# distributed-lab/era-boojum

Measured on AMD Instinct MI355X. Metric: LDE+Merkle commit Goldilocks elems/s (2^22x256, LDE x4), higher is better.
Workload: dtype u64 (Goldilocks); 1 GPU; C3: 2^22 rows x 256 cols, LDE x4, Poseidon2 cap 16; rows=4194304, cols=256, lde=4, cap=16, tree_hasher=poseidon2, parallelism=single, launch=stream

## Files before the change

### era-boojum_amd/csrc/ntt_ct_common.hpp

```cpp
#pragma once
#include <hip/hip_runtime.h>
#include "gl.hpp"
#include "gl_asm.hpp"
#include "ntt_pow2.hpp"

namespace bj {
namespace {

constexpr int NT = 256;
constexpr int PT = 32;
constexpr int TILE = NT * PT;

__device__ __forceinline__ void split2(uint64_t x, uint32_t& lo, uint32_t& hi) {
    lo = (uint32_t)x;
    hi = (uint32_t)(x >> 32);
}
__device__ __forceinline__ uint64_t join2(uint32_t lo, uint32_t hi) { return ((uint64_t)hi << 32) | lo; }

__device__ __forceinline__ void ct_bfly_x4(uint64_t& xa0, uint64_t& xc0, uint64_t& xa1, uint64_t& xc1,
                                           uint64_t& xa2, uint64_t& xc2, uint64_t& xa3, uint64_t& xc3, uint64_t w0,
                                           uint64_t w1, uint64_t w2, uint64_t w3) {
    uint64_t A[4], C[4];
    glasm::ct_bfly_x4((uint32_t)xa0, (uint32_t)(xa0 >> 32), (uint32_t)xc0, (uint32_t)(xc0 >> 32), (uint32_t)w0,
                      (uint32_t)(w0 >> 32), A[0], C[0],
                      (uint32_t)xa1, (uint32_t)(xa1 >> 32), (uint32_t)xc1, (uint32_t)(xc1 >> 32), (uint32_t)w1,
                      (uint32_t)(w1 >> 32), A[1], C[1],
                      (uint32_t)xa2, (uint32_t)(xa2 >> 32), (uint32_t)xc2, (uint32_t)(xc2 >> 32), (uint32_t)w2,
                      (uint32_t)(w2 >> 32), A[2], C[2],
                      (uint32_t)xa3, (uint32_t)(xa3 >> 32), (uint32_t)xc3, (uint32_t)(xc3 >> 32), (uint32_t)w3,
                      (uint32_t)(w3 >> 32), A[3], C[3]);
    xa0 = A[0]; xc0 = C[0];
    xa1 = A[1]; xc1 = C[1];
    xa2 = A[2]; xc2 = C[2];
    xa3 = A[3]; xc3 = C[3];
}

__device__ __forceinline__ void mul4_by(uint64_t& x0, uint64_t& x1, uint64_t& x2, uint64_t& x3, uint64_t k) {
    uint32_t a0[4], a1[4], z0[4], z1[4], k0, k1;
    split2(k, k0, k1);
    split2(x0, a0[0], a1[0]); split2(x1, a0[1], a1[1]);
    split2(x2, a0[2], a1[2]); split2(x3, a0[3], a1[3]);
    glasm::mul_x4(a0[0], a1[0], k0, k1, z0[0], z1[0], a0[1], a1[1], k0, k1, z0[1], z1[1],
                  a0[2], a1[2], k0, k1, z0[2], z1[2], a0[3], a1[3], k0, k1, z0[3], z1[3]);
    x0 = join2(z0[0], z1[0]); x1 = join2(z0[1], z1[1]);
    x2 = join2(z0[2], z1[2]); x3 = join2(z0[3], z1[3]);
}

__device__ __forceinline__ constexpr int pair_lo(int q, int hk) { return (q / hk) * 2 * hk + (q % hk); }

template <int HK>
__device__ __forceinline__ void ct_stage(uint64_t* x, const uint64_t* w) {
#pragma unroll
    for (int b = 0; b < 4; b++) {
        const int q0 = 4 * b;
        ct_bfly_x4(x[pair_lo(q0, HK)], x[pair_lo(q0, HK) + HK], x[pair_lo(q0 + 1, HK)], x[pair_lo(q0 + 1, HK) + HK],
                   x[pair_lo(q0 + 2, HK)], x[pair_lo(q0 + 2, HK) + HK], x[pair_lo(q0 + 3, HK)],
                   x[pair_lo(q0 + 3, HK) + HK], w[q0], w[q0 + 1], w[q0 + 2], w[q0 + 3]);
    }
}

__device__ __forceinline__ void canon4(uint64_t* x) {
    uint32_t z0[4], z1[4];
    glasm::canon_x4((uint32_t)x[0], (uint32_t)(x[0] >> 32), z0[0], z1[0], (uint32_t)x[1], (uint32_t)(x[1] >> 32), z0[1],
                    z1[1], (uint32_t)x[2], (uint32_t)(x[2] >> 32), z0[2], z1[2], (uint32_t)x[3], (uint32_t)(x[3] >> 32),
                    z0[3], z1[3]);
#pragma unroll
    for (int i = 0; i < 4; i++) x[i] = join2(z0[i], z1[i]);
}

__device__ __forceinline__ uint64_t canon_u64(uint64_t v) {
    uint32_t a0, a1, z0, z1;
    split2(v, a0, a1);
    glasm::canon_x1(a0, a1, z0, z1);
    return join2(z0, z1);
}

constexpr size_t EXT_HB = 32;
constexpr size_t EXT_TA = 32 + 1024;
__host__ __device__ __forceinline__ size_t ext_tb(uint32_t u0) { return EXT_TA + ((size_t)32 << u0); }

template <int LOG, bool INV, int B>
__device__ __forceinline__ void dft_p2(uint64_t* x) {
    using namespace p2dft;
    if constexpr (LOG == 1) { if constexpr (INV) dft2_inv<B>(x); else dft2_fwd<B>(x); }
    if constexpr (LOG == 2) { if constexpr (INV) dft4_inv<B>(x); else dft4_fwd<B>(x); }
    if constexpr (LOG == 3) { if constexpr (INV) dft8_inv<B>(x); else dft8_fwd<B>(x); }
    if constexpr (LOG == 4) { if constexpr (INV) dft16_inv<B>(x); else dft16_fwd<B>(x); }
    if constexpr (LOG == 5) { if constexpr (INV) dft32_inv<B>(x); else dft32_fwd<B>(x); }
}

template <int LOG, bool INV, int G = 0>
__device__ __forceinline__ void dft_p2_groups(uint64_t* x) {
    if constexpr (G < (32 >> LOG)) {
        dft_p2<LOG, INV, (G << LOG)>(x);
        dft_p2_groups<LOG, INV, G + 1>(x);
    }
}

__device__ __forceinline__ void load32(uint64_t* r, const uint64_t* __restrict__ f) {
#pragma unroll
    for (int k = 0; k < PT; k++) r[k] = f[k];
}

template <int K>
__device__ __forceinline__ void prescale_n(uint64_t* x, const uint64_t* f) {
#pragma unroll
    for (int k = 0; k < K; k += 4) {
        uint32_t z0[4], z1[4];
        glasm::mul_x4((uint32_t)x[k], (uint32_t)(x[k] >> 32), (uint32_t)f[k], (uint32_t)(f[k] >> 32), z0[0], z1[0],
                      (uint32_t)x[k + 1], (uint32_t)(x[k + 1] >> 32), (uint32_t)f[k + 1], (uint32_t)(f[k + 1] >> 32),
                      z0[1], z1[1], (uint32_t)x[k + 2], (uint32_t)(x[k + 2] >> 32), (uint32_t)f[k + 2],
                      (uint32_t)(f[k + 2] >> 32), z0[2], z1[2], (uint32_t)x[k + 3], (uint32_t)(x[k + 3] >> 32),
                      (uint32_t)f[k + 3], (uint32_t)(f[k + 3] >> 32), z0[3], z1[3]);
#pragma unroll
        for (int i = 0; i < 4; i++) x[k + i] = join2(z0[i], z1[i]);
    }
}

__device__ __forceinline__ void prescale32(uint64_t* x, const uint64_t* f) {
#pragma unroll
    for (int k = 0; k < PT; k += 4) {
        uint32_t z0[4], z1[4];
        glasm::mul_x4((uint32_t)x[k], (uint32_t)(x[k] >> 32), (uint32_t)f[k], (uint32_t)(f[k] >> 32), z0[0], z1[0],
                      (uint32_t)x[k + 1], (uint32_t)(x[k + 1] >> 32), (uint32_t)f[k + 1], (uint32_t)(f[k + 1] >> 32),
                      z0[1], z1[1], (uint32_t)x[k + 2], (uint32_t)(x[k + 2] >> 32), (uint32_t)f[k + 2],
                      (uint32_t)(f[k + 2] >> 32), z0[2], z1[2], (uint32_t)x[k + 3], (uint32_t)(x[k + 3] >> 32),
                      (uint32_t)f[k + 3], (uint32_t)(f[k + 3] >> 32), z0[3], z1[3]);
#pragma unroll
        for (int i = 0; i < 4; i++) x[k + i] = join2(z0[i], z1[i]);
    }
}

constexpr int PAD_LDS = TILE + TILE / 32;

__device__ __forceinline__ uint32_t tail_base_a(uint32_t t) { return t + (t >> 5); }
__device__ __forceinline__ uint32_t tail_base_b(uint32_t thi, uint32_t tlo) { return 264 * thi + tlo; }
__device__ __forceinline__ uint32_t tail_base_c(uint32_t t) { return 33 * t; }
__device__ __forceinline__ constexpr uint32_t tail_off_a(int k) { return 264 * k; }
__device__ __forceinline__ constexpr uint32_t tail_off_b(int k) { return 8 * k + (k >> 2); }

template <int V>
__device__ __forceinline__ void tw_ct_tailC(uint64_t* w, const uint64_t* __restrict__ ct, uint32_t u0, size_t q,
                                            uint32_t t) {
    constexpr int HK = 4 >> (V - 10);
    const uint64_t* base = ct + ((size_t)1 << (u0 + V)) + (q << V) + ((size_t)t << (V - 8));
#pragma unroll
    for (int p = 0; p < 16; p++) w[p] = base[pair_lo(p, HK) >> (13 - V)];
}

}
}
```

### era-boojum_amd/csrc/ntt_lde3.hip

```cpp
#include <hip/hip_runtime.h>
#include "gl.hpp"
#include "gl_asm.hpp"
#include "ntt_pow2.hpp"
#include "ntt_ct_common.hpp"
#include "bj_internal.hpp"

namespace bj {

namespace {

constexpr size_t L3_C = 0;
constexpr size_t L3_HA = 8192;
constexpr size_t L3_HB = L3_HA + 32;
constexpr size_t L3_F1 = L3_HB + 1024;
constexpr size_t L3_U = L3_F1 + ((size_t)1 << 18);
constexpr size_t L3_A = L3_U + 1024;
constexpr size_t L3_F2 = L3_A + ((size_t)1 << 18);

__host__ __device__ constexpr uint32_t cbrev(uint32_t x, int bits) {
    uint32_t r = 0;
    for (int i = 0; i < bits; i++) r |= ((x >> i) & 1u) << (bits - 1 - i);
    return r;
}

__device__ __forceinline__ uint32_t brev(uint32_t x, int bits) {
    return bits == 0 ? 0u : (__builtin_bitreverse32(x) >> (32 - bits));
}

__device__ __forceinline__ void prescale32_brev(uint64_t* y, const uint64_t* x, const uint64_t* f) {
#pragma unroll
    for (int k = 0; k < PT; k += 4) {
        uint32_t z0[4], z1[4];
        const uint64_t a0 = x[cbrev(k, 5)], a1 = x[cbrev(k + 1, 5)], a2 = x[cbrev(k + 2, 5)], a3 = x[cbrev(k + 3, 5)];
        glasm::mul_x4((uint32_t)a0, (uint32_t)(a0 >> 32), (uint32_t)f[k], (uint32_t)(f[k] >> 32), z0[0], z1[0],
                      (uint32_t)a1, (uint32_t)(a1 >> 32), (uint32_t)f[k + 1], (uint32_t)(f[k + 1] >> 32), z0[1], z1[1],
                      (uint32_t)a2, (uint32_t)(a2 >> 32), (uint32_t)f[k + 2], (uint32_t)(f[k + 2] >> 32), z0[2], z1[2],
                      (uint32_t)a3, (uint32_t)(a3 >> 32), (uint32_t)f[k + 3], (uint32_t)(f[k + 3] >> 32), z0[3],
                      z1[3]);
#pragma unroll
        for (int i = 0; i < 4; i++) y[k + i] = join2(z0[i], z1[i]);
    }
}

__device__ __forceinline__ __amdgpu_buffer_rsrc_t uniform_rsrc(const uint64_t* p, uint32_t bytes) {
    const uint64_t a = (uint64_t)p;
    const uint32_t lo = __builtin_amdgcn_readfirstlane((uint32_t)a);
    const uint32_t hi = __builtin_amdgcn_readfirstlane((uint32_t)(a >> 32));
    return __builtin_amdgcn_make_buffer_rsrc((void*)(((uint64_t)hi << 32) | lo), 0, (int)bytes, 0x00020000);
}

typedef unsigned int u32x2 __attribute__((ext_vector_type(2)));
__device__ __forceinline__ u32x2 as_u32x2(uint64_t v) {
    u32x2 r;
    r.x = (uint32_t)v;
    r.y = (uint32_t)(v >> 32);
    return r;
}
__device__ __forceinline__ uint64_t from_u32x2(u32x2 v) { return ((uint64_t)v.y << 32) | v.x; }

__device__ __forceinline__ void prescale32_brev_uniform(uint64_t* y, const uint64_t* x, const uint64_t* __restrict__ h) {
#pragma unroll
    for (int k8 = 0; k8 < PT; k8 += 8) {
        uint64_t hf[8];
#pragma unroll
        for (int i = 0; i < 8; i++) hf[i] = h[k8 + i];
#pragma unroll
        for (int k = k8; k < k8 + 8; k += 4) {
            uint32_t z0[4], z1[4];
            const uint64_t a0 = x[cbrev(k, 5)], a1 = x[cbrev(k + 1, 5)], a2 = x[cbrev(k + 2, 5)], a3 = x[cbrev(k + 3, 5)];
            const uint64_t f0 = hf[k - k8], f1 = hf[k - k8 + 1], f2 = hf[k - k8 + 2], f3 = hf[k - k8 + 3];
            glasm::mul_sb_x4((uint32_t)a0, (uint32_t)(a0 >> 32), (uint32_t)f0, (uint32_t)(f0 >> 32), z0[0], z1[0],
                             (uint32_t)a1, (uint32_t)(a1 >> 32), (uint32_t)f1, (uint32_t)(f1 >> 32), z0[1], z1[1],
                             (uint32_t)a2, (uint32_t)(a2 >> 32), (uint32_t)f2, (uint32_t)(f2 >> 32), z0[2], z1[2],
                             (uint32_t)a3, (uint32_t)(a3 >> 32), (uint32_t)f3, (uint32_t)(f3 >> 32), z0[3], z1[3]);
#pragma unroll
            for (int i = 0; i < 4; i++) y[k + i] = join2(z0[i], z1[i]);
        }
    }
}

__device__ __forceinline__ constexpr int c_reg(int e) { return 8 * (e / 7) + e % 7 + 1; }
template <int E0, int E1>
__device__ __forceinline__ void load_c(uint64_t* f, const uint64_t* __restrict__ c) {
#pragma unroll
    for (int e = E0; e < E1; e++) f[c_reg(e)] = c[c_reg(e)];
}

template <int E0, int E1>
__device__ __forceinline__ void prescale_c(uint64_t* y, const uint64_t* f) {
#pragma unroll
    for (int q = E0 / 4; q < E1 / 4; q++) {
        int k[4];
#pragma unroll
        for (int i = 0; i < 4; i++) k[i] = c_reg(4 * q + i);
        uint32_t z0[4], z1[4];
        glasm::mul_x4((uint32_t)y[k[0]], (uint32_t)(y[k[0]] >> 32), (uint32_t)f[k[0]], (uint32_t)(f[k[0]] >> 32), z0[0],
                      z1[0], (uint32_t)y[k[1]], (uint32_t)(y[k[1]] >> 32), (uint32_t)f[k[1]],
                      (uint32_t)(f[k[1]] >> 32), z0[1], z1[1], (uint32_t)y[k[2]], (uint32_t)(y[k[2]] >> 32),
                      (uint32_t)f[k[2]], (uint32_t)(f[k[2]] >> 32), z0[2], z1[2], (uint32_t)y[k[3]],
                      (uint32_t)(y[k[3]] >> 32), (uint32_t)f[k[3]], (uint32_t)(f[k[3]] >> 32), z0[3], z1[3]);
#pragma unroll
        for (int i = 0; i < 4; i++) y[k[i]] = join2(z0[i], z1[i]);
    }
}

__device__ __forceinline__ size_t coset_offset(uint32_t i, size_t coset_stride, size_t block_stride, uint32_t log_k) {
    return (size_t)(i >> log_k) * block_stride + (size_t)(i & ((1u << log_k) - 1)) * coset_stride;
}

template <int R>
__device__ __forceinline__ void inverse_tail13(uint64_t* x, const uint64_t* __restrict__ inv_tab, uint32_t q,
                                               uint32_t t, uint64_t* lds) {
    constexpr uint32_t LOGN = R + 13;
    const uint32_t ba = tail_base_a(t), bc = tail_base_c(t);
    const uint64_t* ext = inv_tab + ((size_t)1 << LOGN);
    uint64_t f[PT], wa[16], wb[16], wc[16];
    load32(f, ext + EXT_TA + (size_t)q * 32);
    prescale32(x, f);
    dft_p2<5, true, 0>(x);
    const uint32_t tlo = t & 7, thi = t >> 3;
    const uint32_t bb = tail_base_b(thi, tlo);
#pragma unroll
    for (int k = 0; k < PT; k++) lds[ba + tail_off_a(k)] = x[k];
    const uint64_t* tb = ext + ext_tb(R) + ((((size_t)q << 5) | thi) << 5);
#pragma unroll
    for (int k = 0; k < 16; k++) f[k] = tb[k];
    __syncthreads();
#pragma unroll
    for (int k = 0; k < PT; k++) x[k] = lds[bb + tail_off_b(k)];
    prescale_n<8>(x, f);
#pragma unroll
    for (int k = 16; k < 24; k++) f[k] = tb[k];
    prescale_n<8>(x + 8, f + 8);
#pragma unroll
    for (int k = 24; k < PT; k++) f[k] = tb[k];
    prescale_n<8>(x + 16, f + 16);
    prescale_n<8>(x + 24, f + 24);
    dft_p2<5, true, 0>(x);
    tw_ct_tailC<10>(wa, inv_tab, R, q, t);
#pragma unroll
    for (int k = 0; k < PT; k++) lds[bb + tail_off_b(k)] = x[k];
    tw_ct_tailC<11>(wb, inv_tab, R, q, t);
    tw_ct_tailC<12>(wc, inv_tab, R, q, t);
    __syncthreads();
#pragma unroll
    for (int k = 0; k < PT; k++) x[k] = lds[bc + k];
    ct_stage<4>(x, wa);
    ct_stage<2>(x, wb);
    ct_stage<1>(x, wc);
}

template <int R, bool INV_PART, bool MONO>
__global__ __launch_bounds__(NT, 2) void lde3_mid_kernel(const uint64_t* src, size_t src_stride, uint64_t* mono,
                                                         size_t mono_stride, uint64_t* lde, size_t col_stride,
                                                         size_t coset_stride, size_t block_stride, uint32_t log_k, uint32_t n_cols, uint32_t n_cosets,
                                                         const uint64_t* __restrict__ inv_tab,
                                                         const uint64_t* __restrict__ tabs, size_t tab_stride) {
    constexpr uint32_t LOGN = R + 13;
    constexpr int LW = 13 - R;
    constexpr uint32_t W = 1u << LW;
    __shared__ uint64_t lds[PAD_LDS];
    const uint32_t t = threadIdx.x;
    const uint32_t c = __builtin_amdgcn_readfirstlane(blockIdx.x % n_cols);
    const uint32_t q = __builtin_amdgcn_readfirstlane(blockIdx.x / n_cols);
    const uint64_t* blk = src + (size_t)c * src_stride + (size_t)q * TILE;
    const uint32_t ba = tail_base_a(t), bc = tail_base_c(t);
    uint64_t x[PT];
    {
        const auto rb = uniform_rsrc(blk, 8u * TILE);
#pragma unroll
        for (int k = 0; k < PT; k++)
            x[k] = from_u32x2(__builtin_amdgcn_raw_buffer_load_b64(rb, (int)(t * 8), k * 2048, 0));
    }
    if constexpr (INV_PART) {
        inverse_tail13<R>(x, inv_tab, q, t, lds);
    } else {
#pragma unroll
        for (int k = 0; k < PT; k++) lds[ba + tail_off_a(k)] = x[k];
        __syncthreads();
#pragma unroll
        for (int k = 0; k < PT; k++) x[k] = lds[bc + k];
    }
    if constexpr (MONO) {
#pragma unroll
        for (int k = 0; k < PT; k += 4) {
            uint64_t v[4] = {x[k], x[k + 1], x[k + 2], x[k + 3]};
            canon4(v);
#pragma unroll
            for (int i = 0; i < 4; i++) lds[bc + k + i] = v[i];
        }
        __syncthreads();
        const auto rm = uniform_rsrc(mono + (size_t)c * mono_stride + (size_t)q * TILE, 8u * TILE);
#pragma unroll
        for (int k = 0; k < PT; k++)
            __builtin_amdgcn_raw_buffer_store_b64(as_u32x2(lds[ba + tail_off_a(k)]), rm, (int)(t * 8), k * 2048, 0);
    }
    const uint32_t s8 = brev(t, 8);
    const uint32_t b1 = 33 * t;
    const uint32_t b2 = 1056 * (t >> 5) + (t & 31);
    const uint32_t b3 = s8 + (s8 >> 5);
    const uint32_t g5 = brev(t & 31, 5);
    const uint32_t qrot = ((q & 31u) << (R - 5)) | (q >> 5);
    const uint32_t vo = ((t >> LW) << 13) + qrot * W + (t & (W - 1));
#pragma unroll 1
    for (uint32_t i = 0; i < n_cosets; i++) {
        const uint64_t* tab = tabs + (size_t)i * tab_stride;
        uint64_t y[PT], f[PT];
        prescale32_brev_uniform(y, x, tab + L3_HA);
        dft_p2<5, false, 0>(y);
        __syncthreads();
#pragma unroll
        for (int k = 0; k < PT; k++) lds[b1 + cbrev(k, 5)] = y[k];
        const uint64_t* hb = tab + L3_HB + 32 * g5;
#pragma unroll
        for (int k = 0; k < 16; k++) f[k] = hb[k];
        __syncthreads();
#pragma unroll
        for (int k = 0; k < PT; k++) y[k] = lds[b2 + 33 * cbrev(k, 5)];
        prescale_n<8>(y, f);
#pragma unroll
        for (int k = 16; k < 24; k++) f[k] = hb[k];
        prescale_n<8>(y + 8, f + 8);
#pragma unroll
        for (int k = 24; k < PT; k++) f[k] = hb[k];
        prescale_n<8>(y + 16, f + 16);
        prescale_n<8>(y + 24, f + 24);
        dft_p2<5, false, 0>(y);
#pragma unroll
        for (int k = 0; k < PT; k++) lds[b2 + 33 * cbrev(k, 5)] = y[k];
        const uint64_t* fc = tab + L3_C + 32 * t;
        load_c<0, 16>(f, fc);
        __syncthreads();
#pragma unroll
        for (int k = 0; k < PT; k++) y[k] = lds[b3 + 264 * cbrev(k, 5)];
        prescale_c<0, 8>(y, f);
        load_c<16, 28>(f, fc);
        prescale_c<8, 16>(y, f);
        prescale_c<16, 28>(y, f);
        dft_p2_groups<3, false>(y);
        __syncthreads();
#pragma unroll
        for (int k = 0; k < PT; k++) lds[bc + k] = y[k];
        __syncthreads();
#pragma unroll
        for (int k = 0; k < PT; k++) y[k] = lds[ba + tail_off_a(k)];
        const auto rs = uniform_rsrc(lde + (size_t)c * col_stride + coset_offset(i, coset_stride, block_stride, log_k), 8u << LOGN);
#pragma unroll
        for (int k = 0; k < PT; k++)
            __builtin_amdgcn_raw_buffer_store_b64(as_u32x2(y[k]), rs, (int)(vo * 8), (int)((uint32_t)k << (24 - LW)),
                                                  0);
    }
}

constexpr uint32_t kInvFoldConsts = 256;
struct InvFoldZ {
    uint64_t z[kInvFoldConsts];
};

template <uint32_t OUTS, uint32_t F>
__device__ __forceinline__ void fold_term(uint64_t* acc, const uint64_t* x, uint32_t b, uint64_t zb, bool set) {
    const uint32_t z0 = (uint32_t)zb, z1 = (uint32_t)(zb >> 32);
#pragma unroll
    for (uint32_t i = 0; i < OUTS; i += 4) {
        uint32_t p0[4], p1[4], s0[4], s1[4];
        glasm::mul_sb_x4((uint32_t)x[F * i + b], (uint32_t)(x[F * i + b] >> 32), z0, z1, p0[0], p1[0],
                         (uint32_t)x[F * (i + 1) + b], (uint32_t)(x[F * (i + 1) + b] >> 32), z0, z1, p0[1], p1[1],
                         (uint32_t)x[F * (i + 2) + b], (uint32_t)(x[F * (i + 2) + b] >> 32), z0, z1, p0[2], p1[2],
                         (uint32_t)x[F * (i + 3) + b], (uint32_t)(x[F * (i + 3) + b] >> 32), z0, z1, p0[3], p1[3]);
        if (set) {
#pragma unroll
            for (int j = 0; j < 4; j++) acc[i + j] = join2(p0[j], p1[j]);
            continue;
        }
        glasm::add_x4((uint32_t)acc[i], (uint32_t)(acc[i] >> 32), p0[0], p1[0], s0[0], s1[0], (uint32_t)acc[i + 1],
                      (uint32_t)(acc[i + 1] >> 32), p0[1], p1[1], s0[1], s1[1], (uint32_t)acc[i + 2],
                      (uint32_t)(acc[i + 2] >> 32), p0[2], p1[2], s0[2], s1[2], (uint32_t)acc[i + 3],
                      (uint32_t)(acc[i + 3] >> 32), p0[3], p1[3], s0[3], s1[3]);
#pragma unroll
        for (int j = 0; j < 4; j++) acc[i + j] = join2(s0[j], s1[j]);
    }
}

__device__ __forceinline__ void add_sub4(uint64_t* a, uint64_t* b) {
    uint32_t s0[4], s1[4], d0[4], d1[4];
    glasm::add_x4((uint32_t)a[0], (uint32_t)(a[0] >> 32), (uint32_t)b[0], (uint32_t)(b[0] >> 32), s0[0], s1[0],
                  (uint32_t)a[1], (uint32_t)(a[1] >> 32), (uint32_t)b[1], (uint32_t)(b[1] >> 32), s0[1], s1[1],
                  (uint32_t)a[2], (uint32_t)(a[2] >> 32), (uint32_t)b[2], (uint32_t)(b[2] >> 32), s0[2], s1[2],
                  (uint32_t)a[3], (uint32_t)(a[3] >> 32), (uint32_t)b[3], (uint32_t)(b[3] >> 32), s0[3], s1[3]);
    glasm::sub_x4((uint32_t)a[0], (uint32_t)(a[0] >> 32), (uint32_t)b[0], (uint32_t)(b[0] >> 32), d0[0], d1[0],
                  (uint32_t)a[1], (uint32_t)(a[1] >> 32), (uint32_t)b[1], (uint32_t)(b[1] >> 32), d0[1], d1[1],
                  (uint32_t)a[2], (uint32_t)(a[2] >> 32), (uint32_t)b[2], (uint32_t)(b[2] >> 32), d0[2], d1[2],
                  (uint32_t)a[3], (uint32_t)(a[3] >> 32), (uint32_t)b[3], (uint32_t)(b[3] >> 32), d0[3], d1[3]);
#pragma unroll
    for (int j = 0; j < 4; j++) {
        a[j] = join2(s0[j], s1[j]);
        b[j] = join2(d0[j], d1[j]);
    }
}

template <uint32_t OUTS>
__device__ __forceinline__ void store_fold_target(const uint64_t* h, uint64_t* lds, uint32_t P, uint32_t t, uint64_t* dst,
                                                  size_t dst_col_stride, size_t dst_shard_stride, uint32_t c,
                                                  uint32_t q) {
    constexpr uint32_t BLK = NT * OUTS, HALF = PAD_LDS / 2;
    uint64_t* buf = lds + (P & 1) * HALF;
#pragma unroll
    for (uint32_t i = 0; i < OUTS; i++) {
        const uint32_t w = OUTS * t + i;
        buf[w + (w >> 5)] = h[i];
    }
    __syncthreads();
    const auto rs = uniform_rsrc(dst + (size_t)P * dst_shard_stride + (size_t)c * dst_col_stride + (size_t)q * BLK,
                                 8u * BLK);
#pragma unroll
    for (uint32_t k = 0; k < OUTS; k++) {
        const uint32_t w = t + NT * k;
        __builtin_amdgcn_raw_buffer_store_b64(as_u32x2(buf[w + (w >> 5)]), rs, (int)(t * 8), (int)(k * 2048), 0);
    }
}

template <int R, int LOG_F>
__global__ __launch_bounds__(NT, 2) void lde3_inv_fold_kernel(const uint64_t* src, size_t src_stride, uint64_t* dst,
                                                              size_t dst_col_stride, size_t dst_shard_stride,
                                                              uint32_t n_cols, uint32_t shards, uint32_t paired,
                                                              const uint64_t* __restrict__ inv_tab, InvFoldZ zc) {
    __shared__ uint64_t lds[PAD_LDS];
    const uint32_t t = threadIdx.x;
    const uint32_t rest = blockIdx.x >> 3;
    const uint32_t c = __builtin_amdgcn_readfirstlane(rest % n_cols);
    const uint32_t q = __builtin_amdgcn_readfirstlane(((rest / n_cols) << 3) | (blockIdx.x & 7));
    uint64_t x[PT];
    {
        const auto rb = uniform_rsrc(src + (size_t)c * src_stride + (size_t)q * TILE, 8u * TILE);
#pragma unroll
        for (int k = 0; k < PT; k++)
            x[k] = from_u32x2(__builtin_amdgcn_raw_buffer_load_b64(rb, (int)(t * 8), k * 2048, 0));
    }
    inverse_tail13<R>(x, inv_tab, q, t, lds);
    {
        constexpr uint32_t F = 1u << LOG_F, OUTS = PT / F, BLK = TILE / F, HALF = PAD_LDS / 2;
        static_assert(OUTS % 4 == 0 && BLK + BLK / 32 <= HALF, "fold layout");
        __syncthreads();
        if (paired) {
#pragma unroll 1
            for (uint32_t P = 0; P < shards; P += 2) {
                uint64_t h0[OUTS], h1[OUTS];
                if constexpr (F == 2) {
                    const uint64_t z = zc.z[P * F + 1];
#pragma unroll
                    for (uint32_t i = 0; i < OUTS; i++) {
                        h0[i] = x[2 * i];
                        h1[i] = x[2 * i + 1];
                    }
#pragma unroll
                    for (uint32_t i = 0; i < OUTS; i += 4)
                        ct_bfly_x4(h0[i], h1[i], h0[i + 1], h1[i + 1], h0[i + 2], h1[i + 2], h0[i + 3], h1[i + 3], z,
                                   z, z, z);
                } else {
                    uint64_t e[OUTS], o[OUTS];
#pragma unroll
                    for (uint32_t i = 0; i < OUTS; i++) e[i] = x[F * i];
#pragma unroll
                    for (uint32_t b = 1; b < F; b++)
                        fold_term<OUTS, F>(b < F / 2 ? e : o, x, b, zc.z[P * F + b], b == F / 2);
#pragma unroll
                    for (uint32_t i = 0; i < OUTS; i += 4)
                        for (int j = 0; j < 4; j++) {
                            h0[i + j] = e[i + j];
                            h1[i + j] = o[i + j];
                        }
#pragma unroll
                    for (uint32_t i = 0; i < OUTS; i += 4) add_sub4(h0 + i, h1 + i);
                }
#pragma unroll
                for (uint32_t i = 0; i < OUTS; i += 4) {
                    canon4(h0 + i);
                    canon4(h1 + i);
                }
                store_fold_target<OUTS>(h0, lds, P, t, dst, dst_col_stride, dst_shard_stride, c, q);
                store_fold_target<OUTS>(h1, lds, P + 1, t, dst, dst_col_stride, dst_shard_stride, c, q);
            }
            return;
        }
#pragma unroll 1
        for (uint32_t P = 0; P < shards; P++) {
            uint64_t h[OUTS];
#pragma unroll
            for (uint32_t i = 0; i < OUTS; i++) h[i] = x[F * i];
#pragma unroll
            for (uint32_t b = 1; b < F; b++) fold_term<OUTS, F>(h, x, b, zc.z[P * F + b], false);
#pragma unroll
            for (uint32_t i = 0; i < OUTS; i += 4) canon4(h + i);
            store_fold_target<OUTS>(h, lds, P, t, dst, dst_col_stride, dst_shard_stride, c, q);
        }
    }
}

template <int R>
__device__ __forceinline__ constexpr uint32_t fin_slot(uint32_t r, uint32_t o) {
    const uint32_t e = R == 5 ? (o << R) + r : r * (1u << (13 - R)) + o;
    return e + (e >> 5);
}
template <int R>
__device__ __forceinline__ constexpr uint32_t fin_p1(uint32_t t, uint32_t k) {
    constexpr int LW = 13 - R;
    return fin_slot<R>((k << (R - 5)) + cbrev(t >> LW, R - 5), t & ((1u << LW) - 1));
}
template <int R>
__device__ __forceinline__ constexpr uint32_t fin_p2(uint32_t t, uint32_t k) {
    constexpr int LW = 13 - R;
    const uint32_t h = k >> (R - 5), rl = k & ((1u << (R - 5)) - 1);
    const uint32_t p = (t >> LW) + (h << (R - 5));
    return fin_slot<R>((p << (R - 5)) + rl, t & ((1u << LW) - 1));
}
template <int R>
__device__ __forceinline__ constexpr uint32_t fin_p3(uint32_t t, uint32_t k) {
    const uint32_t P = t + 256 * k;
    return fin_slot<R>(P & ((1u << R) - 1), P >> R);
}

template <int R>
struct FinLds {
    static constexpr int LW = 13 - R, RL = R - 5;
    static constexpr uint32_t W = 1u << LW;
    static constexpr bool F1_LDS = R >= 8;
    static constexpr uint32_t F1 = F1_LDS ? 32 * W : 0;
    static constexpr uint32_t A = (1u << RL) * W;
    static constexpr uint32_t UP = (1u << RL) + 1;
    static constexpr uint32_t U = 32 * UP;
};

template <int R, int F2MODE>
__global__ __launch_bounds__(NT, 2) void lde3_final_kernel(uint64_t* lde, size_t col_stride, size_t coset_stride, size_t block_stride, uint32_t log_k,
                                                           uint32_t n_cols, uint32_t n_cosets,
                                                           const uint64_t* __restrict__ tabs, size_t tab_stride) {
    using FL = FinLds<R>;
    constexpr int LW = FL::LW, RL = FL::RL;
    constexpr uint32_t W = FL::W;
    __shared__ uint64_t lds[PAD_LDS];
    __shared__ uint64_t lf1[FL::F1 ? FL::F1 : 1];
    __shared__ uint64_t la[R > 5 && F2MODE == 1 ? FL::A : 1];
    __shared__ uint64_t lu[R > 5 && F2MODE == 1 ? FL::U : 1];
    const uint32_t t = threadIdx.x;
    const uint32_t rest = blockIdx.x >> 3;
    const uint32_t c = __builtin_amdgcn_readfirstlane(rest % n_cols);
    const uint32_t pair = ((rest / n_cols) << 3) | (blockIdx.x & 7);
    const uint32_t i = __builtin_amdgcn_readfirstlane(pair % n_cosets);
    const uint32_t T = __builtin_amdgcn_readfirstlane(pair / n_cosets);
    uint64_t* d = lde + (size_t)c * col_stride + coset_offset(i, coset_stride, block_stride, log_k) + (size_t)T * TILE;
    const uint64_t* tab = tabs + (size_t)i * tab_stride;
    const uint32_t o = t & (W - 1);
    const uint32_t M0 = T * W, M = M0 + o;
    uint64_t x[PT], y[PT], f[PT];
    const auto rd = uniform_rsrc(d, 8u * TILE);
    constexpr uint32_t NF1 = FL::F1_LDS ? FL::F1 / NT : 1;
    uint64_t f1v[NF1];
    if constexpr (FL::F1_LDS) {
#pragma unroll
        for (uint32_t j = 0; j < NF1; j++) {
            const uint32_t e = t + j * NT;
            f1v[j] = tab[L3_F1 + ((size_t)(e >> LW) << 13) + M0 + (e & (W - 1))];
        }
    }
#pragma unroll
    for (int k = 0; k < PT; k++) x[k] = from_u32x2(__builtin_amdgcn_raw_buffer_load_b64(rd, (int)(t * 8), k * 2048, 0));
    if constexpr (R > 5 && F2MODE == 1) {
        la[t] = tab[L3_A + ((size_t)(t >> LW) << 13) + M0 + (t & (W - 1))];
#pragma unroll
        for (uint32_t e = t; e < (32u << RL); e += NT) lu[(e >> RL) * FL::UP + (e & ((1u << RL) - 1))] = tab[L3_U + e];
    }
    uint64_t g2[F2MODE == 0 && R > 5 ? PT : 1];
    if constexpr (F2MODE == 0 && R > 5) {
        const auto rf = uniform_rsrc(tab + L3_F2 + M0, 8u << (R + 13));
        const int vf = (int)((o + ((t >> LW) << 13)) * 8);
#pragma unroll
        for (int k = 0; k < PT; k++) {
            const uint32_t h = k >> RL, rl = k & ((1u << RL) - 1);
            g2[k] = from_u32x2(__builtin_amdgcn_raw_buffer_load_b64(rf, vf, (int)((rl * 32 + (h << RL)) << 16), 0));
        }
    }
    if constexpr (FL::F1_LDS) {
#pragma unroll
        for (uint32_t j = 0; j < NF1; j++) lf1[t + j * NT] = f1v[j];
        __syncthreads();
#pragma unroll
        for (int k = 0; k < PT; k++) f[k] = lf1[k * W + o];
    } else {
        const uint64_t* f1 = tab + L3_F1 + M;
#pragma unroll
        for (int k = 0; k < PT; k++) f[k] = f1[(size_t)k << 13];
    }
    prescale32_brev(y, x, f);
    dft_p2<5, false, 0>(y);
    const uint32_t b1 = fin_p1<R>(t, 0);
#pragma unroll
    for (int k = 0; k < PT; k++) lds[b1 + (fin_p1<R>(0, k) - fin_p1<R>(0, 0))] = y[k];
    if constexpr (R > 5) {
        const uint32_t pl = t >> LW;
        if constexpr (F2MODE == 1) {
            if constexpr (!FL::F1_LDS) __syncthreads();
            uint64_t a[PT];
#pragma unroll
            for (int k = 0; k < PT; k++) {
                const uint32_t h = k >> RL, rl = k & ((1u << RL) - 1);
                a[k] = la[rl * W + o];
                f[k] = lu[(pl + (h << RL)) * FL::UP + rl];
            }
            prescale32(f, a);
        } else {
#pragma unroll
            for (int k = 0; k < PT; k++) f[k] = g2[k];
        }
        __syncthreads();
        const uint32_t b2 = fin_p2<R>(t, 0);
#pragma unroll
        for (int k = 0; k < PT; k++) y[k] = lds[b2 + (fin_p2<R>(0, k) - fin_p2<R>(0, 0))];
        prescale32(y, f);
        dft_p2_groups<RL, false>(y);
#pragma unroll
        for (int k = 0; k < PT; k++) lds[b2 + (fin_p2<R>(0, k) - fin_p2<R>(0, 0))] = y[k];
    }
    __syncthreads();
    const uint32_t b3 = fin_p3<R>(t, 0);
#pragma unroll
    for (int k = 0; k < PT; k++) y[k] = lds[b3 + (fin_p3<R>(0, k) - fin_p3<R>(0, 0))];
#pragma unroll
    for (int k = 0; k < PT; k += 4) canon4(y + k);
#pragma unroll
    for (int k = 0; k < PT; k++) __builtin_amdgcn_raw_buffer_store_b64(as_u32x2(y[k]), rd, (int)(t * 8), k * 2048, 0);
}

__global__ void lde3_table_kernel(uint64_t* out, uint32_t log_n, uint64_t w_n, uint64_t s, size_t len) {
    const size_t n = (size_t)1 << log_n;
    const uint32_t R = log_n - 13;
    for (size_t idx = blockIdx.x * (size_t)blockDim.x + threadIdx.x; idx < len;
         idx += (size_t)gridDim.x * blockDim.x) {
        uint64_t v;
        if (idx < L3_HA) {
            const uint32_t G = (uint32_t)idx >> 3, j = (uint32_t)idx & 7;
            const uint64_t sigma = gl::mul(s, gl::pow(w_n, gl::bitrev32(G, 10)));
            v = gl::pow(sigma, (n >> 13) * j);
        } else if (idx < L3_HB) {
            v = gl::pow(s, (n >> 5) * (idx - L3_HA));
        } else if (idx < L3_F1) {
            const uint32_t j = (uint32_t)(idx - L3_HB);
            const uint64_t sigma = gl::mul(s, gl::pow(w_n, gl::bitrev32(j >> 5, 5)));
            v = gl::pow(sigma, (n >> 10) * (j & 31));
        } else if (idx < L3_U) {
            const uint32_t j = (uint32_t)(idx - L3_F1);
            const uint32_t M = j & 8191, k = j >> 13;
            const uint64_t sigma = gl::mul(s, gl::pow(w_n, gl::bitrev32(M, 13)));
            v = gl::pow(sigma, (uint64_t)k << (R - 5));
        } else if (idx < L3_A) {
            const uint32_t j = (uint32_t)(idx - L3_U);
            const uint32_t p = j >> (R - 5), rl = j & ((1u << (R - 5)) - 1);
            v = (j >> R) ? 0 : gl::pow(gl::pow(w_n, 8192), (uint64_t)gl::bitrev32(p, 5) * rl);
        } else if (idx < L3_F2) {
            const uint32_t j = (uint32_t)(idx - L3_A);
            const uint32_t M = j & 8191, rl = j >> 13;
            const uint64_t sigma = gl::mul(s, gl::pow(w_n, gl::bitrev32(M, 13)));
            v = (rl >> (R - 5)) ? 0 : gl::pow(sigma, rl);
        } else {
            const size_t j = idx - L3_F2;
            const uint32_t M = (uint32_t)(j & 8191), rest = (uint32_t)(j >> 13);
            const uint32_t p = rest & 31, rl = rest >> 5;
            const uint64_t sigma = gl::mul(s, gl::pow(w_n, gl::bitrev32(M * 32 + p, 18)));
            v = gl::pow(sigma, rl);
        }
        out[idx] = gl::canon(v);
    }
}

template <int R>
void launch_lde3_R(uint64_t* lde, size_t col_stride, size_t coset_stride, size_t block_stride, uint32_t log_k, uint32_t n_cosets, const uint64_t* src,
                   size_t src_stride, uint64_t* mono, size_t mono_stride, uint32_t n_cols, const uint64_t* inv_tab,
                   const uint64_t* tabs, size_t tab_stride, hipStream_t st, uint32_t passes) {
    const dim3 gm(n_cols << R);
    if (!(passes & LDE3_MID))
        ;
    else if (inv_tab && mono)
        hipLaunchKernelGGL((lde3_mid_kernel<R, true, true>), gm, dim3(NT), 0, st, src, src_stride, mono, mono_stride,
                           lde, col_stride, coset_stride, block_stride, log_k, n_cols, n_cosets, inv_tab, tabs, tab_stride);
    else if (inv_tab)
        hipLaunchKernelGGL((lde3_mid_kernel<R, true, false>), gm, dim3(NT), 0, st, src, src_stride, mono,
                           mono_stride, lde, col_stride, coset_stride, block_stride, log_k, n_cols, n_cosets, inv_tab, tabs, tab_stride);
    else
        hipLaunchKernelGGL((lde3_mid_kernel<R, false, false>), gm, dim3(NT), 0, st, src, src_stride, mono,
                           mono_stride, lde, col_stride, coset_stride, block_stride, log_k, n_cols, n_cosets, inv_tab, tabs, tab_stride);
    const dim3 gf((n_cols * n_cosets) << R);
    if (passes & LDE3_FINAL)
        hipLaunchKernelGGL((lde3_final_kernel<R, 0>), gf, dim3(NT), 0, st, lde, col_stride, coset_stride, block_stride,
                           log_k, n_cols, n_cosets, tabs, tab_stride);
}

}

bool lde3_supported(uint32_t log_n) { return log_n >= 18 && log_n <= 23; }

size_t lde3_table_len(uint32_t log_n) {
    return log_n > 18 ? L3_F2 + ((size_t)1 << log_n) : L3_F2;
}

hipError_t launch_lde3_table(uint64_t* out, uint32_t log_n, uint64_t shift, hipStream_t st) {
    if (!lde3_supported(log_n)) return hipErrorInvalidValue;
    const size_t len = lde3_table_len(log_n);
    size_t blocks = (len + 255) / 256;
    if (blocks > 16384) blocks = 16384;
    hipLaunchKernelGGL(lde3_table_kernel, dim3((unsigned)blocks), dim3(256), 0, st, out, log_n,
                       gl::domain_generator(log_n), gl::canon(shift), len);
    return hipGetLastError();
}

hipError_t launch_lde3(uint64_t* lde, size_t col_stride, size_t coset_stride, uint32_t n_cosets, const uint64_t* src,
                       size_t src_stride, uint64_t* mono, size_t mono_stride, uint32_t n_cols, uint32_t log_n,
                       const uint64_t* inv_tab, const uint64_t* tabs, size_t tab_stride, hipStream_t st,
                       uint32_t log_k, size_t block_stride, uint32_t passes) {
    if (n_cols == 0 || n_cosets == 0) return hipSuccess;
    if (log_k > 31) log_k = 31;
    if (!lde3_supported(log_n)) return hipErrorInvalidValue;
    if (((uint64_t)n_cols * n_cosets) << (log_n - 13) > (0xffffffffull / NT)) return hipErrorInvalidValue;
#define BJ_LDE3(RR)                                                                                              \
    launch_lde3_R<RR>(lde, col_stride, coset_stride, block_stride, log_k, n_cosets, src, src_stride, mono, mono_stride, n_cols, inv_tab, \
                      tabs, tab_stride, st, passes)
    switch (log_n - 13) {
        case 5: BJ_LDE3(5); break;
        case 6: BJ_LDE3(6); break;
        case 7: BJ_LDE3(7); break;
        case 8: BJ_LDE3(8); break;
        case 9: BJ_LDE3(9); break;
        default: BJ_LDE3(10); break;
    }
#undef BJ_LDE3
    return hipGetLastError();
}

namespace {
template <int R>
void launch_lde3_inv_fold_R(uint64_t* dst, size_t dst_col_stride, size_t dst_shard_stride, const uint64_t* src,
                            size_t src_stride, uint32_t n_cols, uint32_t log_f, uint32_t shards, uint32_t paired,
                            const uint64_t* inv_tab, const InvFoldZ& zc, hipStream_t st) {
    const dim3 g(n_cols << R);
#define BJ_INV(LF)                                                                                             \
    hipLaunchKernelGGL((lde3_inv_fold_kernel<R, LF>), g, dim3(NT), 0, st, src, src_stride, dst, dst_col_stride, \
                       dst_shard_stride, n_cols, shards, paired, inv_tab, zc)
    switch (log_f) {
        case 1: BJ_INV(1); break;
        case 2: BJ_INV(2); break;
        default: BJ_INV(3); break;
    }
#undef BJ_INV
}
}

bool lde3_inv_fold_supported(uint32_t log_n, uint32_t log_f, uint32_t shards) {
    return lde3_supported(log_n) && log_f >= 1 && log_f <= 3 && shards >= 1 &&
           (size_t)shards << log_f <= kInvFoldConsts;
}

hipError_t launch_lde3_inv_fold(uint64_t* dst, size_t dst_col_stride, size_t dst_shard_stride, const uint64_t* src,
                                size_t src_stride, uint32_t n_cols, uint32_t log_n, uint32_t log_f, uint32_t shards,
                                const uint64_t* s_pow_m, const uint64_t* inv_tab, hipStream_t st) {
    if (n_cols == 0) return hipSuccess;
    if (!lde3_inv_fold_supported(log_n, log_f, shards)) return hipErrorInvalidValue;
    if (((uint64_t)n_cols << (log_n - 13)) > 0xffffffffull / NT) return hipErrorInvalidValue;
    InvFoldZ zc{};
    const uint32_t F = 1u << log_f;
    for (uint32_t P = 0; P < shards; P++) {
        uint64_t acc = 1;
        for (uint32_t a = 0; a < F; a++) {
            zc.z[P * F + gl::bitrev32(a, log_f)] = acc;
            acc = gl::mul(acc, s_pow_m[P]);
        }
    }
    uint32_t paired = shards % 2 == 0 && !knobs().inv_fold_unpaired;
    for (uint32_t P = 0; paired && P < shards; P += 2)
        paired = gl::canon(s_pow_m[P + 1]) == gl::canon(gl::sub(0, s_pow_m[P]));
#define BJ_INVR(RR) \
    launch_lde3_inv_fold_R<RR>(dst, dst_col_stride, dst_shard_stride, src, src_stride, n_cols, log_f, shards, paired, \
                               inv_tab, zc, st)
    switch (log_n - 13) {
        case 5: BJ_INVR(5); break;
        case 6: BJ_INVR(6); break;
        case 7: BJ_INVR(7); break;
        case 8: BJ_INVR(8); break;
        case 9: BJ_INVR(9); break;
        default: BJ_INVR(10); break;
    }
#undef BJ_INVR
    return hipGetLastError();
}

}
```

### era-boojum_amd/csrc/ntt_pow2.hpp

```cpp
#pragma once
#include <stdint.h>

namespace glasm {

__device__ __forceinline__ void p2c0_x1(uint32_t a00, uint32_t a10, uint32_t c00, uint32_t c10, uint64_t& A0, uint64_t& C0) {
    uint64_t q40, q42, q64;
    uint32_t k66;
    asm volatile(
        "v_mov_b32 v10, 0xfffeffff\n"
        "s_mov_b32 %[k66], 0xffff\n"
        "v_add_co_u32 v0, %[q40], %[c00], -1\n"
        "s_nop 1\n"
        "v_addc_co_u32 v1, %[q40], %[c10], 0, %[q40]\n"
        "s_nop 1\n"
        "v_cndmask_b32_e64 v2, %[c00], v0, %[q40]\n"
        "v_cndmask_b32_e64 v3, %[c10], v1, %[q40]\n"
        "v_sub_co_u32 v0, %[q42], %[a00], v2\n"
        "s_nop 1\n"
        "v_subb_co_u32 v1, %[q42], %[a10], v3, %[q42]\n"
        "s_nop 1\n"
        "v_cndmask_b32_e64 v6, 0, v10, %[q42]\n"
        "v_mad_i64_i32 %[C0], %[q64], v6, %[k66], v[0:1]\n"
        "v_add_co_u32 v4, %[q40], %[a00], v2\n"
        "s_nop 1\n"
// ... 653 lines not shown
        "v_cndmask_b32_e64 v23, v23, v21, %[q52]\n"
        "v_cndmask_b32_e64 v33, v33, v31, %[q58]\n"
        "v_sub_co_u32 v0, %[q42], %[a00], v2\n"
        "v_sub_co_u32 v10, %[q48], %[a01], v12\n"
        "v_sub_co_u32 v20, %[q54], %[a02], v22\n"
        "v_sub_co_u32 v30, %[q60], %[a03], v32\n"
        "v_subb_co_u32 v1, %[q42], %[a10], v3, %[q42]\n"
        "v_subb_co_u32 v11, %[q48], %[a11], v13, %[q48]\n"
        "v_subb_co_u32 v21, %[q54], %[a12], v23, %[q54]\n"
        "v_subb_co_u32 v31, %[q60], %[a13], v33, %[q60]\n"
        "v_cndmask_b32_e64 v6, 0, v40, %[q42]\n"
        "v_cndmask_b32_e64 v16, 0, v40, %[q48]\n"
        "v_cndmask_b32_e64 v26, 0, v40, %[q54]\n"
        "v_cndmask_b32_e64 v36, 0, v40, %[q60]\n"
        "v_mad_i64_i32 %[C0], %[q64], v6, %[k66], v[0:1]\n"
        "v_mad_i64_i32 %[C1], %[q64], v16, %[k66], v[10:11]\n"
        "v_mad_i64_i32 %[C2], %[q64], v26, %[k66], v[20:21]\n"
        "v_mad_i64_i32 %[C3], %[q64], v36, %[k66], v[30:31]\n"
        "v_add_co_u32 v4, %[q40], %[a00], v2\n"
        "v_add_co_u32 v14, %[q46], %[a01], v12\n"
        "v_add_co_u32 v24, %[q52], %[a02], v22\n"
        "v_add_co_u32 v34, %[q58], %[a03], v32\n"
        "v_addc_co_u32 v5, %[q40], %[a10], v3, %[q40]\n"
        "v_addc_co_u32 v15, %[q46], %[a11], v13, %[q46]\n"
        "v_addc_co_u32 v25, %[q52], %[a12], v23, %[q52]\n"
        "v_addc_co_u32 v35, %[q58], %[a13], v33, %[q58]\n"
        "v_cndmask_b32_e64 v2, 0, -1, %[q40]\n"
        "v_cndmask_b32_e64 v12, 0, -1, %[q46]\n"
        "v_cndmask_b32_e64 v22, 0, -1, %[q52]\n"
        "v_cndmask_b32_e64 v32, 0, -1, %[q58]\n"
        "v_mad_u64_u32 %[A0], %[q64], v2, 1, v[4:5]\n"
        "v_mad_u64_u32 %[A1], %[q64], v12, 1, v[14:15]\n"
        "v_mad_u64_u32 %[A2], %[q64], v22, 1, v[24:25]\n"
        "v_mad_u64_u32 %[A3], %[q64], v32, 1, v[34:35]\n"
        : [A0] "=&v"(A0), [C0] "=&v"(C0), [A1] "=&v"(A1), [C1] "=&v"(C1), [A2] "=&v"(A2), [C2] "=&v"(C2), [A3] "=&v"(A3), [C3] "=&v"(C3), [q40] "=&s"(q40), [q42] "=&s"(q42), [q46] "=&s"(q46), [q48] "=&s"(q48), [q52] "=&s"(q52), [q54] "=&s"(q54), [q58] "=&s"(q58), [q60] "=&s"(q60), [q64] "=&s"(q64), [k66] "=&s"(k66)
        : [a00] "v"(a00), [a10] "v"(a10), [c00] "v"(c00), [c10] "v"(c10), [e0] "n"(S0), [r0] "n"(32 - S0), [a01] "v"(a01), [a11] "v"(a11), [c01] "v"(c01), [c11] "v"(c11), [e1] "n"(S1), [r1] "n"(32 - S1), [a02] "v"(a02), [a12] "v"(a12), [c02] "v"(c02), [c12] "v"(c12), [e2] "n"(S2), [r2] "n"(32 - S2), [a03] "v"(a03), [a13] "v"(a13), [c03] "v"(c03), [c13] "v"(c13), [e3] "n"(S3), [r3] "n"(32 - S3)
        : "v0", "v1", "v2", "v3", "v4", "v5", "v6", "v7", "v8", "v9", "v10", "v11", "v12", "v13", "v14", "v15", "v16", "v17", "v18", "v19", "v20", "v21", "v22", "v23", "v24", "v25", "v26", "v27", "v28", "v29", "v30", "v31", "v32", "v33", "v34", "v35", "v36", "v37", "v38", "v39", "v40");
}

template <int S0>
__device__ __forceinline__ void p2c3_x1(uint32_t a00, uint32_t a10, uint32_t c00, uint32_t c10, uint64_t& A0, uint64_t& C0) {
    uint64_t q40, q42, q64;
    uint32_t k66;
    asm volatile(
        "v_mov_b32 v10, 0xfffeffff\n"
        "s_mov_b32 %[k66], 0xffff\n"
        "v_lshlrev_b32 v8, %[e0], %[c00]\n"
        "v_alignbit_b32 v4, %[c10], %[c00], %[r0]\n"
        "v_lshrrev_b32 v5, %[r0], %[c10]\n"
        "v_mad_u64_u32 v[2:3], %[q64], v8, -1, 0\n"
        "v_sub_co_u32 v2, %[q42], v2, v4\n"
        "s_nop 1\n"
        "v_subb_co_u32 v3, %[q42], v3, v5, %[q42]\n"
        "s_nop 1\n"
        "v_cndmask_b32_e64 v9, 0, v10, %[q42]\n"
        "v_mad_i64_i32 v[2:3], %[q64], v9, %[k66], v[2:3]\n"
        "v_add_co_u32 v0, %[q40], v2, -1\n"
        "s_nop 1\n"
        "v_addc_co_u32 v1, %[q40], v3, 0, %[q40]\n"
        "s_nop 1\n"
        "v_cndmask_b32_e64 v2, v2, v0, %[q40]\n"
        "v_cndmask_b32_e64 v3, v3, v1, %[q40]\n"
        "v_sub_co_u32 v0, %[q42], %[a00], v2\n"
        "s_nop 1\n"
        "v_subb_co_u32 v1, %[q42], %[a10], v3, %[q42]\n"
        "s_nop 1\n"
        "v_cndmask_b32_e64 v6, 0, v10, %[q42]\n"
        "v_mad_i64_i32 %[C0], %[q64], v6, %[k66], v[0:1]\n"
        "v_add_co_u32 v4, %[q40], %[a00], v2\n"
        "s_nop 1\n"
        "v_addc_co_u32 v5, %[q40], %[a10], v3, %[q40]\n"
        "s_nop 1\n"
        "v_cndmask_b32_e64 v2, 0, -1, %[q40]\n"
        "v_mad_u64_u32 %[A0], %[q64], v2, 1, v[4:5]\n"
        : [A0] "=&v"(A0), [C0] "=&v"(C0), [q40] "=&s"(q40), [q42] "=&s"(q42), [q64] "=&s"(q64), [k66] "=&s"(k66)
        : [a00] "v"(a00), [a10] "v"(a10), [c00] "v"(c00), [c10] "v"(c10), [e0] "n"(S0), [r0] "n"(32 - S0)
        : "v0", "v1", "v2", "v3", "v4", "v5", "v6", "v7", "v8", "v9", "v10");
}

template <int S0, int S1>
__device__ __forceinline__ void p2c3_x2(uint32_t a00, uint32_t a10, uint32_t c00, uint32_t c10, uint64_t& A0, uint64_t& C0, uint32_t a01, uint32_t a11, uint32_t c01, uint32_t c11, uint64_t& A1, uint64_t& C1) {
    uint64_t q40, q42, q46, q48, q64;
    uint32_t k66;
    asm volatile(
        "v_mov_b32 v20, 0xfffeffff\n"
        "s_mov_b32 %[k66], 0xffff\n"
        "v_lshlrev_b32 v8, %[e0], %[c00]\n"
        "v_lshlrev_b32 v18, %[e1], %[c01]\n"
        "v_alignbit_b32 v4, %[c10], %[c00], %[r0]\n"
        "v_alignbit_b32 v14, %[c11], %[c01], %[r1]\n"
        "v_lshrrev_b32 v5, %[r0], %[c10]\n"
        "v_lshrrev_b32 v15, %[r1], %[c11]\n"
        "v_mad_u64_u32 v[2:3], %[q64], v8, -1, 0\n"
        "v_mad_u64_u32 v[12:13], %[q64], v18, -1, 0\n"
        "v_sub_co_u32 v2, %[q42], v2, v4\n"
        "v_sub_co_u32 v12, %[q48], v12, v14\n"
        "s_nop 0\n"
        "v_subb_co_u32 v3, %[q42], v3, v5, %[q42]\n"
        "v_subb_co_u32 v13, %[q48], v13, v15, %[q48]\n"
        "s_nop 0\n"
        "v_cndmask_b32_e64 v9, 0, v20, %[q42]\n"
        "v_cndmask_b32_e64 v19, 0, v20, %[q48]\n"
        "v_mad_i64_i32 v[2:3], %[q64], v9, %[k66], v[2:3]\n"
        "v_mad_i64_i32 v[12:13], %[q64], v19, %[k66], v[12:13]\n"
        "v_add_co_u32 v0, %[q40], v2, -1\n"
        "v_add_co_u32 v10, %[q46], v12, -1\n"
        "s_nop 0\n"
        "v_addc_co_u32 v1, %[q40], v3, 0, %[q40]\n"
        "v_addc_co_u32 v11, %[q46], v13, 0, %[q46]\n"
        "s_nop 0\n"
        "v_cndmask_b32_e64 v2, v2, v0, %[q40]\n"
        "v_cndmask_b32_e64 v12, v12, v10, %[q46]\n"
        "v_cndmask_b32_e64 v3, v3, v1, %[q40]\n"
        "v_cndmask_b32_e64 v13, v13, v11, %[q46]\n"
        "v_sub_co_u32 v0, %[q42], %[a00], v2\n"
        "v_sub_co_u32 v10, %[q48], %[a01], v12\n"
        "s_nop 0\n"
        "v_subb_co_u32 v1, %[q42], %[a10], v3, %[q42]\n"
        "v_subb_co_u32 v11, %[q48], %[a11], v13, %[q48]\n"
        "s_nop 0\n"
        "v_cndmask_b32_e64 v6, 0, v20, %[q42]\n"
        "v_cndmask_b32_e64 v16, 0, v20, %[q48]\n"
        "v_mad_i64_i32 %[C0], %[q64], v6, %[k66], v[0:1]\n"
        "v_mad_i64_i32 %[C1], %[q64], v16, %[k66], v[10:11]\n"
        "v_add_co_u32 v4, %[q40], %[a00], v2\n"
        "v_add_co_u32 v14, %[q46], %[a01], v12\n"
        "s_nop 0\n"
        "v_addc_co_u32 v5, %[q40], %[a10], v3, %[q40]\n"
        "v_addc_co_u32 v15, %[q46], %[a11], v13, %[q46]\n"
        "s_nop 0\n"
        "v_cndmask_b32_e64 v2, 0, -1, %[q40]\n"
        "v_cndmask_b32_e64 v12, 0, -1, %[q46]\n"
        "v_mad_u64_u32 %[A0], %[q64], v2, 1, v[4:5]\n"
        "v_mad_u64_u32 %[A1], %[q64], v12, 1, v[14:15]\n"
        : [A0] "=&v"(A0), [C0] "=&v"(C0), [A1] "=&v"(A1), [C1] "=&v"(C1), [q40] "=&s"(q40), [q42] "=&s"(q42), [q46] "=&s"(q46), [q48] "=&s"(q48), [q64] "=&s"(q64), [k66] "=&s"(k66)
        : [a00] "v"(a00), [a10] "v"(a10), [c00] "v"(c00), [c10] "v"(c10), [e0] "n"(S0), [r0] "n"(32 - S0), [a01] "v"(a01), [a11] "v"(a11), [c01] "v"(c01), [c11] "v"(c11), [e1] "n"(S1), [r1] "n"(32 - S1)
        : "v0", "v1", "v2", "v3", "v4", "v5", "v6", "v7", "v8", "v9", "v10", "v11", "v12", "v13", "v14", "v15", "v16", "v17", "v18", "v19", "v20");
}

template <int S0, int S1, int S2>
__device__ __forceinline__ void p2c3_x3(uint32_t a00, uint32_t a10, uint32_t c00, uint32_t c10, uint64_t& A0, uint64_t& C0, uint32_t a01, uint32_t a11, uint32_t c01, uint32_t c11, uint64_t& A1, uint64_t& C1, uint32_t a02, uint32_t a12, uint32_t c02, uint32_t c12, uint64_t& A2, uint64_t& C2) {
    uint64_t q40, q42, q46, q48, q52, q54, q64;
    uint32_t k66;
    asm volatile(
        "v_mov_b32 v30, 0xfffeffff\n"
        "s_mov_b32 %[k66], 0xffff\n"
        "v_lshlrev_b32 v8, %[e0], %[c00]\n"
        "v_lshlrev_b32 v18, %[e1], %[c01]\n"
        "v_lshlrev_b32 v28, %[e2], %[c02]\n"
        "v_alignbit_b32 v4, %[c10], %[c00], %[r0]\n"
        "v_alignbit_b32 v14, %[c11], %[c01], %[r1]\n"
        "v_alignbit_b32 v24, %[c12], %[c02], %[r2]\n"
        "v_lshrrev_b32 v5, %[r0], %[c10]\n"
        "v_lshrrev_b32 v15, %[r1], %[c11]\n"
        "v_lshrrev_b32 v25, %[r2], %[c12]\n"
        "v_mad_u64_u32 v[2:3], %[q64], v8, -1, 0\n"
        "v_mad_u64_u32 v[12:13], %[q64], v18, -1, 0\n"
        "v_mad_u64_u32 v[22:23], %[q64], v28, -1, 0\n"
        "v_sub_co_u32 v2, %[q42], v2, v4\n"
        "v_sub_co_u32 v12, %[q48], v12, v14\n"
        "v_sub_co_u32 v22, %[q54], v22, v24\n"
        "v_subb_co_u32 v3, %[q42], v3, v5, %[q42]\n"
        "v_subb_co_u32 v13, %[q48], v13, v15, %[q48]\n"
        "v_subb_co_u32 v23, %[q54], v23, v25, %[q54]\n"
        "v_cndmask_b32_e64 v9, 0, v30, %[q42]\n"
        "v_cndmask_b32_e64 v19, 0, v30, %[q48]\n"
        "v_cndmask_b32_e64 v29, 0, v30, %[q54]\n"
        "v_mad_i64_i32 v[2:3], %[q64], v9, %[k66], v[2:3]\n"
        "v_mad_i64_i32 v[12:13], %[q64], v19, %[k66], v[12:13]\n"
        "v_mad_i64_i32 v[22:23], %[q64], v29, %[k66], v[22:23]\n"
        "v_add_co_u32 v0, %[q40], v2, -1\n"
        "v_add_co_u32 v10, %[q46], v12, -1\n"
        "v_add_co_u32 v20, %[q52], v22, -1\n"
        "v_addc_co_u32 v1, %[q40], v3, 0, %[q40]\n"
        "v_addc_co_u32 v11, %[q46], v13, 0, %[q46]\n"
        "v_addc_co_u32 v21, %[q52], v23, 0, %[q52]\n"
        "v_cndmask_b32_e64 v2, v2, v0, %[q40]\n"
        "v_cndmask_b32_e64 v12, v12, v10, %[q46]\n"
        "v_cndmask_b32_e64 v22, v22, v20, %[q52]\n"
        "v_cndmask_b32_e64 v3, v3, v1, %[q40]\n"
        "v_cndmask_b32_e64 v13, v13, v11, %[q46]\n"
        "v_cndmask_b32_e64 v23, v23, v21, %[q52]\n"
        "v_sub_co_u32 v0, %[q42], %[a00], v2\n"
        "v_sub_co_u32 v10, %[q48], %[a01], v12\n"
        "v_sub_co_u32 v20, %[q54], %[a02], v22\n"
        "v_subb_co_u32 v1, %[q42], %[a10], v3, %[q42]\n"
        "v_subb_co_u32 v11, %[q48], %[a11], v13, %[q48]\n"
        "v_subb_co_u32 v21, %[q54], %[a12], v23, %[q54]\n"
        "v_cndmask_b32_e64 v6, 0, v30, %[q42]\n"
        "v_cndmask_b32_e64 v16, 0, v30, %[q48]\n"
        "v_cndmask_b32_e64 v26, 0, v30, %[q54]\n"
        "v_mad_i64_i32 %[C0], %[q64], v6, %[k66], v[0:1]\n"
        "v_mad_i64_i32 %[C1], %[q64], v16, %[k66], v[10:11]\n"
        "v_mad_i64_i32 %[C2], %[q64], v26, %[k66], v[20:21]\n"
        "v_add_co_u32 v4, %[q40], %[a00], v2\n"
        "v_add_co_u32 v14, %[q46], %[a01], v12\n"
        "v_add_co_u32 v24, %[q52], %[a02], v22\n"
        "v_addc_co_u32 v5, %[q40], %[a10], v3, %[q40]\n"
        "v_addc_co_u32 v15, %[q46], %[a11], v13, %[q46]\n"
        "v_addc_co_u32 v25, %[q52], %[a12], v23, %[q52]\n"
        "v_cndmask_b32_e64 v2, 0, -1, %[q40]\n"
        "v_cndmask_b32_e64 v12, 0, -1, %[q46]\n"
        "v_cndmask_b32_e64 v22, 0, -1, %[q52]\n"
        "v_mad_u64_u32 %[A0], %[q64], v2, 1, v[4:5]\n"
        "v_mad_u64_u32 %[A1], %[q64], v12, 1, v[14:15]\n"
        "v_mad_u64_u32 %[A2], %[q64], v22, 1, v[24:25]\n"
        : [A0] "=&v"(A0), [C0] "=&v"(C0), [A1] "=&v"(A1), [C1] "=&v"(C1), [A2] "=&v"(A2), [C2] "=&v"(C2), [q40] "=&s"(q40), [q42] "=&s"(q42), [q46] "=&s"(q46), [q48] "=&s"(q48), [q52] "=&s"(q52), [q54] "=&s"(q54), [q64] "=&s"(q64), [k66] "=&s"(k66)
        : [a00] "v"(a00), [a10] "v"(a10), [c00] "v"(c00), [c10] "v"(c10), [e0] "n"(S0), [r0] "n"(32 - S0), [a01] "v"(a01), [a11] "v"(a11), [c01] "v"(c01), [c11] "v"(c11), [e1] "n"(S1), [r1] "n"(32 - S1), [a02] "v"(a02), [a12] "v"(a12), [c02] "v"(c02), [c12] "v"(c12), [e2] "n"(S2), [r2] "n"(32 - S2)
        : "v0", "v1", "v2", "v3", "v4", "v5", "v6", "v7", "v8", "v9", "v10", "v11", "v12", "v13", "v14", "v15", "v16", "v17", "v18", "v19", "v20", "v21", "v22", "v23", "v24", "v25", "v26", "v27", "v28", "v29", "v30");
}

template <int S0, int S1, int S2, int S3>
__device__ __forceinline__ void p2c3_x4(uint32_t a00, uint32_t a10, uint32_t c00, uint32_t c10, uint64_t& A0, uint64_t& C0, uint32_t a01, uint32_t a11, uint32_t c01, uint32_t c11, uint64_t& A1, uint64_t& C1, uint32_t a02, uint32_t a12, uint32_t c02, uint32_t c12, uint64_t& A2, uint64_t& C2, uint32_t a03, uint32_t a13, uint32_t c03, uint32_t c13, uint64_t& A3, uint64_t& C3) {
    uint64_t q40, q42, q46, q48, q52, q54, q58, q60, q64;
    uint32_t k66;
    asm volatile(
        "v_mov_b32 v40, 0xfffeffff\n"
        "s_mov_b32 %[k66], 0xffff\n"
        "v_lshlrev_b32 v8, %[e0], %[c00]\n"
        "v_lshlrev_b32 v18, %[e1], %[c01]\n"
        "v_lshlrev_b32 v28, %[e2], %[c02]\n"
        "v_lshlrev_b32 v38, %[e3], %[c03]\n"
        "v_alignbit_b32 v4, %[c10], %[c00], %[r0]\n"
        "v_alignbit_b32 v14, %[c11], %[c01], %[r1]\n"
        "v_alignbit_b32 v24, %[c12], %[c02], %[r2]\n"
        "v_alignbit_b32 v34, %[c13], %[c03], %[r3]\n"
        "v_lshrrev_b32 v5, %[r0], %[c10]\n"
        "v_lshrrev_b32 v15, %[r1], %[c11]\n"
        "v_lshrrev_b32 v25, %[r2], %[c12]\n"
        "v_lshrrev_b32 v35, %[r3], %[c13]\n"
        "v_mad_u64_u32 v[2:3], %[q64], v8, -1, 0\n"
        "v_mad_u64_u32 v[12:13], %[q64], v18, -1, 0\n"
        "v_mad_u64_u32 v[22:23], %[q64], v28, -1, 0\n"
        "v_mad_u64_u32 v[32:33], %[q64], v38, -1, 0\n"
        "v_sub_co_u32 v2, %[q42], v2, v4\n"
        "v_sub_co_u32 v12, %[q48], v12, v14\n"
        "v_sub_co_u32 v22, %[q54], v22, v24\n"
        "v_sub_co_u32 v32, %[q60], v32, v34\n"
        "v_subb_co_u32 v3, %[q42], v3, v5, %[q42]\n"
        "v_subb_co_u32 v13, %[q48], v13, v15, %[q48]\n"
        "v_subb_co_u32 v23, %[q54], v23, v25, %[q54]\n"
        "v_subb_co_u32 v33, %[q60], v33, v35, %[q60]\n"
        "v_cndmask_b32_e64 v9, 0, v40, %[q42]\n"
        "v_cndmask_b32_e64 v19, 0, v40, %[q48]\n"
        "v_cndmask_b32_e64 v29, 0, v40, %[q54]\n"
        "v_cndmask_b32_e64 v39, 0, v40, %[q60]\n"
        "v_mad_i64_i32 v[2:3], %[q64], v9, %[k66], v[2:3]\n"
        "v_mad_i64_i32 v[12:13], %[q64], v19, %[k66], v[12:13]\n"
        "v_mad_i64_i32 v[22:23], %[q64], v29, %[k66], v[22:23]\n"
        "v_mad_i64_i32 v[32:33], %[q64], v39, %[k66], v[32:33]\n"
        "v_add_co_u32 v0, %[q40], v2, -1\n"
        "v_add_co_u32 v10, %[q46], v12, -1\n"
        "v_add_co_u32 v20, %[q52], v22, -1\n"
        "v_add_co_u32 v30, %[q58], v32, -1\n"
        "v_addc_co_u32 v1, %[q40], v3, 0, %[q40]\n"
        "v_addc_co_u32 v11, %[q46], v13, 0, %[q46]\n"
        "v_addc_co_u32 v21, %[q52], v23, 0, %[q52]\n"
        "v_addc_co_u32 v31, %[q58], v33, 0, %[q58]\n"
        "v_cndmask_b32_e64 v2, v2, v0, %[q40]\n"
        "v_cndmask_b32_e64 v12, v12, v10, %[q46]\n"
        "v_cndmask_b32_e64 v22, v22, v20, %[q52]\n"
        "v_cndmask_b32_e64 v32, v32, v30, %[q58]\n"
        "v_cndmask_b32_e64 v3, v3, v1, %[q40]\n"
        "v_cndmask_b32_e64 v13, v13, v11, %[q46]\n"
        "v_cndmask_b32_e64 v23, v23, v21, %[q52]\n"
        "v_cndmask_b32_e64 v33, v33, v31, %[q58]\n"
        "v_sub_co_u32 v0, %[q42], %[a00], v2\n"
        "v_sub_co_u32 v10, %[q48], %[a01], v12\n"
        "v_sub_co_u32 v20, %[q54], %[a02], v22\n"
        "v_sub_co_u32 v30, %[q60], %[a03], v32\n"
        "v_subb_co_u32 v1, %[q42], %[a10], v3, %[q42]\n"
        "v_subb_co_u32 v11, %[q48], %[a11], v13, %[q48]\n"
        "v_subb_co_u32 v21, %[q54], %[a12], v23, %[q54]\n"
        "v_subb_co_u32 v31, %[q60], %[a13], v33, %[q60]\n"
        "v_cndmask_b32_e64 v6, 0, v40, %[q42]\n"
        "v_cndmask_b32_e64 v16, 0, v40, %[q48]\n"
        "v_cndmask_b32_e64 v26, 0, v40, %[q54]\n"
        "v_cndmask_b32_e64 v36, 0, v40, %[q60]\n"
        "v_mad_i64_i32 %[C0], %[q64], v6, %[k66], v[0:1]\n"
        "v_mad_i64_i32 %[C1], %[q64], v16, %[k66], v[10:11]\n"
        "v_mad_i64_i32 %[C2], %[q64], v26, %[k66], v[20:21]\n"
        "v_mad_i64_i32 %[C3], %[q64], v36, %[k66], v[30:31]\n"
        "v_add_co_u32 v4, %[q40], %[a00], v2\n"
        "v_add_co_u32 v14, %[q46], %[a01], v12\n"
        "v_add_co_u32 v24, %[q52], %[a02], v22\n"
        "v_add_co_u32 v34, %[q58], %[a03], v32\n"
        "v_addc_co_u32 v5, %[q40], %[a10], v3, %[q40]\n"
        "v_addc_co_u32 v15, %[q46], %[a11], v13, %[q46]\n"
        "v_addc_co_u32 v25, %[q52], %[a12], v23, %[q52]\n"
        "v_addc_co_u32 v35, %[q58], %[a13], v33, %[q58]\n"
        "v_cndmask_b32_e64 v2, 0, -1, %[q40]\n"
        "v_cndmask_b32_e64 v12, 0, -1, %[q46]\n"
        "v_cndmask_b32_e64 v22, 0, -1, %[q52]\n"
        "v_cndmask_b32_e64 v32, 0, -1, %[q58]\n"
        "v_mad_u64_u32 %[A0], %[q64], v2, 1, v[4:5]\n"
        "v_mad_u64_u32 %[A1], %[q64], v12, 1, v[14:15]\n"
        "v_mad_u64_u32 %[A2], %[q64], v22, 1, v[24:25]\n"
        "v_mad_u64_u32 %[A3], %[q64], v32, 1, v[34:35]\n"
        : [A0] "=&v"(A0), [C0] "=&v"(C0), [A1] "=&v"(A1), [C1] "=&v"(C1), [A2] "=&v"(A2), [C2] "=&v"(C2), [A3] "=&v"(A3), [C3] "=&v"(C3), [q40] "=&s"(q40), [q42] "=&s"(q42), [q46] "=&s"(q46), [q48] "=&s"(q48), [q52] "=&s"(q52), [q54] "=&s"(q54), [q58] "=&s"(q58), [q60] "=&s"(q60), [q64] "=&s"(q64), [k66] "=&s"(k66)
        : [a00] "v"(a00), [a10] "v"(a10), [c00] "v"(c00), [c10] "v"(c10), [e0] "n"(S0), [r0] "n"(32 - S0), [a01] "v"(a01), [a11] "v"(a11), [c01] "v"(c01), [c11] "v"(c11), [e1] "n"(S1), [r1] "n"(32 - S1), [a02] "v"(a02), [a12] "v"(a12), [c02] "v"(c02), [c12] "v"(c12), [e2] "n"(S2), [r2] "n"(32 - S2), [a03] "v"(a03), [a13] "v"(a13), [c03] "v"(c03), [c13] "v"(c13), [e3] "n"(S3), [r3] "n"(32 - S3)
        : "v0", "v1", "v2", "v3", "v4", "v5", "v6", "v7", "v8", "v9", "v10", "v11", "v12", "v13", "v14", "v15", "v16", "v17", "v18", "v19", "v20", "v21", "v22", "v23", "v24", "v25", "v26", "v27", "v28", "v29", "v30", "v31", "v32", "v33", "v34", "v35", "v36", "v37", "v38", "v39", "v40");
}

}

namespace bj {
namespace p2dft {
#define LO(v) ((uint32_t)(v))
#define HI(v) ((uint32_t)((v) >> 32))

template <int B>
__device__ __forceinline__ void dft2_fwd(uint64_t* x) {
    {
        uint64_t ta0, tc0;
        glasm::p2c0_x1(LO(x[B + 0]), HI(x[B + 0]), LO(x[B + 1]), HI(x[B + 1]), ta0, tc0);
        x[B + 0] = ta0; x[B + 1] = tc0;
    }
}

template <int B>
__device__ __forceinline__ void dft4_fwd(uint64_t* x) {
    {
        uint64_t ta0, tc0, ta1, tc1;
        glasm::p2c0_x2(LO(x[B + 0]), HI(x[B + 0]), LO(x[B + 2]), HI(x[B + 2]), ta0, tc0, LO(x[B + 1]), HI(x[B + 1]), LO(x[B + 3]), HI(x[B + 3]), ta1, tc1);
        x[B + 0] = ta0; x[B + 2] = tc0;
        x[B + 1] = ta1; x[B + 3] = tc1;
    }
    {
        uint64_t ta0, tc0;
        glasm::p2c0_x1(LO(x[B + 0]), HI(x[B + 0]), LO(x[B + 1]), HI(x[B + 1]), ta0, tc0);
        x[B + 0] = ta0; x[B + 1] = tc0;
    }
    {
        uint64_t ta0, tc0;
        glasm::p2c2_x1<16>(LO(x[B + 2]), HI(x[B + 2]), LO(x[B + 3]), HI(x[B + 3]), ta0, tc0);
        x[B + 2] = ta0; x[B + 3] = tc0;
    }
}

template <int B>
__device__ __forceinline__ void dft8_fwd(uint64_t* x) {
    {
        uint64_t ta0, tc0, ta1, tc1, ta2, tc2, ta3, tc3;
        glasm::p2c0_x4(LO(x[B + 0]), HI(x[B + 0]), LO(x[B + 4]), HI(x[B + 4]), ta0, tc0, LO(x[B + 1]), HI(x[B + 1]), LO(x[B + 5]), HI(x[B + 5]), ta1, tc1, LO(x[B + 2]), HI(x[B + 2]), LO(x[B + 6]), HI(x[B + 6]), ta2, tc2, LO(x[B + 3]), HI(x[B + 3]), LO(x[B + 7]), HI(x[B + 7]), ta3, tc3);
        x[B + 0] = ta0; x[B + 4] = tc0;
        x[B + 1] = ta1; x[B + 5] = tc1;
        x[B + 2] = ta2; x[B + 6] = tc2;
        x[B + 3] = ta3; x[B + 7] = tc3;
    }
    {
        uint64_t ta0, tc0, ta1, tc1;
        glasm::p2c0_x2(LO(x[B + 0]), HI(x[B + 0]), LO(x[B + 2]), HI(x[B + 2]), ta0, tc0, LO(x[B + 1]), HI(x[B + 1]), LO(x[B + 3]), HI(x[B + 3]), ta1, tc1);
        x[B + 0] = ta0; x[B + 2] = tc0;
        x[B + 1] = ta1; x[B + 3] = tc1;
    }
    {
        uint64_t ta0, tc0, ta1, tc1;
        glasm::p2c2_x2<16, 16>(LO(x[B + 4]), HI(x[B + 4]), LO(x[B + 6]), HI(x[B + 6]), ta0, tc0, LO(x[B + 5]), HI(x[B + 5]), LO(x[B + 7]), HI(x[B + 7]), ta1, tc1);
        x[B + 4] = ta0; x[B + 6] = tc0;
        x[B + 5] = ta1; x[B + 7] = tc1;
    }
    {
        uint64_t ta0, tc0;
        glasm::p2c0_x1(LO(x[B + 0]), HI(x[B + 0]), LO(x[B + 1]), HI(x[B + 1]), ta0, tc0);
        x[B + 0] = ta0; x[B + 1] = tc0;
    }
    {
        uint64_t ta0, tc0;
        glasm::p2c1_x1<24>(LO(x[B + 4]), HI(x[B + 4]), LO(x[B + 5]), HI(x[B + 5]), ta0, tc0);
        x[B + 4] = tc0; x[B + 5] = ta0;
    }
    {
        uint64_t ta0, tc0;
        glasm::p2c2_x1<16>(LO(x[B + 2]), HI(x[B + 2]), LO(x[B + 3]), HI(x[B + 3]), ta0, tc0);
        x[B + 2] = ta0; x[B + 3] = tc0;
    }
    {
        uint64_t ta0, tc0;
        glasm::p2c3_x1<8>(LO(x[B + 6]), HI(x[B + 6]), LO(x[B + 7]), HI(x[B + 7]), ta0, tc0);
        x[B + 6] = tc0; x[B + 7] = ta0;
    }
}

template <int B>
__device__ __forceinline__ void dft16_fwd(uint64_t* x) {
    {
        uint64_t ta0, tc0, ta1, tc1, ta2, tc2, ta3, tc3;
        glasm::p2c0_x4(LO(x[B + 0]), HI(x[B + 0]), LO(x[B + 8]), HI(x[B + 8]), ta0, tc0, LO(x[B + 1]), HI(x[B + 1]), LO(x[B + 9]), HI(x[B + 9]), ta1, tc1, LO(x[B + 2]), HI(x[B + 2]), LO(x[B + 10]), HI(x[B + 10]), ta2, tc2, LO(x[B + 3]), HI(x[B + 3]), LO(x[B + 11]), HI(x[B + 11]), ta3, tc3);
        x[B + 0] = ta0; x[B + 8] = tc0;
        x[B + 1] = ta1; x[B + 9] = tc1;
        x[B + 2] = ta2; x[B + 10] = tc2;
        x[B + 3] = ta3; x[B + 11] = tc3;
    }
    {
        uint64_t ta0, tc0, ta1, tc1, ta2, tc2, ta3, tc3;
        glasm::p2c0_x4(LO(x[B + 4]), HI(x[B + 4]), LO(x[B + 12]), HI(x[B + 12]), ta0, tc0, LO(x[B + 5]), HI(x[B + 5]), LO(x[B + 13]), HI(x[B + 13]), ta1, tc1, LO(x[B + 6]), HI(x[B + 6]), LO(x[B + 14]), HI(x[B + 14]), ta2, tc2, LO(x[B + 7]), HI(x[B + 7]), LO(x[B + 15]), HI(x[B + 15]), ta3, tc3);
        x[B + 4] = ta0; x[B + 12] = tc0;
        x[B + 5] = ta1; x[B + 13] = tc1;
        x[B + 6] = ta2; x[B + 14] = tc2;
        x[B + 7] = ta3; x[B + 15] = tc3;
    }
    {
        uint64_t ta0, tc0, ta1, tc1, ta2, tc2, ta3, tc3;
        glasm::p2c0_x4(LO(x[B + 0]), HI(x[B + 0]), LO(x[B + 4]), HI(x[B + 4]), ta0, tc0, LO(x[B + 1]), HI(x[B + 1]), LO(x[B + 5]), HI(x[B + 5]), ta1, tc1, LO(x[B + 2]), HI(x[B + 2]), LO(x[B + 6]), HI(x[B + 6]), ta2, tc2, LO(x[B + 3]), HI(x[B + 3]), LO(x[B + 7]), HI(x[B + 7]), ta3, tc3);
        x[B + 0] = ta0; x[B + 4] = tc0;
        x[B + 1] = ta1; x[B + 5] = tc1;
        x[B + 2] = ta2; x[B + 6] = tc2;
        x[B + 3] = ta3; x[B + 7] = tc3;
    }
    {
        uint64_t ta0, tc0, ta1, tc1, ta2, tc2, ta3, tc3;
        glasm::p2c2_x4<16, 16, 16, 16>(LO(x[B + 8]), HI(x[B + 8]), LO(x[B + 12]), HI(x[B + 12]), ta0, tc0, LO(x[B + 9]), HI(x[B + 9]), LO(x[B + 13]), HI(x[B + 13]), ta1, tc1, LO(x[B + 10]), HI(x[B + 10]), LO(x[B + 14]), HI(x[B + 14]), ta2, tc2, LO(x[B + 11]), HI(x[B + 11]), LO(x[B + 15]), HI(x[B + 15]), ta3, tc3);
        x[B + 8] = ta0; x[B + 12] = tc0;
        x[B + 9] = ta1; x[B + 13] = tc1;
        x[B + 10] = ta2; x[B + 14] = tc2;
        x[B + 11] = ta3; x[B + 15] = tc3;
    }
    {
        uint64_t ta0, tc0, ta1, tc1;
        glasm::p2c0_x2(LO(x[B + 0]), HI(x[B + 0]), LO(x[B + 2]), HI(x[B + 2]), ta0, tc0, LO(x[B + 1]), HI(x[B + 1]), LO(x[B + 3]), HI(x[B + 3]), ta1, tc1);
        x[B + 0] = ta0; x[B + 2] = tc0;
        x[B + 1] = ta1; x[B + 3] = tc1;
    }
    {
        uint64_t ta0, tc0, ta1, tc1;
        glasm::p2c1_x2<24, 24>(LO(x[B + 8]), HI(x[B + 8]), LO(x[B + 10]), HI(x[B + 10]), ta0, tc0, LO(x[B + 9]), HI(x[B + 9]), LO(x[B + 11]), HI(x[B + 11]), ta1, tc1);
        x[B + 8] = tc0; x[B + 10] = ta0;
        x[B + 9] = tc1; x[B + 11] = ta1;
    }
    {
        uint64_t ta0, tc0, ta1, tc1;
        glasm::p2c2_x2<16, 16>(LO(x[B + 4]), HI(x[B + 4]), LO(x[B + 6]), HI(x[B + 6]), ta0, tc0, LO(x[B + 5]), HI(x[B + 5]), LO(x[B + 7]), HI(x[B + 7]), ta1, tc1);
        x[B + 4] = ta0; x[B + 6] = tc0;
        x[B + 5] = ta1; x[B + 7] = tc1;
    }
    {
        uint64_t ta0, tc0, ta1, tc1;
        glasm::p2c3_x2<8, 8>(LO(x[B + 12]), HI(x[B + 12]), LO(x[B + 14]), HI(x[B + 14]), ta0, tc0, LO(x[B + 13]), HI(x[B + 13]), LO(x[B + 15]), HI(x[B + 15]), ta1, tc1);
        x[B + 12] = tc0; x[B + 14] = ta0;
        x[B + 13] = tc1; x[B + 15] = ta1;
    }
    {
        uint64_t ta0, tc0;
        glasm::p2c0_x1(LO(x[B + 0]), HI(x[B + 0]), LO(x[B + 1]), HI(x[B + 1]), ta0, tc0);
        x[B + 0] = ta0; x[B + 1] = tc0;
    }
    {
        uint64_t ta0, tc0, ta1, tc1;
        glasm::p2c1_x2<24, 12>(LO(x[B + 4]), HI(x[B + 4]), LO(x[B + 5]), HI(x[B + 5]), ta0, tc0, LO(x[B + 10]), HI(x[B + 10]), LO(x[B + 11]), HI(x[B + 11]), ta1, tc1);
        x[B + 4] = tc0; x[B + 5] = ta0;
        x[B + 10] = ta1; x[B + 11] = tc1;
    }
    {
        uint64_t ta0, tc0, ta1, tc1, ta2, tc2;
        glasm::p2c2_x3<16, 28, 4>(LO(x[B + 2]), HI(x[B + 2]), LO(x[B + 3]), HI(x[B + 3]), ta0, tc0, LO(x[B + 8]), HI(x[B + 8]), LO(x[B + 9]), HI(x[B + 9]), ta1, tc1, LO(x[B + 14]), HI(x[B + 14]), LO(x[B + 15]), HI(x[B + 15]), ta2, tc2);
        x[B + 2] = ta0; x[B + 3] = tc0;
        x[B + 8] = tc1; x[B + 9] = ta1;
        x[B + 14] = tc2; x[B + 15] = ta2;
    }
    {
        uint64_t ta0, tc0, ta1, tc1;
        glasm::p2c3_x2<8, 20>(LO(x[B + 6]), HI(x[B + 6]), LO(x[B + 7]), HI(x[B + 7]), ta0, tc0, LO(x[B + 12]), HI(x[B + 12]), LO(x[B + 13]), HI(x[B + 13]), ta1, tc1);
        x[B + 6] = tc0; x[B + 7] = ta0;
        x[B + 12] = ta1; x[B + 13] = tc1;
    }
}

template <int B>
__device__ __forceinline__ void dft32_fwd(uint64_t* x) {
    {
        uint64_t ta0, tc0, ta1, tc1, ta2, tc2, ta3, tc3;
        glasm::p2c0_x4(LO(x[B + 0]), HI(x[B + 0]), LO(x[B + 16]), HI(x[B + 16]), ta0, tc0, LO(x[B + 1]), HI(x[B + 1]), LO(x[B + 17]), HI(x[B + 17]), ta1, tc1, LO(x[B + 2]), HI(x[B + 2]), LO(x[B + 18]), HI(x[B + 18]), ta2, tc2, LO(x[B + 3]), HI(x[B + 3]), LO(x[B + 19]), HI(x[B + 19]), ta3, tc3);
        x[B + 0] = ta0; x[B + 16] = tc0;
        x[B + 1] = ta1; x[B + 17] = tc1;
        x[B + 2] = ta2; x[B + 18] = tc2;
        x[B + 3] = ta3; x[B + 19] = tc3;
    }
    {
        uint64_t ta0, tc0, ta1, tc1, ta2, tc2, ta3, tc3;
        glasm::p2c0_x4(LO(x[B + 4]), HI(x[B + 4]), LO(x[B + 20]), HI(x[B + 20]), ta0, tc0, LO(x[B + 5]), HI(x[B + 5]), LO(x[B + 21]), HI(x[B + 21]), ta1, tc1, LO(x[B + 6]), HI(x[B + 6]), LO(x[B + 22]), HI(x[B + 22]), ta2, tc2, LO(x[B + 7]), HI(x[B + 7]), LO(x[B + 23]), HI(x[B + 23]), ta3, tc3);
        x[B + 4] = ta0; x[B + 20] = tc0;
        x[B + 5] = ta1; x[B + 21] = tc1;
        x[B + 6] = ta2; x[B + 22] = tc2;
        x[B + 7] = ta3; x[B + 23] = tc3;
    }
    {
        uint64_t ta0, tc0, ta1, tc1, ta2, tc2, ta3, tc3;
        glasm::p2c0_x4(LO(x[B + 8]), HI(x[B + 8]), LO(x[B + 24]), HI(x[B + 24]), ta0, tc0, LO(x[B + 9]), HI(x[B + 9]), LO(x[B + 25]), HI(x[B + 25]), ta1, tc1, LO(x[B + 10]), HI(x[B + 10]), LO(x[B + 26]), HI(x[B + 26]), ta2, tc2, LO(x[B + 11]), HI(x[B + 11]), LO(x[B + 27]), HI(x[B + 27]), ta3, tc3);
        x[B + 8] = ta0; x[B + 24] = tc0;
        x[B + 9] = ta1; x[B + 25] = tc1;
        x[B + 10] = ta2; x[B + 26] = tc2;
        x[B + 11] = ta3; x[B + 27] = tc3;
    }
    {
        uint64_t ta0, tc0, ta1, tc1, ta2, tc2, ta3, tc3;
        glasm::p2c0_x4(LO(x[B + 12]), HI(x[B + 12]), LO(x[B + 28]), HI(x[B + 28]), ta0, tc0, LO(x[B + 13]), HI(x[B + 13]), LO(x[B + 29]), HI(x[B + 29]), ta1, tc1, LO(x[B + 14]), HI(x[B + 14]), LO(x[B + 30]), HI(x[B + 30]), ta2, tc2, LO(x[B + 15]), HI(x[B + 15]), LO(x[B + 31]), HI(x[B + 31]), ta3, tc3);
        x[B + 12] = ta0; x[B + 28] = tc0;
        x[B + 13] = ta1; x[B + 29] = tc1;
        x[B + 14] = ta2; x[B + 30] = tc2;
        x[B + 15] = ta3; x[B + 31] = tc3;
    }
    {
        uint64_t ta0, tc0, ta1, tc1, ta2, tc2, ta3, tc3;
        glasm::p2c0_x4(LO(x[B + 0]), HI(x[B + 0]), LO(x[B + 8]), HI(x[B + 8]), ta0, tc0, LO(x[B + 1]), HI(x[B + 1]), LO(x[B + 9]), HI(x[B + 9]), ta1, tc1, LO(x[B + 2]), HI(x[B + 2]), LO(x[B + 10]), HI(x[B + 10]), ta2, tc2, LO(x[B + 3]), HI(x[B + 3]), LO(x[B + 11]), HI(x[B + 11]), ta3, tc3);
        x[B + 0] = ta0; x[B + 8] = tc0;
        x[B + 1] = ta1; x[B + 9] = tc1;
        x[B + 2] = ta2; x[B + 10] = tc2;
        x[B + 3] = ta3; x[B + 11] = tc3;
    }
    {
        uint64_t ta0, tc0, ta1, tc1, ta2, tc2, ta3, tc3;
        glasm::p2c0_x4(LO(x[B + 4]), HI(x[B + 4]), LO(x[B + 12]), HI(x[B + 12]), ta0, tc0, LO(x[B + 5]), HI(x[B + 5]), LO(x[B + 13]), HI(x[B + 13]), ta1, tc1, LO(x[B + 6]), HI(x[B + 6]), LO(x[B + 14]), HI(x[B + 14]), ta2, tc2, LO(x[B + 7]), HI(x[B + 7]), LO(x[B + 15]), HI(x[B + 15]), ta3, tc3);
        x[B + 4] = ta0; x[B + 12] = tc0;
        x[B + 5] = ta1; x[B + 13] = tc1;
        x[B + 6] = ta2; x[B + 14] = tc2;
        x[B + 7] = ta3; x[B + 15] = tc3;
    }
    {
        uint64_t ta0, tc0, ta1, tc1, ta2, tc2, ta3, tc3;
        glasm::p2c2_x4<16, 16, 16, 16>(LO(x[B + 16]), HI(x[B + 16]), LO(x[B + 24]), HI(x[B + 24]), ta0, tc0, LO(x[B + 17]), HI(x[B + 17]), LO(x[B + 25]), HI(x[B + 25]), ta1, tc1, LO(x[B + 18]), HI(x[B + 18]), LO(x[B + 26]), HI(x[B + 26]), ta2, tc2, LO(x[B + 19]), HI(x[B + 19]), LO(x[B + 27]), HI(x[B + 27]), ta3, tc3);
        x[B + 16] = ta0; x[B + 24] = tc0;
        x[B + 17] = ta1; x[B + 25] = tc1;
        x[B + 18] = ta2; x[B + 26] = tc2;
        x[B + 19] = ta3; x[B + 27] = tc3;
    }
    {
        uint64_t ta0, tc0, ta1, tc1, ta2, tc2, ta3, tc3;
        glasm::p2c2_x4<16, 16, 16, 16>(LO(x[B + 20]), HI(x[B + 20]), LO(x[B + 28]), HI(x[B + 28]), ta0, tc0, LO(x[B + 21]), HI(x[B + 21]), LO(x[B + 29]), HI(x[B + 29]), ta1, tc1, LO(x[B + 22]), HI(x[B + 22]), LO(x[B + 30]), HI(x[B + 30]), ta2, tc2, LO(x[B + 23]), HI(x[B + 23]), LO(x[B + 31]), HI(x[B + 31]), ta3, tc3);
        x[B + 20] = ta0; x[B + 28] = tc0;
        x[B + 21] = ta1; x[B + 29] = tc1;
        x[B + 22] = ta2; x[B + 30] = tc2;
        x[B + 23] = ta3; x[B + 31] = tc3;
    }
    {
        uint64_t ta0, tc0, ta1, tc1, ta2, tc2, ta3, tc3;
        glasm::p2c0_x4(LO(x[B + 0]), HI(x[B + 0]), LO(x[B + 4]), HI(x[B + 4]), ta0, tc0, LO(x[B + 1]), HI(x[B + 1]), LO(x[B + 5]), HI(x[B + 5]), ta1, tc1, LO(x[B + 2]), HI(x[B + 2]), LO(x[B + 6]), HI(x[B + 6]), ta2, tc2, LO(x[B + 3]), HI(x[B + 3]), LO(x[B + 7]), HI(x[B + 7]), ta3, tc3);
        x[B + 0] = ta0; x[B + 4] = tc0;
        x[B + 1] = ta1; x[B + 5] = tc1;
        x[B + 2] = ta2; x[B + 6] = tc2;
        x[B + 3] = ta3; x[B + 7] = tc3;
    }
    {
        uint64_t ta0, tc0, ta1, tc1, ta2, tc2, ta3, tc3;
        glasm::p2c1_x4<24, 24, 24, 24>(LO(x[B + 16]), HI(x[B + 16]), LO(x[B + 20]), HI(x[B + 20]), ta0, tc0, LO(x[B + 17]), HI(x[B + 17]), LO(x[B + 21]), HI(x[B + 21]), ta1, tc1, LO(x[B + 18]), HI(x[B + 18]), LO(x[B + 22]), HI(x[B + 22]), ta2, tc2, LO(x[B + 19]), HI(x[B + 19]), LO(x[B + 23]), HI(x[B + 23]), ta3, tc3);
        x[B + 16] = tc0; x[B + 20] = ta0;
        x[B + 17] = tc1; x[B + 21] = ta1;
        x[B + 18] = tc2; x[B + 22] = ta2;
        x[B + 19] = tc3; x[B + 23] = ta3;
    }
    {
        uint64_t ta0, tc0, ta1, tc1, ta2, tc2, ta3, tc3;
        glasm::p2c2_x4<16, 16, 16, 16>(LO(x[B + 8]), HI(x[B + 8]), LO(x[B + 12]), HI(x[B + 12]), ta0, tc0, LO(x[B + 9]), HI(x[B + 9]), LO(x[B + 13]), HI(x[B + 13]), ta1, tc1, LO(x[B + 10]), HI(x[B + 10]), LO(x[B + 14]), HI(x[B + 14]), ta2, tc2, LO(x[B + 11]), HI(x[B + 11]), LO(x[B + 15]), HI(x[B + 15]), ta3, tc3);
        x[B + 8] = ta0; x[B + 12] = tc0;
        x[B + 9] = ta1; x[B + 13] = tc1;
        x[B + 10] = ta2; x[B + 14] = tc2;
        x[B + 11] = ta3; x[B + 15] = tc3;
    }
    {
        uint64_t ta0, tc0, ta1, tc1, ta2, tc2, ta3, tc3;
        glasm::p2c3_x4<8, 8, 8, 8>(LO(x[B + 24]), HI(x[B + 24]), LO(x[B + 28]), HI(x[B + 28]), ta0, tc0, LO(x[B + 25]), HI(x[B + 25]), LO(x[B + 29]), HI(x[B + 29]), ta1, tc1, LO(x[B + 26]), HI(x[B + 26]), LO(x[B + 30]), HI(x[B + 30]), ta2, tc2, LO(x[B + 27]), HI(x[B + 27]), LO(x[B + 31]), HI(x[B + 31]), ta3, tc3);
        x[B + 24] = tc0; x[B + 28] = ta0;
        x[B + 25] = tc1; x[B + 29] = ta1;
        x[B + 26] = tc2; x[B + 30] = ta2;
        x[B + 27] = tc3; x[B + 31] = ta3;
    }
    {
        uint64_t ta0, tc0, ta1, tc1;
        glasm::p2c0_x2(LO(x[B + 0]), HI(x[B + 0]), LO(x[B + 2]), HI(x[B + 2]), ta0, tc0, LO(x[B + 1]), HI(x[B + 1]), LO(x[B + 3]), HI(x[B + 3]), ta1, tc1);
        x[B + 0] = ta0; x[B + 2] = tc0;
        x[B + 1] = ta1; x[B + 3] = tc1;
    }
    {
        uint64_t ta0, tc0, ta1, tc1, ta2, tc2, ta3, tc3;
        glasm::p2c1_x4<24, 24, 12, 12>(LO(x[B + 8]), HI(x[B + 8]), LO(x[B + 10]), HI(x[B + 10]), ta0, tc0, LO(x[B + 9]), HI(x[B + 9]), LO(x[B + 11]), HI(x[B + 11]), ta1, tc1, LO(x[B + 20]), HI(x[B + 20]), LO(x[B + 22]), HI(x[B + 22]), ta2, tc2, LO(x[B + 21]), HI(x[B + 21]), LO(x[B + 23]), HI(x[B + 23]), ta3, tc3);
        x[B + 8] = tc0; x[B + 10] = ta0;
        x[B + 9] = tc1; x[B + 11] = ta1;
        x[B + 20] = ta2; x[B + 22] = tc2;
        x[B + 21] = ta3; x[B + 23] = tc3;
    }
    {
        uint64_t ta0, tc0, ta1, tc1, ta2, tc2, ta3, tc3;
        glasm::p2c2_x4<16, 16, 28, 28>(LO(x[B + 4]), HI(x[B + 4]), LO(x[B + 6]), HI(x[B + 6]), ta0, tc0, LO(x[B + 5]), HI(x[B + 5]), LO(x[B + 7]), HI(x[B + 7]), ta1, tc1, LO(x[B + 16]), HI(x[B + 16]), LO(x[B + 18]), HI(x[B + 18]), ta2, tc2, LO(x[B + 17]), HI(x[B + 17]), LO(x[B + 19]), HI(x[B + 19]), ta3, tc3);
        x[B + 4] = ta0; x[B + 6] = tc0;
        x[B + 5] = ta1; x[B + 7] = tc1;
        x[B + 16] = tc2; x[B + 18] = ta2;
        x[B + 17] = tc3; x[B + 19] = ta3;
    }
    {
        uint64_t ta0, tc0, ta1, tc1;
        glasm::p2c2_x2<4, 4>(LO(x[B + 28]), HI(x[B + 28]), LO(x[B + 30]), HI(x[B + 30]), ta0, tc0, LO(x[B + 29]), HI(x[B + 29]), LO(x[B + 31]), HI(x[B + 31]), ta1, tc1);
        x[B + 28] = tc0; x[B + 30] = ta0;
        x[B + 29] = tc1; x[B + 31] = ta1;
    }
    {
        uint64_t ta0, tc0, ta1, tc1, ta2, tc2, ta3, tc3;
        glasm::p2c3_x4<8, 8, 20, 20>(LO(x[B + 12]), HI(x[B + 12]), LO(x[B + 14]), HI(x[B + 14]), ta0, tc0, LO(x[B + 13]), HI(x[B + 13]), LO(x[B + 15]), HI(x[B + 15]), ta1, tc1, LO(x[B + 24]), HI(x[B + 24]), LO(x[B + 26]), HI(x[B + 26]), ta2, tc2, LO(x[B + 25]), HI(x[B + 25]), LO(x[B + 27]), HI(x[B + 27]), ta3, tc3);
        x[B + 12] = tc0; x[B + 14] = ta0;
        x[B + 13] = tc1; x[B + 15] = ta1;
        x[B + 24] = ta2; x[B + 26] = tc2;
        x[B + 25] = ta3; x[B + 27] = tc3;
    }
    {
        uint64_t ta0, tc0;
        glasm::p2c0_x1(LO(x[B + 0]), HI(x[B + 0]), LO(x[B + 1]), HI(x[B + 1]), ta0, tc0);
        x[B + 0] = ta0; x[B + 1] = tc0;
    }
    {
        uint64_t ta0, tc0, ta1, tc1, ta2, tc2, ta3, tc3;
        glasm::p2c1_x4<24, 12, 30, 6>(LO(x[B + 4]), HI(x[B + 4]), LO(x[B + 5]), HI(x[B + 5]), ta0, tc0, LO(x[B + 10]), HI(x[B + 10]), LO(x[B + 11]), HI(x[B + 11]), ta1, tc1, LO(x[B + 18]), HI(x[B + 18]), LO(x[B + 19]), HI(x[B + 19]), ta2, tc2, LO(x[B + 20]), HI(x[B + 20]), LO(x[B + 21]), HI(x[B + 21]), ta3, tc3);
        x[B + 4] = tc0; x[B + 5] = ta0;
        x[B + 10] = ta1; x[B + 11] = tc1;
        x[B + 18] = tc2; x[B + 19] = ta2;
        x[B + 20] = ta3; x[B + 21] = tc3;
    }
    {
        uint64_t ta0, tc0;
        glasm::p2c1_x1<18>(LO(x[B + 30]), HI(x[B + 30]), LO(x[B + 31]), HI(x[B + 31]), ta0, tc0);
        x[B + 30] = ta0; x[B + 31] = tc0;
    }
    {
        uint64_t ta0, tc0, ta1, tc1, ta2, tc2, ta3, tc3;
        glasm::p2c2_x4<16, 28, 4, 22>(LO(x[B + 2]), HI(x[B + 2]), LO(x[B + 3]), HI(x[B + 3]), ta0, tc0, LO(x[B + 8]), HI(x[B + 8]), LO(x[B + 9]), HI(x[B + 9]), ta1, tc1, LO(x[B + 14]), HI(x[B + 14]), LO(x[B + 15]), HI(x[B + 15]), ta2, tc2, LO(x[B + 22]), HI(x[B + 22]), LO(x[B + 23]), HI(x[B + 23]), ta3, tc3);
        x[B + 2] = ta0; x[B + 3] = tc0;
        x[B + 8] = tc1; x[B + 9] = ta1;
        x[B + 14] = tc2; x[B + 15] = ta2;
        x[B + 22] = ta3; x[B + 23] = tc3;
    }
    {
        uint64_t ta0, tc0;
        glasm::p2c2_x1<10>(LO(x[B + 24]), HI(x[B + 24]), LO(x[B + 25]), HI(x[B + 25]), ta0, tc0);
        x[B + 24] = ta0; x[B + 25] = tc0;
    }
    {
        uint64_t ta0, tc0, ta1, tc1, ta2, tc2, ta3, tc3;
        glasm::p2c3_x4<8, 20, 14, 26>(LO(x[B + 6]), HI(x[B + 6]), LO(x[B + 7]), HI(x[B + 7]), ta0, tc0, LO(x[B + 12]), HI(x[B + 12]), LO(x[B + 13]), HI(x[B + 13]), ta1, tc1, LO(x[B + 16]), HI(x[B + 16]), LO(x[B + 17]), HI(x[B + 17]), ta2, tc2, LO(x[B + 26]), HI(x[B + 26]), LO(x[B + 27]), HI(x[B + 27]), ta3, tc3);
        x[B + 6] = tc0; x[B + 7] = ta0;
        x[B + 12] = ta1; x[B + 13] = tc1;
        x[B + 16] = ta2; x[B + 17] = tc2;
        x[B + 26] = ta3; x[B + 27] = tc3;
    }
    {
        uint64_t ta0, tc0;
        glasm::p2c3_x1<2>(LO(x[B + 28]), HI(x[B + 28]), LO(x[B + 29]), HI(x[B + 29]), ta0, tc0);
        x[B + 28] = tc0; x[B + 29] = ta0;
    }
}

template <int B>
__device__ __forceinline__ void dft2_inv(uint64_t* x) {
    {
        uint64_t ta0, tc0;
        glasm::p2c0_x1(LO(x[B + 0]), HI(x[B + 0]), LO(x[B + 1]), HI(x[B + 1]), ta0, tc0);
        x[B + 0] = ta0; x[B + 1] = tc0;
    }
}

template <int B>
__device__ __forceinline__ void dft4_inv(uint64_t* x) {
    {
        uint64_t ta0, tc0, ta1, tc1;
        glasm::p2c0_x2(LO(x[B + 0]), HI(x[B + 0]), LO(x[B + 2]), HI(x[B + 2]), ta0, tc0, LO(x[B + 1]), HI(x[B + 1]), LO(x[B + 3]), HI(x[B + 3]), ta1, tc1);
        x[B + 0] = ta0; x[B + 2] = tc0;
        x[B + 1] = ta1; x[B + 3] = tc1;
    }
    {
        uint64_t ta0, tc0;
        glasm::p2c0_x1(LO(x[B + 0]), HI(x[B + 0]), LO(x[B + 1]), HI(x[B + 1]), ta0, tc0);
        x[B + 0] = ta0; x[B + 1] = tc0;
    }
    {
        uint64_t ta0, tc0;
        glasm::p2c2_x1<16>(LO(x[B + 2]), HI(x[B + 2]), LO(x[B + 3]), HI(x[B + 3]), ta0, tc0);
        x[B + 2] = tc0; x[B + 3] = ta0;
    }
}

template <int B>
__device__ __forceinline__ void dft8_inv(uint64_t* x) {
    {
        uint64_t ta0, tc0, ta1, tc1, ta2, tc2, ta3, tc3;
        glasm::p2c0_x4(LO(x[B + 0]), HI(x[B + 0]), LO(x[B + 4]), HI(x[B + 4]), ta0, tc0, LO(x[B + 1]), HI(x[B + 1]), LO(x[B + 5]), HI(x[B + 5]), ta1, tc1, LO(x[B + 2]), HI(x[B + 2]), LO(x[B + 6]), HI(x[B + 6]), ta2, tc2, LO(x[B + 3]), HI(x[B + 3]), LO(x[B + 7]), HI(x[B + 7]), ta3, tc3);
        x[B + 0] = ta0; x[B + 4] = tc0;
        x[B + 1] = ta1; x[B + 5] = tc1;
        x[B + 2] = ta2; x[B + 6] = tc2;
        x[B + 3] = ta3; x[B + 7] = tc3;
    }
    {
        uint64_t ta0, tc0, ta1, tc1;
        glasm::p2c0_x2(LO(x[B + 0]), HI(x[B + 0]), LO(x[B + 2]), HI(x[B + 2]), ta0, tc0, LO(x[B + 1]), HI(x[B + 1]), LO(x[B + 3]), HI(x[B + 3]), ta1, tc1);
        x[B + 0] = ta0; x[B + 2] = tc0;
        x[B + 1] = ta1; x[B + 3] = tc1;
    }
    {
        uint64_t ta0, tc0, ta1, tc1;
        glasm::p2c2_x2<16, 16>(LO(x[B + 4]), HI(x[B + 4]), LO(x[B + 6]), HI(x[B + 6]), ta0, tc0, LO(x[B + 5]), HI(x[B + 5]), LO(x[B + 7]), HI(x[B + 7]), ta1, tc1);
        x[B + 4] = tc0; x[B + 6] = ta0;
        x[B + 5] = tc1; x[B + 7] = ta1;
    }
    {
        uint64_t ta0, tc0;
        glasm::p2c0_x1(LO(x[B + 0]), HI(x[B + 0]), LO(x[B + 1]), HI(x[B + 1]), ta0, tc0);
        x[B + 0] = ta0; x[B + 1] = tc0;
    }
    {
        uint64_t ta0, tc0;
        glasm::p2c1_x1<24>(LO(x[B + 6]), HI(x[B + 6]), LO(x[B + 7]), HI(x[B + 7]), ta0, tc0);
        x[B + 6] = ta0; x[B + 7] = tc0;
    }
    {
        uint64_t ta0, tc0;
        glasm::p2c2_x1<16>(LO(x[B + 2]), HI(x[B + 2]), LO(x[B + 3]), HI(x[B + 3]), ta0, tc0);
        x[B + 2] = tc0; x[B + 3] = ta0;
    }
    {
        uint64_t ta0, tc0;
        glasm::p2c3_x1<8>(LO(x[B + 4]), HI(x[B + 4]), LO(x[B + 5]), HI(x[B + 5]), ta0, tc0);
        x[B + 4] = ta0; x[B + 5] = tc0;
    }
}

template <int B>
__device__ __forceinline__ void dft16_inv(uint64_t* x) {
    {
        uint64_t ta0, tc0, ta1, tc1, ta2, tc2, ta3, tc3;
        glasm::p2c0_x4(LO(x[B + 0]), HI(x[B + 0]), LO(x[B + 8]), HI(x[B + 8]), ta0, tc0, LO(x[B + 1]), HI(x[B + 1]), LO(x[B + 9]), HI(x[B + 9]), ta1, tc1, LO(x[B + 2]), HI(x[B + 2]), LO(x[B + 10]), HI(x[B + 10]), ta2, tc2, LO(x[B + 3]), HI(x[B + 3]), LO(x[B + 11]), HI(x[B + 11]), ta3, tc3);
        x[B + 0] = ta0; x[B + 8] = tc0;
        x[B + 1] = ta1; x[B + 9] = tc1;
        x[B + 2] = ta2; x[B + 10] = tc2;
        x[B + 3] = ta3; x[B + 11] = tc3;
    }
    {
        uint64_t ta0, tc0, ta1, tc1, ta2, tc2, ta3, tc3;
        glasm::p2c0_x4(LO(x[B + 4]), HI(x[B + 4]), LO(x[B + 12]), HI(x[B + 12]), ta0, tc0, LO(x[B + 5]), HI(x[B + 5]), LO(x[B + 13]), HI(x[B + 13]), ta1, tc1, LO(x[B + 6]), HI(x[B + 6]), LO(x[B + 14]), HI(x[B + 14]), ta2, tc2, LO(x[B + 7]), HI(x[B + 7]), LO(x[B + 15]), HI(x[B + 15]), ta3, tc3);
        x[B + 4] = ta0; x[B + 12] = tc0;
        x[B + 5] = ta1; x[B + 13] = tc1;
        x[B + 6] = ta2; x[B + 14] = tc2;
        x[B + 7] = ta3; x[B + 15] = tc3;
    }
    {
        uint64_t ta0, tc0, ta1, tc1, ta2, tc2, ta3, tc3;
        glasm::p2c0_x4(LO(x[B + 0]), HI(x[B + 0]), LO(x[B + 4]), HI(x[B + 4]), ta0, tc0, LO(x[B + 1]), HI(x[B + 1]), LO(x[B + 5]), HI(x[B + 5]), ta1, tc1, LO(x[B + 2]), HI(x[B + 2]), LO(x[B + 6]), HI(x[B + 6]), ta2, tc2, LO(x[B + 3]), HI(x[B + 3]), LO(x[B + 7]), HI(x[B + 7]), ta3, tc3);
        x[B + 0] = ta0; x[B + 4] = tc0;
        x[B + 1] = ta1; x[B + 5] = tc1;
        x[B + 2] = ta2; x[B + 6] = tc2;
        x[B + 3] = ta3; x[B + 7] = tc3;
    }
    {
        uint64_t ta0, tc0, ta1, tc1, ta2, tc2, ta3, tc3;
        glasm::p2c2_x4<16, 16, 16, 16>(LO(x[B + 8]), HI(x[B + 8]), LO(x[B + 12]), HI(x[B + 12]), ta0, tc0, LO(x[B + 9]), HI(x[B + 9]), LO(x[B + 13]), HI(x[B + 13]), ta1, tc1, LO(x[B + 10]), HI(x[B + 10]), LO(x[B + 14]), HI(x[B + 14]), ta2, tc2, LO(x[B + 11]), HI(x[B + 11]), LO(x[B + 15]), HI(x[B + 15]), ta3, tc3);
        x[B + 8] = tc0; x[B + 12] = ta0;
        x[B + 9] = tc1; x[B + 13] = ta1;
        x[B + 10] = tc2; x[B + 14] = ta2;
        x[B + 11] = tc3; x[B + 15] = ta3;
    }
    {
        uint64_t ta0, tc0, ta1, tc1;
        glasm::p2c0_x2(LO(x[B + 0]), HI(x[B + 0]), LO(x[B + 2]), HI(x[B + 2]), ta0, tc0, LO(x[B + 1]), HI(x[B + 1]), LO(x[B + 3]), HI(x[B + 3]), ta1, tc1);
        x[B + 0] = ta0; x[B + 2] = tc0;
        x[B + 1] = ta1; x[B + 3] = tc1;
    }
    {
        uint64_t ta0, tc0, ta1, tc1;
        glasm::p2c1_x2<24, 24>(LO(x[B + 12]), HI(x[B + 12]), LO(x[B + 14]), HI(x[B + 14]), ta0, tc0, LO(x[B + 13]), HI(x[B + 13]), LO(x[B + 15]), HI(x[B + 15]), ta1, tc1);
        x[B + 12] = ta0; x[B + 14] = tc0;
        x[B + 13] = ta1; x[B + 15] = tc1;
    }
    {
        uint64_t ta0, tc0, ta1, tc1;
        glasm::p2c2_x2<16, 16>(LO(x[B + 4]), HI(x[B + 4]), LO(x[B + 6]), HI(x[B + 6]), ta0, tc0, LO(x[B + 5]), HI(x[B + 5]), LO(x[B + 7]), HI(x[B + 7]), ta1, tc1);
        x[B + 4] = tc0; x[B + 6] = ta0;
        x[B + 5] = tc1; x[B + 7] = ta1;
    }
    {
        uint64_t ta0, tc0, ta1, tc1;
        glasm::p2c3_x2<8, 8>(LO(x[B + 8]), HI(x[B + 8]), LO(x[B + 10]), HI(x[B + 10]), ta0, tc0, LO(x[B + 9]), HI(x[B + 9]), LO(x[B + 11]), HI(x[B + 11]), ta1, tc1);
        x[B + 8] = ta0; x[B + 10] = tc0;
        x[B + 9] = ta1; x[B + 11] = tc1;
    }
    {
        uint64_t ta0, tc0;
        glasm::p2c0_x1(LO(x[B + 0]), HI(x[B + 0]), LO(x[B + 1]), HI(x[B + 1]), ta0, tc0);
        x[B + 0] = ta0; x[B + 1] = tc0;
    }
    {
        uint64_t ta0, tc0, ta1, tc1;
        glasm::p2c1_x2<24, 12>(LO(x[B + 6]), HI(x[B + 6]), LO(x[B + 7]), HI(x[B + 7]), ta0, tc0, LO(x[B + 12]), HI(x[B + 12]), LO(x[B + 13]), HI(x[B + 13]), ta1, tc1);
        x[B + 6] = ta0; x[B + 7] = tc0;
        x[B + 12] = tc1; x[B + 13] = ta1;
    }
    {
        uint64_t ta0, tc0, ta1, tc1, ta2, tc2;
        glasm::p2c2_x3<16, 4, 28>(LO(x[B + 2]), HI(x[B + 2]), LO(x[B + 3]), HI(x[B + 3]), ta0, tc0, LO(x[B + 8]), HI(x[B + 8]), LO(x[B + 9]), HI(x[B + 9]), ta1, tc1, LO(x[B + 14]), HI(x[B + 14]), LO(x[B + 15]), HI(x[B + 15]), ta2, tc2);
        x[B + 2] = tc0; x[B + 3] = ta0;
        x[B + 8] = ta1; x[B + 9] = tc1;
        x[B + 14] = ta2; x[B + 15] = tc2;
    }
    {
        uint64_t ta0, tc0, ta1, tc1;
        glasm::p2c3_x2<8, 20>(LO(x[B + 4]), HI(x[B + 4]), LO(x[B + 5]), HI(x[B + 5]), ta0, tc0, LO(x[B + 10]), HI(x[B + 10]), LO(x[B + 11]), HI(x[B + 11]), ta1, tc1);
        x[B + 4] = ta0; x[B + 5] = tc0;
        x[B + 10] = tc1; x[B + 11] = ta1;
    }
}

template <int B>
__device__ __forceinline__ void dft32_inv(uint64_t* x) {
    {
        uint64_t ta0, tc0, ta1, tc1, ta2, tc2, ta3, tc3;
        glasm::p2c0_x4(LO(x[B + 0]), HI(x[B + 0]), LO(x[B + 16]), HI(x[B + 16]), ta0, tc0, LO(x[B + 1]), HI(x[B + 1]), LO(x[B + 17]), HI(x[B + 17]), ta1, tc1, LO(x[B + 2]), HI(x[B + 2]), LO(x[B + 18]), HI(x[B + 18]), ta2, tc2, LO(x[B + 3]), HI(x[B + 3]), LO(x[B + 19]), HI(x[B + 19]), ta3, tc3);
        x[B + 0] = ta0; x[B + 16] = tc0;
        x[B + 1] = ta1; x[B + 17] = tc1;
        x[B + 2] = ta2; x[B + 18] = tc2;
        x[B + 3] = ta3; x[B + 19] = tc3;
    }
    {
        uint64_t ta0, tc0, ta1, tc1, ta2, tc2, ta3, tc3;
        glasm::p2c0_x4(LO(x[B + 4]), HI(x[B + 4]), LO(x[B + 20]), HI(x[B + 20]), ta0, tc0, LO(x[B + 5]), HI(x[B + 5]), LO(x[B + 21]), HI(x[B + 21]), ta1, tc1, LO(x[B + 6]), HI(x[B + 6]), LO(x[B + 22]), HI(x[B + 22]), ta2, tc2, LO(x[B + 7]), HI(x[B + 7]), LO(x[B + 23]), HI(x[B + 23]), ta3, tc3);
        x[B + 4] = ta0; x[B + 20] = tc0;
        x[B + 5] = ta1; x[B + 21] = tc1;
        x[B + 6] = ta2; x[B + 22] = tc2;
        x[B + 7] = ta3; x[B + 23] = tc3;
    }
    {
        uint64_t ta0, tc0, ta1, tc1, ta2, tc2, ta3, tc3;
        glasm::p2c0_x4(LO(x[B + 8]), HI(x[B + 8]), LO(x[B + 24]), HI(x[B + 24]), ta0, tc0, LO(x[B + 9]), HI(x[B + 9]), LO(x[B + 25]), HI(x[B + 25]), ta1, tc1, LO(x[B + 10]), HI(x[B + 10]), LO(x[B + 26]), HI(x[B + 26]), ta2, tc2, LO(x[B + 11]), HI(x[B + 11]), LO(x[B + 27]), HI(x[B + 27]), ta3, tc3);
        x[B + 8] = ta0; x[B + 24] = tc0;
        x[B + 9] = ta1; x[B + 25] = tc1;
        x[B + 10] = ta2; x[B + 26] = tc2;
        x[B + 11] = ta3; x[B + 27] = tc3;
    }
    {
        uint64_t ta0, tc0, ta1, tc1, ta2, tc2, ta3, tc3;
        glasm::p2c0_x4(LO(x[B + 12]), HI(x[B + 12]), LO(x[B + 28]), HI(x[B + 28]), ta0, tc0, LO(x[B + 13]), HI(x[B + 13]), LO(x[B + 29]), HI(x[B + 29]), ta1, tc1, LO(x[B + 14]), HI(x[B + 14]), LO(x[B + 30]), HI(x[B + 30]), ta2, tc2, LO(x[B + 15]), HI(x[B + 15]), LO(x[B + 31]), HI(x[B + 31]), ta3, tc3);
        x[B + 12] = ta0; x[B + 28] = tc0;
        x[B + 13] = ta1; x[B + 29] = tc1;
        x[B + 14] = ta2; x[B + 30] = tc2;
        x[B + 15] = ta3; x[B + 31] = tc3;
    }
    {
        uint64_t ta0, tc0, ta1, tc1, ta2, tc2, ta3, tc3;
        glasm::p2c0_x4(LO(x[B + 0]), HI(x[B + 0]), LO(x[B + 8]), HI(x[B + 8]), ta0, tc0, LO(x[B + 1]), HI(x[B + 1]), LO(x[B + 9]), HI(x[B + 9]), ta1, tc1, LO(x[B + 2]), HI(x[B + 2]), LO(x[B + 10]), HI(x[B + 10]), ta2, tc2, LO(x[B + 3]), HI(x[B + 3]), LO(x[B + 11]), HI(x[B + 11]), ta3, tc3);
        x[B + 0] = ta0; x[B + 8] = tc0;
        x[B + 1] = ta1; x[B + 9] = tc1;
        x[B + 2] = ta2; x[B + 10] = tc2;
        x[B + 3] = ta3; x[B + 11] = tc3;
    }
    {
        uint64_t ta0, tc0, ta1, tc1, ta2, tc2, ta3, tc3;
        glasm::p2c0_x4(LO(x[B + 4]), HI(x[B + 4]), LO(x[B + 12]), HI(x[B + 12]), ta0, tc0, LO(x[B + 5]), HI(x[B + 5]), LO(x[B + 13]), HI(x[B + 13]), ta1, tc1, LO(x[B + 6]), HI(x[B + 6]), LO(x[B + 14]), HI(x[B + 14]), ta2, tc2, LO(x[B + 7]), HI(x[B + 7]), LO(x[B + 15]), HI(x[B + 15]), ta3, tc3);
        x[B + 4] = ta0; x[B + 12] = tc0;
        x[B + 5] = ta1; x[B + 13] = tc1;
        x[B + 6] = ta2; x[B + 14] = tc2;
        x[B + 7] = ta3; x[B + 15] = tc3;
    }
    {
        uint64_t ta0, tc0, ta1, tc1, ta2, tc2, ta3, tc3;
        glasm::p2c2_x4<16, 16, 16, 16>(LO(x[B + 16]), HI(x[B + 16]), LO(x[B + 24]), HI(x[B + 24]), ta0, tc0, LO(x[B + 17]), HI(x[B + 17]), LO(x[B + 25]), HI(x[B + 25]), ta1, tc1, LO(x[B + 18]), HI(x[B + 18]), LO(x[B + 26]), HI(x[B + 26]), ta2, tc2, LO(x[B + 19]), HI(x[B + 19]), LO(x[B + 27]), HI(x[B + 27]), ta3, tc3);
        x[B + 16] = tc0; x[B + 24] = ta0;
        x[B + 17] = tc1; x[B + 25] = ta1;
        x[B + 18] = tc2; x[B + 26] = ta2;
        x[B + 19] = tc3; x[B + 27] = ta3;
    }
    {
        uint64_t ta0, tc0, ta1, tc1, ta2, tc2, ta3, tc3;
        glasm::p2c2_x4<16, 16, 16, 16>(LO(x[B + 20]), HI(x[B + 20]), LO(x[B + 28]), HI(x[B + 28]), ta0, tc0, LO(x[B + 21]), HI(x[B + 21]), LO(x[B + 29]), HI(x[B + 29]), ta1, tc1, LO(x[B + 22]), HI(x[B + 22]), LO(x[B + 30]), HI(x[B + 30]), ta2, tc2, LO(x[B + 23]), HI(x[B + 23]), LO(x[B + 31]), HI(x[B + 31]), ta3, tc3);
        x[B + 20] = tc0; x[B + 28] = ta0;
        x[B + 21] = tc1; x[B + 29] = ta1;
        x[B + 22] = tc2; x[B + 30] = ta2;
        x[B + 23] = tc3; x[B + 31] = ta3;
    }
    {
        uint64_t ta0, tc0, ta1, tc1, ta2, tc2, ta3, tc3;
        glasm::p2c0_x4(LO(x[B + 0]), HI(x[B + 0]), LO(x[B + 4]), HI(x[B + 4]), ta0, tc0, LO(x[B + 1]), HI(x[B + 1]), LO(x[B + 5]), HI(x[B + 5]), ta1, tc1, LO(x[B + 2]), HI(x[B + 2]), LO(x[B + 6]), HI(x[B + 6]), ta2, tc2, LO(x[B + 3]), HI(x[B + 3]), LO(x[B + 7]), HI(x[B + 7]), ta3, tc3);
        x[B + 0] = ta0; x[B + 4] = tc0;
        x[B + 1] = ta1; x[B + 5] = tc1;
        x[B + 2] = ta2; x[B + 6] = tc2;
        x[B + 3] = ta3; x[B + 7] = tc3;
    }
    {
        uint64_t ta0, tc0, ta1, tc1, ta2, tc2, ta3, tc3;
        glasm::p2c1_x4<24, 24, 24, 24>(LO(x[B + 24]), HI(x[B + 24]), LO(x[B + 28]), HI(x[B + 28]), ta0, tc0, LO(x[B + 25]), HI(x[B + 25]), LO(x[B + 29]), HI(x[B + 29]), ta1, tc1, LO(x[B + 26]), HI(x[B + 26]), LO(x[B + 30]), HI(x[B + 30]), ta2, tc2, LO(x[B + 27]), HI(x[B + 27]), LO(x[B + 31]), HI(x[B + 31]), ta3, tc3);
        x[B + 24] = ta0; x[B + 28] = tc0;
        x[B + 25] = ta1; x[B + 29] = tc1;
        x[B + 26] = ta2; x[B + 30] = tc2;
        x[B + 27] = ta3; x[B + 31] = tc3;
    }
    {
        uint64_t ta0, tc0, ta1, tc1, ta2, tc2, ta3, tc3;
        glasm::p2c2_x4<16, 16, 16, 16>(LO(x[B + 8]), HI(x[B + 8]), LO(x[B + 12]), HI(x[B + 12]), ta0, tc0, LO(x[B + 9]), HI(x[B + 9]), LO(x[B + 13]), HI(x[B + 13]), ta1, tc1, LO(x[B + 10]), HI(x[B + 10]), LO(x[B + 14]), HI(x[B + 14]), ta2, tc2, LO(x[B + 11]), HI(x[B + 11]), LO(x[B + 15]), HI(x[B + 15]), ta3, tc3);
        x[B + 8] = tc0; x[B + 12] = ta0;
        x[B + 9] = tc1; x[B + 13] = ta1;
        x[B + 10] = tc2; x[B + 14] = ta2;
        x[B + 11] = tc3; x[B + 15] = ta3;
    }
    {
        uint64_t ta0, tc0, ta1, tc1, ta2, tc2, ta3, tc3;
        glasm::p2c3_x4<8, 8, 8, 8>(LO(x[B + 16]), HI(x[B + 16]), LO(x[B + 20]), HI(x[B + 20]), ta0, tc0, LO(x[B + 17]), HI(x[B + 17]), LO(x[B + 21]), HI(x[B + 21]), ta1, tc1, LO(x[B + 18]), HI(x[B + 18]), LO(x[B + 22]), HI(x[B + 22]), ta2, tc2, LO(x[B + 19]), HI(x[B + 19]), LO(x[B + 23]), HI(x[B + 23]), ta3, tc3);
        x[B + 16] = ta0; x[B + 20] = tc0;
        x[B + 17] = ta1; x[B + 21] = tc1;
        x[B + 18] = ta2; x[B + 22] = tc2;
        x[B + 19] = ta3; x[B + 23] = tc3;
    }
    {
        uint64_t ta0, tc0, ta1, tc1;
        glasm::p2c0_x2(LO(x[B + 0]), HI(x[B + 0]), LO(x[B + 2]), HI(x[B + 2]), ta0, tc0, LO(x[B + 1]), HI(x[B + 1]), LO(x[B + 3]), HI(x[B + 3]), ta1, tc1);
        x[B + 0] = ta0; x[B + 2] = tc0;
        x[B + 1] = ta1; x[B + 3] = tc1;
    }
    {
        uint64_t ta0, tc0, ta1, tc1, ta2, tc2, ta3, tc3;
        glasm::p2c1_x4<24, 24, 12, 12>(LO(x[B + 12]), HI(x[B + 12]), LO(x[B + 14]), HI(x[B + 14]), ta0, tc0, LO(x[B + 13]), HI(x[B + 13]), LO(x[B + 15]), HI(x[B + 15]), ta1, tc1, LO(x[B + 24]), HI(x[B + 24]), LO(x[B + 26]), HI(x[B + 26]), ta2, tc2, LO(x[B + 25]), HI(x[B + 25]), LO(x[B + 27]), HI(x[B + 27]), ta3, tc3);
        x[B + 12] = ta0; x[B + 14] = tc0;
        x[B + 13] = ta1; x[B + 15] = tc1;
        x[B + 24] = tc2; x[B + 26] = ta2;
        x[B + 25] = tc3; x[B + 27] = ta3;
    }
    {
        uint64_t ta0, tc0, ta1, tc1, ta2, tc2, ta3, tc3;
        glasm::p2c2_x4<16, 16, 4, 4>(LO(x[B + 4]), HI(x[B + 4]), LO(x[B + 6]), HI(x[B + 6]), ta0, tc0, LO(x[B + 5]), HI(x[B + 5]), LO(x[B + 7]), HI(x[B + 7]), ta1, tc1, LO(x[B + 16]), HI(x[B + 16]), LO(x[B + 18]), HI(x[B + 18]), ta2, tc2, LO(x[B + 17]), HI(x[B + 17]), LO(x[B + 19]), HI(x[B + 19]), ta3, tc3);
        x[B + 4] = tc0; x[B + 6] = ta0;
        x[B + 5] = tc1; x[B + 7] = ta1;
        x[B + 16] = ta2; x[B + 18] = tc2;
        x[B + 17] = ta3; x[B + 19] = tc3;
    }
    {
        uint64_t ta0, tc0, ta1, tc1;
        glasm::p2c2_x2<28, 28>(LO(x[B + 28]), HI(x[B + 28]), LO(x[B + 30]), HI(x[B + 30]), ta0, tc0, LO(x[B + 29]), HI(x[B + 29]), LO(x[B + 31]), HI(x[B + 31]), ta1, tc1);
        x[B + 28] = ta0; x[B + 30] = tc0;
        x[B + 29] = ta1; x[B + 31] = tc1;
    }
    {
        uint64_t ta0, tc0, ta1, tc1, ta2, tc2, ta3, tc3;
        glasm::p2c3_x4<8, 8, 20, 20>(LO(x[B + 8]), HI(x[B + 8]), LO(x[B + 10]), HI(x[B + 10]), ta0, tc0, LO(x[B + 9]), HI(x[B + 9]), LO(x[B + 11]), HI(x[B + 11]), ta1, tc1, LO(x[B + 20]), HI(x[B + 20]), LO(x[B + 22]), HI(x[B + 22]), ta2, tc2, LO(x[B + 21]), HI(x[B + 21]), LO(x[B + 23]), HI(x[B + 23]), ta3, tc3);
        x[B + 8] = ta0; x[B + 10] = tc0;
        x[B + 9] = ta1; x[B + 11] = tc1;
        x[B + 20] = tc2; x[B + 22] = ta2;
        x[B + 21] = tc3; x[B + 23] = ta3;
    }
    {
        uint64_t ta0, tc0;
        glasm::p2c0_x1(LO(x[B + 0]), HI(x[B + 0]), LO(x[B + 1]), HI(x[B + 1]), ta0, tc0);
        x[B + 0] = ta0; x[B + 1] = tc0;
    }
    {
        uint64_t ta0, tc0, ta1, tc1, ta2, tc2, ta3, tc3;
        glasm::p2c1_x4<24, 12, 18, 6>(LO(x[B + 6]), HI(x[B + 6]), LO(x[B + 7]), HI(x[B + 7]), ta0, tc0, LO(x[B + 12]), HI(x[B + 12]), LO(x[B + 13]), HI(x[B + 13]), ta1, tc1, LO(x[B + 16]), HI(x[B + 16]), LO(x[B + 17]), HI(x[B + 17]), ta2, tc2, LO(x[B + 26]), HI(x[B + 26]), LO(x[B + 27]), HI(x[B + 27]), ta3, tc3);
        x[B + 6] = ta0; x[B + 7] = tc0;
        x[B + 12] = tc1; x[B + 13] = ta1;
        x[B + 16] = tc2; x[B + 17] = ta2;
        x[B + 26] = tc3; x[B + 27] = ta3;
    }
    {
        uint64_t ta0, tc0;
        glasm::p2c1_x1<30>(LO(x[B + 28]), HI(x[B + 28]), LO(x[B + 29]), HI(x[B + 29]), ta0, tc0);
        x[B + 28] = ta0; x[B + 29] = tc0;
    }
    {
        uint64_t ta0, tc0, ta1, tc1, ta2, tc2, ta3, tc3;
        glasm::p2c2_x4<16, 4, 28, 10>(LO(x[B + 2]), HI(x[B + 2]), LO(x[B + 3]), HI(x[B + 3]), ta0, tc0, LO(x[B + 8]), HI(x[B + 8]), LO(x[B + 9]), HI(x[B + 9]), ta1, tc1, LO(x[B + 14]), HI(x[B + 14]), LO(x[B + 15]), HI(x[B + 15]), ta2, tc2, LO(x[B + 22]), HI(x[B + 22]), LO(x[B + 23]), HI(x[B + 23]), ta3, tc3);
        x[B + 2] = tc0; x[B + 3] = ta0;
        x[B + 8] = ta1; x[B + 9] = tc1;
        x[B + 14] = ta2; x[B + 15] = tc2;
        x[B + 22] = tc3; x[B + 23] = ta3;
    }
    {
        uint64_t ta0, tc0;
        glasm::p2c2_x1<22>(LO(x[B + 24]), HI(x[B + 24]), LO(x[B + 25]), HI(x[B + 25]), ta0, tc0);
        x[B + 24] = tc0; x[B + 25] = ta0;
    }
    {
        uint64_t ta0, tc0, ta1, tc1, ta2, tc2, ta3, tc3;
        glasm::p2c3_x4<8, 20, 2, 26>(LO(x[B + 4]), HI(x[B + 4]), LO(x[B + 5]), HI(x[B + 5]), ta0, tc0, LO(x[B + 10]), HI(x[B + 10]), LO(x[B + 11]), HI(x[B + 11]), ta1, tc1, LO(x[B + 18]), HI(x[B + 18]), LO(x[B + 19]), HI(x[B + 19]), ta2, tc2, LO(x[B + 20]), HI(x[B + 20]), LO(x[B + 21]), HI(x[B + 21]), ta3, tc3);
        x[B + 4] = ta0; x[B + 5] = tc0;
        x[B + 10] = tc1; x[B + 11] = ta1;
        x[B + 18] = ta2; x[B + 19] = tc2;
        x[B + 20] = tc3; x[B + 21] = ta3;
    }
    {
        uint64_t ta0, tc0;
        glasm::p2c3_x1<14>(LO(x[B + 30]), HI(x[B + 30]), LO(x[B + 31]), HI(x[B + 31]), ta0, tc0);
        x[B + 30] = tc0; x[B + 31] = ta0;
    }
}

#undef LO
#undef HI
}
}
```

Before: 5.900 billion elems/s.

## Fuse twiddle prescale with first two radix-2 stages via lazy radix-4 asm

Replaces the separate per-element prescale multiply followed by a full 32-point DFT with a hand-written asm radix-4 group. That group multiplies four elements by their factors, uses lazy (not fully reduced) products, and performs the first two butterfly stages in one block. The remaining stages run through new dft32_*_from2 routines that start after those two stages. Twiddle-factor loads are regrouped to match the radix-4 access pattern. This aims to cut reductions and instructions in the NTT inner kernels, at the cost of a large hand-coded asm block with many clobbered registers that may raise register pressure.

```diff
diff --git a/era-boojum_amd/csrc/ntt_ct_common.hpp b/era-boojum_amd/csrc/ntt_ct_common.hpp
--- a/era-boojum_amd/csrc/ntt_ct_common.hpp
+++ b/era-boojum_amd/csrc/ntt_ct_common.hpp
@@ -97,6 +97,38 @@
     }
 }
 
+template <bool INV>
+__device__ __forceinline__ void lazy_r4_group(uint64_t* y, int k, uint64_t xa, uint64_t xb, uint64_t xc, uint64_t xd,
+                                              uint64_t fa, uint64_t fb, uint64_t fc, uint64_t fd) {
+    uint64_t z0, z1, z2, z3;
+    if constexpr (INV)
+        glasm::lazy_r4_inv((uint32_t)xa, (uint32_t)(xa >> 32), (uint32_t)fa, (uint32_t)(fa >> 32), (uint32_t)xb,
+                           (uint32_t)(xb >> 32), (uint32_t)fb, (uint32_t)(fb >> 32), (uint32_t)xc, (uint32_t)(xc >> 32),
+                           (uint32_t)fc, (uint32_t)(fc >> 32), (uint32_t)xd, (uint32_t)(xd >> 32), (uint32_t)fd,
+                           (uint32_t)(fd >> 32), z0, z1, z2, z3);
+    else
+        glasm::lazy_r4_fwd((uint32_t)xa, (uint32_t)(xa >> 32), (uint32_t)fa, (uint32_t)(fa >> 32), (uint32_t)xb,
+                           (uint32_t)(xb >> 32), (uint32_t)fb, (uint32_t)(fb >> 32), (uint32_t)xc, (uint32_t)(xc >> 32),
+                           (uint32_t)fc, (uint32_t)(fc >> 32), (uint32_t)xd, (uint32_t)(xd >> 32), (uint32_t)fd,
+                           (uint32_t)(fd >> 32), z0, z1, z2, z3);
+    y[k] = z0;
+    y[k + 8] = z1;
+    y[k + 16] = z2;
+    y[k + 24] = z3;
+}
+
+template <bool INV, int K0, int K1>
+__device__ __forceinline__ void lazy_head32(uint64_t* x, const uint64_t* f) {
+#pragma unroll
+    for (int k = K0; k < K1; k++)
+        lazy_r4_group<INV>(x, k, x[k], x[k + 8], x[k + 16], x[k + 24], f[k], f[k + 8], f[k + 16], f[k + 24]);
+}
+
+template <bool INV>
+__device__ __forceinline__ void dft32_tail(uint64_t* x) {
+    if constexpr (INV) p2dft::dft32_inv_from2<0>(x); else p2dft::dft32_fwd_from2<0>(x);
+}
+
 __device__ __forceinline__ void load32(uint64_t* r, const uint64_t* __restrict__ f) {
 #pragma unroll
     for (int k = 0; k < PT; k++) r[k] = f[k];
diff --git a/era-boojum_amd/csrc/ntt_lde3.hip b/era-boojum_amd/csrc/ntt_lde3.hip
--- a/era-boojum_amd/csrc/ntt_lde3.hip
+++ b/era-boojum_amd/csrc/ntt_lde3.hip
@@ -27,19 +27,19 @@
     return bits == 0 ? 0u : (__builtin_bitreverse32(x) >> (32 - bits));
 }
 
-__device__ __forceinline__ void prescale32_brev(uint64_t* y, const uint64_t* x, const uint64_t* f) {
-#pragma unroll
-    for (int k = 0; k < PT; k += 4) {
-        uint32_t z0[4], z1[4];
-        const uint64_t a0 = x[cbrev(k, 5)], a1 = x[cbrev(k + 1, 5)], a2 = x[cbrev(k + 2, 5)], a3 = x[cbrev(k + 3, 5)];
-        glasm::mul_x4((uint32_t)a0, (uint32_t)(a0 >> 32), (uint32_t)f[k], (uint32_t)(f[k] >> 32), z0[0], z1[0],
-                      (uint32_t)a1, (uint32_t)(a1 >> 32), (uint32_t)f[k + 1], (uint32_t)(f[k + 1] >> 32), z0[1], z1[1],
-                      (uint32_t)a2, (uint32_t)(a2 >> 32), (uint32_t)f[k + 2], (uint32_t)(f[k + 2] >> 32), z0[2], z1[2],
-                      (uint32_t)a3, (uint32_t)(a3 >> 32), (uint32_t)f[k + 3], (uint32_t)(f[k + 3] >> 32), z0[3],
-                      z1[3]);
-#pragma unroll
-        for (int i = 0; i < 4; i++) y[k + i] = join2(z0[i], z1[i]);
-    }
+template <int K0, int K1>
+__device__ __forceinline__ void load_groups(uint64_t* f, const uint64_t* __restrict__ t) {
+#pragma unroll
+    for (int r = 0; r < 4; r++)
+#pragma unroll
+        for (int k = K0; k < K1; k++) f[8 * r + k] = t[8 * r + k];
+}
+
+__device__ __forceinline__ void lazy_head32_brev(uint64_t* y, const uint64_t* x, const uint64_t* f) {
+#pragma unroll
+    for (int k = 0; k < 8; k++)
+        lazy_r4_group<false>(y, k, x[cbrev(k, 5)], x[cbrev(k + 8, 5)], x[cbrev(k + 16, 5)], x[cbrev(k + 24, 5)], f[k],
+                             f[k + 8], f[k + 16], f[k + 24]);
 }
 
 __device__ __forceinline__ __amdgpu_buffer_rsrc_t uniform_rsrc(const uint64_t* p, uint32_t bytes) {
@@ -58,23 +58,19 @@
 }
 __device__ __forceinline__ uint64_t from_u32x2(u32x2 v) { return ((uint64_t)v.y << 32) | v.x; }
 
-__device__ __forceinline__ void prescale32_brev_uniform(uint64_t* y, const uint64_t* x, const uint64_t* __restrict__ h) {
-#pragma unroll
-    for (int k8 = 0; k8 < PT; k8 += 8) {
-        uint64_t hf[8];
-#pragma unroll
-        for (int i = 0; i < 8; i++) hf[i] = h[k8 + i];
-#pragma unroll
-        for (int k = k8; k < k8 + 8; k += 4) {
-            uint32_t z0[4], z1[4];
-            const uint64_t a0 = x[cbrev(k, 5)], a1 = x[cbrev(k + 1, 5)], a2 = x[cbrev(k + 2, 5)], a3 = x[cbrev(k + 3, 5)];
-            const uint64_t f0 = hf[k - k8], f1 = hf[k - k8 + 1], f2 = hf[k - k8 + 2], f3 = hf[k - k8 + 3];
-            glasm::mul_sb_x4((uint32_t)a0, (uint32_t)(a0 >> 32), (uint32_t)f0, (uint32_t)(f0 >> 32), z0[0], z1[0],
-                             (uint32_t)a1, (uint32_t)(a1 >> 32), (uint32_t)f1, (uint32_t)(f1 >> 32), z0[1], z1[1],
-                             (uint32_t)a2, (uint32_t)(a2 >> 32), (uint32_t)f2, (uint32_t)(f2 >> 32), z0[2], z1[2],
-                             (uint32_t)a3, (uint32_t)(a3 >> 32), (uint32_t)f3, (uint32_t)(f3 >> 32), z0[3], z1[3]);
-#pragma unroll
-            for (int i = 0; i < 4; i++) y[k + i] = join2(z0[i], z1[i]);
+__device__ __forceinline__ void lazy_head32_brev_uniform(uint64_t* y, const uint64_t* x, const uint64_t* __restrict__ h) {
+#pragma unroll
+    for (int k4 = 0; k4 < 8; k4 += 4) {
+        uint64_t hf[4][4];
+#pragma unroll
+        for (int r = 0; r < 4; r++)
+#pragma unroll
+            for (int i = 0; i < 4; i++) hf[r][i] = h[8 * r + k4 + i];
+#pragma unroll
+        for (int i = 0; i < 4; i++) {
+            const int k = k4 + i;
+            lazy_r4_group<false>(y, k, x[cbrev(k, 5)], x[cbrev(k + 8, 5)], x[cbrev(k + 16, 5)], x[cbrev(k + 24, 5)],
+                                 hf[0][i], hf[1][i], hf[2][i], hf[3][i]);
         }
     }
 }
@@ -116,27 +112,24 @@
     const uint64_t* ext = inv_tab + ((size_t)1 << LOGN);
     uint64_t f[PT], wa[16], wb[16], wc[16];
     load32(f, ext + EXT_TA + (size_t)q * 32);
-    prescale32(x, f);
-    dft_p2<5, true, 0>(x);
+    lazy_head32<true, 0, 8>(x, f);
+    dft32_tail<true>(x);
     const uint32_t tlo = t & 7, thi = t >> 3;
     const uint32_t bb = tail_base_b(thi, tlo);
 #pragma unroll
     for (int k = 0; k < PT; k++) lds[ba + tail_off_a(k)] = x[k];
     const uint64_t* tb = ext + ext_tb(R) + ((((size_t)q << 5) | thi) << 5);
-#pragma unroll
-    for (int k = 0; k < 16; k++) f[k] = tb[k];
+    load_groups<0, 4>(f, tb);
     __syncthreads();
 #pragma unroll
     for (int k = 0; k < PT; k++) x[k] = lds[bb + tail_off_b(k)];
-    prescale_n<8>(x, f);
-#pragma unroll
-    for (int k = 16; k < 24; k++) f[k] = tb[k];
-    prescale_n<8>(x + 8, f + 8);
-#pragma unroll
-    for (int k = 24; k < PT; k++) f[k] = tb[k];
-    prescale_n<8>(x + 16, f + 16);
-    prescale_n<8>(x + 24, f + 24);
-    dft_p2<5, true, 0>(x);
+    lazy_head32<true, 0, 2>(x, f);
+    load_groups<4, 6>(f, tb);
+    lazy_head32<true, 2, 4>(x, f);
+    load_groups<6, 8>(f, tb);
+    lazy_head32<true, 4, 6>(x, f);
+    lazy_head32<true, 6, 8>(x, f);
+    dft32_tail<true>(x);
     tw_ct_tailC<10>(wa, inv_tab, R, q, t);
 #pragma unroll
     for (int k = 0; k < PT; k++) lds[bb + tail_off_b(k)] = x[k];
@@ -206,26 +199,23 @@
     for (uint32_t i = 0; i < n_cosets; i++) {
         const uint64_t* tab = tabs + (size_t)i * tab_stride;
         uint64_t y[PT], f[PT];
-        prescale32_brev_uniform(y, x, tab + L3_HA);
-        dft_p2<5, false, 0>(y);
+        lazy_head32_brev_uniform(y, x, tab + L3_HA);
+        dft32_tail<false>(y);
         __syncthreads();
 #pragma unroll
         for (int k = 0; k < PT; k++) lds[b1 + cbrev(k, 5)] = y[k];
         const uint64_t* hb = tab + L3_HB + 32 * g5;
-#pragma unroll
-        for (int k = 0; k < 16; k++) f[k] = hb[k];
+        load_groups<0, 4>(f, hb);
         __syncthreads();
 #pragma unroll
         for (int k = 0; k < PT; k++) y[k] = lds[b2 + 33 * cbrev(k, 5)];
-        prescale_n<8>(y, f);
-#pragma unroll
-        for (int k = 16; k < 24; k++) f[k] = hb[k];
-        prescale_n<8>(y + 8, f + 8);
-#pragma unroll
-        for (int k = 24; k < PT; k++) f[k] = hb[k];
-        prescale_n<8>(y + 16, f + 16);
-        prescale_n<8>(y + 24, f + 24);
-        dft_p2<5, false, 0>(y);
+        lazy_head32<false, 0, 2>(y, f);
+        load_groups<4, 6>(f, hb);
+        lazy_head32<false, 2, 4>(y, f);
+        load_groups<6, 8>(f, hb);
+        lazy_head32<false, 4, 6>(y, f);
+        lazy_head32<false, 6, 8>(y, f);
+        dft32_tail<false>(y);
 #pragma unroll
         for (int k = 0; k < PT; k++) lds[b2 + 33 * cbrev(k, 5)] = y[k];
         const uint64_t* fc = tab + L3_C + 32 * t;
@@ -490,8 +480,8 @@
 #pragma unroll
         for (int k = 0; k < PT; k++) f[k] = f1[(size_t)k << 13];
     }
-    prescale32_brev(y, x, f);
-    dft_p2<5, false, 0>(y);
+    lazy_head32_brev(y, x, f);
+    dft32_tail<false>(y);
     const uint32_t b1 = fin_p1<R>(t, 0);
 #pragma unroll
     for (int k = 0; k < PT; k++) lds[b1 + (fin_p1<R>(0, k) - fin_p1<R>(0, 0))] = y[k];
diff --git a/era-boojum_amd/csrc/ntt_pow2.hpp b/era-boojum_amd/csrc/ntt_pow2.hpp
--- a/era-boojum_amd/csrc/ntt_pow2.hpp
+++ b/era-boojum_amd/csrc/ntt_pow2.hpp
@@ -979,6 +979,218 @@
         : "v0", "v1", "v2", "v3", "v4", "v5", "v6", "v7", "v8", "v9", "v10", "v11", "v12", "v13", "v14", "v15", "v16", "v17", "v18", "v19", "v20", "v21", "v22", "v23", "v24", "v25", "v26", "v27", "v28", "v29", "v30", "v31", "v32", "v33", "v34", "v35", "v36", "v37", "v38", "v39", "v40");
 }
 
+__device__ __forceinline__ void lazy_r4_fwd(uint32_t a00, uint32_t a10, uint32_t b00, uint32_t b10, uint32_t a01, uint32_t a11, uint32_t b01, uint32_t b11, uint32_t a02, uint32_t a12, uint32_t b02, uint32_t b12, uint32_t a03, uint32_t a13, uint32_t b03, uint32_t b13, uint64_t& z0, uint64_t& z1, uint64_t& z2, uint64_t& z3) {
+    uint64_t q40, q42, q44, q46, q48, q50, q52, q54, q56, q58, q60, q62, q64;
+    asm volatile(
+        "v_mov_b32 v33, 9\n"
+        "v_mov_b32 v35, 3\n"
+        "v_mov_b32 v37, 0\n"
+        "v_mov_b32 v39, 0\n"
+        "v_mad_u64_u32 v[2:3], %[q64], %[a10], %[b00], %[cU0]\n"
+        "v_mad_u64_u32 v[10:11], %[q64], %[a11], %[b01], %[cU1]\n"
+        "v_mad_u64_u32 v[18:19], %[q64], %[a12], %[b02], %[cU2]\n"
+        "v_mad_u64_u32 v[26:27], %[q64], %[a13], %[b03], %[cU3]\n"
+        "v_mad_u64_u32 v[0:1], %[q64], %[a00], %[b00], %[cP0]\n"
+        "v_mad_u64_u32 v[8:9], %[q64], %[a01], %[b01], %[cP1]\n"
+        "v_mad_u64_u32 v[16:17], %[q64], %[a02], %[b02], %[cP2]\n"
+        "v_mad_u64_u32 v[24:25], %[q64], %[a03], %[b03], %[cP3]\n"
+        "v_mad_u64_u32 v[4:5], %[q44], %[a00], %[b10], v[2:3]\n"
+        "v_mad_u64_u32 v[12:13], %[q50], %[a01], %[b11], v[10:11]\n"
+        "v_mad_u64_u32 v[20:21], %[q56], %[a02], %[b12], v[18:19]\n"
+        "v_mad_u64_u32 v[28:29], %[q62], %[a03], %[b13], v[26:27]\n"
+        "v_mad_u64_u32 v[6:7], %[q64], %[a10], %[b10], 0\n"
+        "v_mad_u64_u32 v[14:15], %[q64], %[a11], %[b11], 0\n"
+        "v_mad_u64_u32 v[22:23], %[q64], %[a12], %[b12], 0\n"
+        "v_mad_u64_u32 v[30:31], %[q64], %[a13], %[b13], 0\n"
+        "v_add_co_u32 v1, %[q40], v1, v4\n"
+        "v_add_co_u32 v9, %[q46], v9, v12\n"
+        "v_add_co_u32 v17, %[q52], v17, v20\n"
+        "v_add_co_u32 v25, %[q58], v25, v28\n"
+        "v_addc_co_u32 v7, %[q64], v7, 0, %[q44]\n"
+        "v_addc_co_u32 v15, %[q64], v15, 0, %[q50]\n"
+        "v_addc_co_u32 v23, %[q64], v23, 0, %[q56]\n"
+        "v_addc_co_u32 v31, %[q64], v31, 0, %[q62]\n"
+        "v_addc_co_u32 v32, %[q42], v5, v6, %[q40]\n"
+        "v_addc_co_u32 v34, %[q48], v13, v14, %[q46]\n"
+        "v_mad_u64_u32 v[4:5], %[q64], v1, 1, v[32:33]\n"
+        "v_mad_u64_u32 v[12:13], %[q64], v9, 1, v[34:35]\n"
+        "v_not_b32 v32, v32\n"
+        "v_not_b32 v34, v34\n"
+        "v_subb_co_u32 v2, %[q64], -1, v7, %[q42]\n"
+        "v_subb_co_u32 v10, %[q64], -1, v15, %[q48]\n"
+        "v_mad_u64_u32 v[6:7], %[q64], v0, 1, v[32:33]\n"
+        "v_mad_u64_u32 v[14:15], %[q64], v8, 1, v[34:35]\n"
+        "v_mad_u64_u32 v[6:7], %[q64], v2, 1, v[6:7]\n"
+        "v_mad_u64_u32 v[14:15], %[q64], v10, 1, v[14:15]\n"
+        "v_addc_co_u32 v36, %[q54], v21, v22, %[q52]\n"
+        "v_addc_co_u32 v38, %[q60], v29, v30, %[q58]\n"
+        "v_mad_u64_u32 v[20:21], %[q64], v17, 1, v[36:37]\n"
+        "v_mad_u64_u32 v[28:29], %[q64], v25, 1, v[38:39]\n"
+        "v_not_b32 v36, v36\n"
+        "v_not_b32 v38, v38\n"
+        "v_subb_co_u32 v18, %[q64], -1, v23, %[q54]\n"
+        "v_subb_co_u32 v26, %[q64], -1, v31, %[q60]\n"
+        "v_mad_u64_u32 v[22:23], %[q64], v16, 1, v[36:37]\n"
+        "v_mad_u64_u32 v[30:31], %[q64], v24, 1, v[38:39]\n"
+        "v_mad_u64_u32 v[22:23], %[q64], v18, 1, v[22:23]\n"
+        "v_mad_u64_u32 v[30:31], %[q64], v26, 1, v[30:31]\n"
+        "v_lshl_add_u64 v[0:1], v[6:7], 0, v[22:23]\n"
+        "v_sub_co_u32 v16, %[q40], v6, v22\n"
+        "v_lshl_add_u64 v[8:9], v[14:15], 0, v[30:31]\n"
+        "v_sub_co_u32 v24, %[q42], v14, v30\n"
+        "v_lshl_add_u64 v[2:3], v[4:5], 0, v[20:21]\n"
+        "v_subb_co_u32 v17, %[q64], v7, v23, %[q40]\n"
+        "v_lshl_add_u64 v[10:11], v[12:13], 0, v[28:29]\n"
+        "v_subb_co_u32 v25, %[q64], v15, v31, %[q42]\n"
+        "v_sub_co_u32 v18, %[q40], v4, v20\n"
+        "v_sub_co_u32 v26, %[q42], v12, v28\n"
+        "s_nop 0\n"
+        "v_subb_co_u32 v19, %[q64], v5, v21, %[q40]\n"
+        "v_subb_co_u32 v27, %[q64], v13, v29, %[q42]\n"
+        "v_lshl_add_u64 v[4:5], v[0:1], 0, v[8:9]\n"
+        "v_sub_co_u32 v12, %[q40], v0, v8\n"
+        "v_lshlrev_b64 v[30:31], 16, v[26:27]\n"
+        "v_lshl_add_u64 v[28:29], v[24:25], 0, v[26:27]\n"
+        "v_lshl_add_u64 v[6:7], v[2:3], 0, v[10:11]\n"
+        "v_subb_co_u32 v13, %[q64], v1, v9, %[q40]\n"
+        "v_lshl_add_u64 v[20:21], v[16:17], 0, v[30:31]\n"
+        "v_lshlrev_b64 v[28:29], 16, v[28:29]\n"
+        "v_sub_co_u32 v14, %[q40], v2, v10\n"
+        "v_not_b32 v30, v30\n"
+        "v_lshl_add_u64 v[22:23], v[18:19], 0, v[28:29]\n"
+        "v_subb_co_u32 v15, %[q64], v3, v11, %[q40]\n"
+        "v_xor_b32 v31, 0x7ffff, v31\n"
+        "v_not_b32 v28, v28\n"
+        "v_lshl_add_u64 v[16:17], v[16:17], 0, v[30:31]\n"
+        "v_xor_b32 v29, 0xfffff, v29\n"
+        "v_lshl_add_u64 v[18:19], v[18:19], 0, v[28:29]\n"
+        "v_mad_u64_u32 v[0:1], %[q64], v7, -1, v[4:5]\n"
+        "v_mad_u64_u32 v[8:9], %[q64], v15, -1, v[12:13]\n"
+        "v_mad_u64_u32 v[24:25], %[q64], v23, -1, v[16:17]\n"
+        "v_mad_u64_u32 v[28:29], %[q64], v19, -1, v[20:21]\n"
+        "v_add_co_u32 v1, %[q40], v1, v6\n"
+        "v_add_co_u32 v9, %[q42], v9, v14\n"
+        "v_add_co_u32 v25, %[q44], v25, v22\n"
+        "v_add_co_u32 v29, %[q46], v29, v18\n"
+        "v_cndmask_b32_e64 v2, 0, -1, %[q40]\n"
+        "v_cndmask_b32_e64 v10, 0, -1, %[q42]\n"
+        "v_cndmask_b32_e64 v26, 0, -1, %[q44]\n"
+        "v_cndmask_b32_e64 v30, 0, -1, %[q46]\n"
+        "v_mad_u64_u32 %[z0], %[q64], v2, 1, v[0:1]\n"
+        "v_mad_u64_u32 %[z1], %[q64], v10, 1, v[8:9]\n"
+        "v_mad_u64_u32 %[z2], %[q64], v26, 1, v[24:25]\n"
+        "v_mad_u64_u32 %[z3], %[q64], v30, 1, v[28:29]\n"
+        : [z0] "=&v"(z0), [z1] "=&v"(z1), [z2] "=&v"(z2), [z3] "=&v"(z3), [q40] "=&s"(q40), [q42] "=&s"(q42), [q44] "=&s"(q44), [q46] "=&s"(q46), [q48] "=&s"(q48), [q50] "=&s"(q50), [q52] "=&s"(q52), [q54] "=&s"(q54), [q56] "=&s"(q56), [q58] "=&s"(q58), [q60] "=&s"(q60), [q62] "=&s"(q62), [q64] "=&s"(q64)
+        : [a00] "v"(a00), [a10] "v"(a10), [b00] "v"(b00), [b10] "v"(b10), [cP0] "s"((uint64_t)0x8004000cull), [cU0] "s"((uint64_t)0xbff9ffebull), [a01] "v"(a01), [a11] "v"(a11), [b01] "v"(b01), [b11] "v"(b11), [cP1] "s"((uint64_t)0xffffc004ull), [cU1] "s"((uint64_t)0xfffffffaull), [a02] "v"(a02), [a12] "v"(a12), [b02] "v"(b02), [b12] "v"(b12), [cP2] "s"((uint64_t)0x7ffc0002ull), [cU2] "s"((uint64_t)0x4005fffdull), [a03] "v"(a03), [a13] "v"(a13), [b03] "v"(b03), [b13] "v"(b13), [cP3] "s"((uint64_t)0x4005ull), [cU3] "s"((uint64_t)0xfffffff9ull)
+        : "v0", "v1", "v2", "v3", "v4", "v5", "v6", "v7", "v8", "v9", "v10", "v11", "v12", "v13", "v14", "v15", "v16", "v17", "v18", "v19", "v20", "v21", "v22", "v23", "v24", "v25", "v26", "v27", "v28", "v29", "v30", "v31", "v32", "v33", "v34", "v35", "v36", "v37", "v38", "v39");
+}
+
+__device__ __forceinline__ void lazy_r4_inv(uint32_t a00, uint32_t a10, uint32_t b00, uint32_t b10, uint32_t a01, uint32_t a11, uint32_t b01, uint32_t b11, uint32_t a02, uint32_t a12, uint32_t b02, uint32_t b12, uint32_t a03, uint32_t a13, uint32_t b03, uint32_t b13, uint64_t& z0, uint64_t& z1, uint64_t& z2, uint64_t& z3) {
+    uint64_t q40, q42, q44, q46, q48, q50, q52, q54, q56, q58, q60, q62, q64;
+    asm volatile(
+        "v_mov_b32 v33, 9\n"
+        "v_mov_b32 v35, 3\n"
+        "v_mov_b32 v37, 0\n"
+        "v_mov_b32 v39, 0\n"
+        "v_mad_u64_u32 v[2:3], %[q64], %[a10], %[b00], %[cU0]\n"
+        "v_mad_u64_u32 v[10:11], %[q64], %[a11], %[b01], %[cU1]\n"
+        "v_mad_u64_u32 v[18:19], %[q64], %[a12], %[b02], %[cU2]\n"
+        "v_mad_u64_u32 v[26:27], %[q64], %[a13], %[b03], %[cU3]\n"
+        "v_mad_u64_u32 v[0:1], %[q64], %[a00], %[b00], %[cP0]\n"
+        "v_mad_u64_u32 v[8:9], %[q64], %[a01], %[b01], %[cP1]\n"
+        "v_mad_u64_u32 v[16:17], %[q64], %[a02], %[b02], %[cP2]\n"
+        "v_mad_u64_u32 v[24:25], %[q64], %[a03], %[b03], %[cP3]\n"
+        "v_mad_u64_u32 v[4:5], %[q44], %[a00], %[b10], v[2:3]\n"
+        "v_mad_u64_u32 v[12:13], %[q50], %[a01], %[b11], v[10:11]\n"
+        "v_mad_u64_u32 v[20:21], %[q56], %[a02], %[b12], v[18:19]\n"
+        "v_mad_u64_u32 v[28:29], %[q62], %[a03], %[b13], v[26:27]\n"
+        "v_mad_u64_u32 v[6:7], %[q64], %[a10], %[b10], 0\n"
+        "v_mad_u64_u32 v[14:15], %[q64], %[a11], %[b11], 0\n"
+        "v_mad_u64_u32 v[22:23], %[q64], %[a12], %[b12], 0\n"
+        "v_mad_u64_u32 v[30:31], %[q64], %[a13], %[b13], 0\n"
+        "v_add_co_u32 v1, %[q40], v1, v4\n"
+        "v_add_co_u32 v9, %[q46], v9, v12\n"
+        "v_add_co_u32 v17, %[q52], v17, v20\n"
+        "v_add_co_u32 v25, %[q58], v25, v28\n"
+        "v_addc_co_u32 v7, %[q64], v7, 0, %[q44]\n"
+        "v_addc_co_u32 v15, %[q64], v15, 0, %[q50]\n"
+        "v_addc_co_u32 v23, %[q64], v23, 0, %[q56]\n"
+        "v_addc_co_u32 v31, %[q64], v31, 0, %[q62]\n"
+        "v_addc_co_u32 v32, %[q42], v5, v6, %[q40]\n"
+        "v_addc_co_u32 v34, %[q48], v13, v14, %[q46]\n"
+        "v_mad_u64_u32 v[4:5], %[q64], v1, 1, v[32:33]\n"
+        "v_mad_u64_u32 v[12:13], %[q64], v9, 1, v[34:35]\n"
+        "v_not_b32 v32, v32\n"
+        "v_not_b32 v34, v34\n"
+        "v_subb_co_u32 v2, %[q64], -1, v7, %[q42]\n"
+        "v_subb_co_u32 v10, %[q64], -1, v15, %[q48]\n"
+        "v_mad_u64_u32 v[6:7], %[q64], v0, 1, v[32:33]\n"
+        "v_mad_u64_u32 v[14:15], %[q64], v8, 1, v[34:35]\n"
+        "v_mad_u64_u32 v[6:7], %[q64], v2, 1, v[6:7]\n"
+        "v_mad_u64_u32 v[14:15], %[q64], v10, 1, v[14:15]\n"
+        "v_addc_co_u32 v36, %[q54], v21, v22, %[q52]\n"
+        "v_addc_co_u32 v38, %[q60], v29, v30, %[q58]\n"
+        "v_mad_u64_u32 v[20:21], %[q64], v17, 1, v[36:37]\n"
+        "v_mad_u64_u32 v[28:29], %[q64], v25, 1, v[38:39]\n"
+        "v_not_b32 v36, v36\n"
+        "v_not_b32 v38, v38\n"
+        "v_subb_co_u32 v18, %[q64], -1, v23, %[q54]\n"
+        "v_subb_co_u32 v26, %[q64], -1, v31, %[q60]\n"
+        "v_mad_u64_u32 v[22:23], %[q64], v16, 1, v[36:37]\n"
+        "v_mad_u64_u32 v[30:31], %[q64], v24, 1, v[38:39]\n"
+        "v_mad_u64_u32 v[22:23], %[q64], v18, 1, v[22:23]\n"
+        "v_mad_u64_u32 v[30:31], %[q64], v26, 1, v[30:31]\n"
+        "v_lshl_add_u64 v[0:1], v[6:7], 0, v[22:23]\n"
+        "v_sub_co_u32 v16, %[q40], v6, v22\n"
+        "v_lshl_add_u64 v[8:9], v[14:15], 0, v[30:31]\n"
+        "v_sub_co_u32 v24, %[q42], v14, v30\n"
+        "v_lshl_add_u64 v[2:3], v[4:5], 0, v[20:21]\n"
+        "v_subb_co_u32 v17, %[q64], v7, v23, %[q40]\n"
+        "v_lshl_add_u64 v[10:11], v[12:13], 0, v[28:29]\n"
+        "v_subb_co_u32 v25, %[q64], v15, v31, %[q42]\n"
+        "v_sub_co_u32 v18, %[q40], v4, v20\n"
+        "v_sub_co_u32 v26, %[q42], v12, v28\n"
+        "s_nop 0\n"
+        "v_subb_co_u32 v19, %[q64], v5, v21, %[q40]\n"
+        "v_subb_co_u32 v27, %[q64], v13, v29, %[q42]\n"
+        "v_lshl_add_u64 v[4:5], v[0:1], 0, v[8:9]\n"
+        "v_sub_co_u32 v12, %[q40], v0, v8\n"
+        "v_lshlrev_b64 v[30:31], 16, v[26:27]\n"
+        "v_lshl_add_u64 v[28:29], v[24:25], 0, v[26:27]\n"
+        "v_lshl_add_u64 v[6:7], v[2:3], 0, v[10:11]\n"
+        "v_subb_co_u32 v13, %[q64], v1, v9, %[q40]\n"
+        "v_lshl_add_u64 v[20:21], v[16:17], 0, v[30:31]\n"
+        "v_lshlrev_b64 v[28:29], 16, v[28:29]\n"
+        "v_sub_co_u32 v14, %[q40], v2, v10\n"
+        "v_not_b32 v30, v30\n"
+        "v_lshl_add_u64 v[22:23], v[18:19], 0, v[28:29]\n"
+        "v_subb_co_u32 v15, %[q64], v3, v11, %[q40]\n"
+        "v_xor_b32 v31, 0x7ffff, v31\n"
+        "v_not_b32 v28, v28\n"
+        "v_lshl_add_u64 v[16:17], v[16:17], 0, v[30:31]\n"
+        "v_xor_b32 v29, 0xfffff, v29\n"
+        "v_lshl_add_u64 v[18:19], v[18:19], 0, v[28:29]\n"
+        "v_mad_u64_u32 v[0:1], %[q64], v7, -1, v[4:5]\n"
+        "v_mad_u64_u32 v[8:9], %[q64], v15, -1, v[12:13]\n"
+        "v_mad_u64_u32 v[24:25], %[q64], v23, -1, v[16:17]\n"
+        "v_mad_u64_u32 v[28:29], %[q64], v19, -1, v[20:21]\n"
+        "v_add_co_u32 v1, %[q40], v1, v6\n"
+        "v_add_co_u32 v9, %[q42], v9, v14\n"
+        "v_add_co_u32 v25, %[q44], v25, v22\n"
+        "v_add_co_u32 v29, %[q46], v29, v18\n"
+        "v_cndmask_b32_e64 v2, 0, -1, %[q40]\n"
+        "v_cndmask_b32_e64 v10, 0, -1, %[q42]\n"
+        "v_cndmask_b32_e64 v26, 0, -1, %[q44]\n"
+        "v_cndmask_b32_e64 v30, 0, -1, %[q46]\n"
+        "v_mad_u64_u32 %[z0], %[q64], v2, 1, v[0:1]\n"
+        "v_mad_u64_u32 %[z1], %[q64], v10, 1, v[8:9]\n"
+        "v_mad_u64_u32 %[z3], %[q64], v26, 1, v[24:25]\n"
+        "v_mad_u64_u32 %[z2], %[q64], v30, 1, v[28:29]\n"
+        : [z0] "=&v"(z0), [z1] "=&v"(z1), [z2] "=&v"(z2), [z3] "=&v"(z3), [q40] "=&s"(q40), [q42] "=&s"(q42), [q44] "=&s"(q44), [q46] "=&s"(q46), [q48] "=&s"(q48), [q50] "=&s"(q50), [q52] "=&s"(q52), [q54] "=&s"(q54), [q56] "=&s"(q56), [q58] "=&s"(q58), [q60] "=&s"(q60), [q62] "=&s"(q62), [q64] "=&s"(q64)
+        : [a00] "v"(a00), [a10] "v"(a10), [b00] "v"(b00), [b10] "v"(b10), [cP0] "s"((uint64_t)0x8004000cull), [cU0] "s"((uint64_t)0xbff9ffebull), [a01] "v"(a01), [a11] "v"(a11), [b01] "v"(b01), [b11] "v"(b11), [cP1] "s"((uint64_t)0xffffc004ull), [cU1] "s"((uint64_t)0xfffffffaull), [a02] "v"(a02), [a12] "v"(a12), [b02] "v"(b02), [b12] "v"(b12), [cP2] "s"((uint64_t)0x7ffc0002ull), [cU2] "s"((uint64_t)0x4005fffdull), [a03] "v"(a03), [a13] "v"(a13), [b03] "v"(b03), [b13] "v"(b13), [cP3] "s"((uint64_t)0x4005ull), [cU3] "s"((uint64_t)0xfffffff9ull)
+        : "v0", "v1", "v2", "v3", "v4", "v5", "v6", "v7", "v8", "v9", "v10", "v11", "v12", "v13", "v14", "v15", "v16", "v17", "v18", "v19", "v20", "v21", "v22", "v23", "v24", "v25", "v26", "v27", "v28", "v29", "v30", "v31", "v32", "v33", "v34", "v35", "v36", "v37", "v38", "v39");
+}
+
 }
 
 namespace bj {
@@ -1324,36 +1536,7 @@
 }
 
 template <int B>
-__device__ __forceinline__ void dft2_inv(uint64_t* x) {
-    {
-        uint64_t ta0, tc0;
-        glasm::p2c0_x1(LO(x[B + 0]), HI(x[B + 0]), LO(x[B + 1]), HI(x[B + 1]), ta0, tc0);
-        x[B + 0] = ta0; x[B + 1] = tc0;
-    }
-}
-
-template <int B>
-__device__ __forceinline__ void dft4_inv(uint64_t* x) {
-    {
-        uint64_t ta0, tc0, ta1, tc1;
-        glasm::p2c0_x2(LO(x[B + 0]), HI(x[B + 0]), LO(x[B + 2]), HI(x[B + 2]), ta0, tc0, LO(x[B + 1]), HI(x[B + 1]), LO(x[B + 3]), HI(x[B + 3]), ta1, tc1);
-        x[B + 0] = ta0; x[B + 2] = tc0;
-        x[B + 1] = ta1; x[B + 3] = tc1;
-    }
-    {
-        uint64_t ta0, tc0;
-        glasm::p2c0_x1(LO(x[B + 0]), HI(x[B + 0]), LO(x[B + 1]), HI(x[B + 1]), ta0, tc0);
-        x[B + 0] = ta0; x[B + 1] = tc0;
-    }
-    {
-        uint64_t ta0, tc0;
-        glasm::p2c2_x1<16>(LO(x[B + 2]), HI(x[B + 2]), LO(x[B + 3]), HI(x[B + 3]), ta0, tc0);
-        x[B + 2] = tc0; x[B + 3] = ta0;
-    }
-}
-
-template <int B>
-__device__ __forceinline__ void dft8_inv(uint64_t* x) {
+__device__ __forceinline__ void dft32_fwd_from2(uint64_t* x) {
     {
         uint64_t ta0, tc0, ta1, tc1, ta2, tc2, ta3, tc3;
         glasm::p2c0_x4(LO(x[B + 0]), HI(x[B + 0]), LO(x[B + 4]), HI(x[B + 4]), ta0, tc0, LO(x[B + 1]), HI(x[B + 1]), LO(x[B + 5]), HI(x[B + 5]), ta1, tc1, LO(x[B + 2]), HI(x[B + 2]), LO(x[B + 6]), HI(x[B + 6]), ta2, tc2, LO(x[B + 3]), HI(x[B + 3]), LO(x[B + 7]), HI(x[B + 7]), ta3, tc3);
@@ -1363,6 +1546,151 @@
         x[B + 3] = ta3; x[B + 7] = tc3;
     }
     {
+        uint64_t ta0, tc0, ta1, tc1, ta2, tc2, ta3, tc3;
+        glasm::p2c1_x4<24, 24, 24, 24>(LO(x[B + 16]), HI(x[B + 16]), LO(x[B + 20]), HI(x[B + 20]), ta0, tc0, LO(x[B + 17]), HI(x[B + 17]), LO(x[B + 21]), HI(x[B + 21]), ta1, tc1, LO(x[B + 18]), HI(x[B + 18]), LO(x[B + 22]), HI(x[B + 22]), ta2, tc2, LO(x[B + 19]), HI(x[B + 19]), LO(x[B + 23]), HI(x[B + 23]), ta3, tc3);
+        x[B + 16] = tc0; x[B + 20] = ta0;
+        x[B + 17] = tc1; x[B + 21] = ta1;
+        x[B + 18] = tc2; x[B + 22] = ta2;
+        x[B + 19] = tc3; x[B + 23] = ta3;
+    }
+    {
+        uint64_t ta0, tc0, ta1, tc1, ta2, tc2, ta3, tc3;
+        glasm::p2c2_x4<16, 16, 16, 16>(LO(x[B + 8]), HI(x[B + 8]), LO(x[B + 12]), HI(x[B + 12]), ta0, tc0, LO(x[B + 9]), HI(x[B + 9]), LO(x[B + 13]), HI(x[B + 13]), ta1, tc1, LO(x[B + 10]), HI(x[B + 10]), LO(x[B + 14]), HI(x[B + 14]), ta2, tc2, LO(x[B + 11]), HI(x[B + 11]), LO(x[B + 15]), HI(x[B + 15]), ta3, tc3);
+        x[B + 8] = ta0; x[B + 12] = tc0;
+        x[B + 9] = ta1; x[B + 13] = tc1;
+        x[B + 10] = ta2; x[B + 14] = tc2;
+        x[B + 11] = ta3; x[B + 15] = tc3;
+    }
+    {
+        uint64_t ta0, tc0, ta1, tc1, ta2, tc2, ta3, tc3;
+        glasm::p2c3_x4<8, 8, 8, 8>(LO(x[B + 24]), HI(x[B + 24]), LO(x[B + 28]), HI(x[B + 28]), ta0, tc0, LO(x[B + 25]), HI(x[B + 25]), LO(x[B + 29]), HI(x[B + 29]), ta1, tc1, LO(x[B + 26]), HI(x[B + 26]), LO(x[B + 30]), HI(x[B + 30]), ta2, tc2, LO(x[B + 27]), HI(x[B + 27]), LO(x[B + 31]), HI(x[B + 31]), ta3, tc3);
+        x[B + 24] = tc0; x[B + 28] = ta0;
+        x[B + 25] = tc1; x[B + 29] = ta1;
+        x[B + 26] = tc2; x[B + 30] = ta2;
+        x[B + 27] = tc3; x[B + 31] = ta3;
+    }
+    {
+        uint64_t ta0, tc0, ta1, tc1;
+        glasm::p2c0_x2(LO(x[B + 0]), HI(x[B + 0]), LO(x[B + 2]), HI(x[B + 2]), ta0, tc0, LO(x[B + 1]), HI(x[B + 1]), LO(x[B + 3]), HI(x[B + 3]), ta1, tc1);
+        x[B + 0] = ta0; x[B + 2] = tc0;
+        x[B + 1] = ta1; x[B + 3] = tc1;
+    }
+    {
+        uint64_t ta0, tc0, ta1, tc1, ta2, tc2, ta3, tc3;
+        glasm::p2c1_x4<24, 24, 12, 12>(LO(x[B + 8]), HI(x[B + 8]), LO(x[B + 10]), HI(x[B + 10]), ta0, tc0, LO(x[B + 9]), HI(x[B + 9]), LO(x[B + 11]), HI(x[B + 11]), ta1, tc1, LO(x[B + 20]), HI(x[B + 20]), LO(x[B + 22]), HI(x[B + 22]), ta2, tc2, LO(x[B + 21]), HI(x[B + 21]), LO(x[B + 23]), HI(x[B + 23]), ta3, tc3);
+        x[B + 8] = tc0; x[B + 10] = ta0;
+        x[B + 9] = tc1; x[B + 11] = ta1;
+        x[B + 20] = ta2; x[B + 22] = tc2;
+        x[B + 21] = ta3; x[B + 23] = tc3;
+    }
+    {
+        uint64_t ta0, tc0, ta1, tc1, ta2, tc2, ta3, tc3;
+        glasm::p2c2_x4<16, 16, 28, 28>(LO(x[B + 4]), HI(x[B + 4]), LO(x[B + 6]), HI(x[B + 6]), ta0, tc0, LO(x[B + 5]), HI(x[B + 5]), LO(x[B + 7]), HI(x[B + 7]), ta1, tc1, LO(x[B + 16]), HI(x[B + 16]), LO(x[B + 18]), HI(x[B + 18]), ta2, tc2, LO(x[B + 17]), HI(x[B + 17]), LO(x[B + 19]), HI(x[B + 19]), ta3, tc3);
+        x[B + 4] = ta0; x[B + 6] = tc0;
+        x[B + 5] = ta1; x[B + 7] = tc1;
+        x[B + 16] = tc2; x[B + 18] = ta2;
+        x[B + 17] = tc3; x[B + 19] = ta3;
+    }
+    {
+        uint64_t ta0, tc0, ta1, tc1;
+        glasm::p2c2_x2<4, 4>(LO(x[B + 28]), HI(x[B + 28]), LO(x[B + 30]), HI(x[B + 30]), ta0, tc0, LO(x[B + 29]), HI(x[B + 29]), LO(x[B + 31]), HI(x[B + 31]), ta1, tc1);
+        x[B + 28] = tc0; x[B + 30] = ta0;
+        x[B + 29] = tc1; x[B + 31] = ta1;
+    }
+    {
+        uint64_t ta0, tc0, ta1, tc1, ta2, tc2, ta3, tc3;
+        glasm::p2c3_x4<8, 8, 20, 20>(LO(x[B + 12]), HI(x[B + 12]), LO(x[B + 14]), HI(x[B + 14]), ta0, tc0, LO(x[B + 13]), HI(x[B + 13]), LO(x[B + 15]), HI(x[B + 15]), ta1, tc1, LO(x[B + 24]), HI(x[B + 24]), LO(x[B + 26]), HI(x[B + 26]), ta2, tc2, LO(x[B + 25]), HI(x[B + 25]), LO(x[B + 27]), HI(x[B + 27]), ta3, tc3);
+        x[B + 12] = tc0; x[B + 14] = ta0;
+        x[B + 13] = tc1; x[B + 15] = ta1;
+        x[B + 24] = ta2; x[B + 26] = tc2;
+        x[B + 25] = ta3; x[B + 27] = tc3;
+    }
+    {
+        uint64_t ta0, tc0;
+        glasm::p2c0_x1(LO(x[B + 0]), HI(x[B + 0]), LO(x[B + 1]), HI(x[B + 1]), ta0, tc0);
+        x[B + 0] = ta0; x[B + 1] = tc0;
+    }
+    {
+        uint64_t ta0, tc0, ta1, tc1, ta2, tc2, ta3, tc3;
+        glasm::p2c1_x4<24, 12, 30, 6>(LO(x[B + 4]), HI(x[B + 4]), LO(x[B + 5]), HI(x[B + 5]), ta0, tc0, LO(x[B + 10]), HI(x[B + 10]), LO(x[B + 11]), HI(x[B + 11]), ta1, tc1, LO(x[B + 18]), HI(x[B + 18]), LO(x[B + 19]), HI(x[B + 19]), ta2, tc2, LO(x[B + 20]), HI(x[B + 20]), LO(x[B + 21]), HI(x[B + 21]), ta3, tc3);
+        x[B + 4] = tc0; x[B + 5] = ta0;
+        x[B + 10] = ta1; x[B + 11] = tc1;
+        x[B + 18] = tc2; x[B + 19] = ta2;
+        x[B + 20] = ta3; x[B + 21] = tc3;
+    }
+    {
+        uint64_t ta0, tc0;
+        glasm::p2c1_x1<18>(LO(x[B + 30]), HI(x[B + 30]), LO(x[B + 31]), HI(x[B + 31]), ta0, tc0);
+        x[B + 30] = ta0; x[B + 31] = tc0;
+    }
+    {
+        uint64_t ta0, tc0, ta1, tc1, ta2, tc2, ta3, tc3;
+        glasm::p2c2_x4<16, 28, 4, 22>(LO(x[B + 2]), HI(x[B + 2]), LO(x[B + 3]), HI(x[B + 3]), ta0, tc0, LO(x[B + 8]), HI(x[B + 8]), LO(x[B + 9]), HI(x[B + 9]), ta1, tc1, LO(x[B + 14]), HI(x[B + 14]), LO(x[B + 15]), HI(x[B + 15]), ta2, tc2, LO(x[B + 22]), HI(x[B + 22]), LO(x[B + 23]), HI(x[B + 23]), ta3, tc3);
+        x[B + 2] = ta0; x[B + 3] = tc0;
+        x[B + 8] = tc1; x[B + 9] = ta1;
+        x[B + 14] = tc2; x[B + 15] = ta2;
+        x[B + 22] = ta3; x[B + 23] = tc3;
+    }
+    {
+        uint64_t ta0, tc0;
+        glasm::p2c2_x1<10>(LO(x[B + 24]), HI(x[B + 24]), LO(x[B + 25]), HI(x[B + 25]), ta0, tc0);
+        x[B + 24] = ta0; x[B + 25] = tc0;
+    }
+    {
+        uint64_t ta0, tc0, ta1, tc1, ta2, tc2, ta3, tc3;
+        glasm::p2c3_x4<8, 20, 14, 26>(LO(x[B + 6]), HI(x[B + 6]), LO(x[B + 7]), HI(x[B + 7]), ta0, tc0, LO(x[B + 12]), HI(x[B + 12]), LO(x[B + 13]), HI(x[B + 13]), ta1, tc1, LO(x[B + 16]), HI(x[B + 16]), LO(x[B + 17]), HI(x[B + 17]), ta2, tc2, LO(x[B + 26]), HI(x[B + 26]), LO(x[B + 27]), HI(x[B + 27]), ta3, tc3);
+        x[B + 6] = tc0; x[B + 7] = ta0;
+        x[B + 12] = ta1; x[B + 13] = tc1;
+        x[B + 16] = ta2; x[B + 17] = tc2;
+        x[B + 26] = ta3; x[B + 27] = tc3;
+    }
+    {
+        uint64_t ta0, tc0;
+        glasm::p2c3_x1<2>(LO(x[B + 28]), HI(x[B + 28]), LO(x[B + 29]), HI(x[B + 29]), ta0, tc0);
+        x[B + 28] = tc0; x[B + 29] = ta0;
+    }
+}
+
+template <int B>
+__device__ __forceinline__ void dft2_inv(uint64_t* x) {
+    {
+        uint64_t ta0, tc0;
+        glasm::p2c0_x1(LO(x[B + 0]), HI(x[B + 0]), LO(x[B + 1]), HI(x[B + 1]), ta0, tc0);
+        x[B + 0] = ta0; x[B + 1] = tc0;
+    }
+}
+
+template <int B>
+__device__ __forceinline__ void dft4_inv(uint64_t* x) {
+    {
+        uint64_t ta0, tc0, ta1, tc1;
+        glasm::p2c0_x2(LO(x[B + 0]), HI(x[B + 0]), LO(x[B + 2]), HI(x[B + 2]), ta0, tc0, LO(x[B + 1]), HI(x[B + 1]), LO(x[B + 3]), HI(x[B + 3]), ta1, tc1);
+        x[B + 0] = ta0; x[B + 2] = tc0;
+        x[B + 1] = ta1; x[B + 3] = tc1;
+    }
+    {
+        uint64_t ta0, tc0;
+        glasm::p2c0_x1(LO(x[B + 0]), HI(x[B + 0]), LO(x[B + 1]), HI(x[B + 1]), ta0, tc0);
+        x[B + 0] = ta0; x[B + 1] = tc0;
+    }
+    {
+        uint64_t ta0, tc0;
+        glasm::p2c2_x1<16>(LO(x[B + 2]), HI(x[B + 2]), LO(x[B + 3]), HI(x[B + 3]), ta0, tc0);
+        x[B + 2] = tc0; x[B + 3] = ta0;
+    }
+}
+
+template <int B>
+__device__ __forceinline__ void dft8_inv(uint64_t* x) {
+    {
+        uint64_t ta0, tc0, ta1, tc1, ta2, tc2, ta3, tc3;
+        glasm::p2c0_x4(LO(x[B + 0]), HI(x[B + 0]), LO(x[B + 4]), HI(x[B + 4]), ta0, tc0, LO(x[B + 1]), HI(x[B + 1]), LO(x[B + 5]), HI(x[B + 5]), ta1, tc1, LO(x[B + 2]), HI(x[B + 2]), LO(x[B + 6]), HI(x[B + 6]), ta2, tc2, LO(x[B + 3]), HI(x[B + 3]), LO(x[B + 7]), HI(x[B + 7]), ta3, tc3);
+        x[B + 0] = ta0; x[B + 4] = tc0;
+        x[B + 1] = ta1; x[B + 5] = tc1;
+        x[B + 2] = ta2; x[B + 6] = tc2;
+        x[B + 3] = ta3; x[B + 7] = tc3;
+    }
+    {
         uint64_t ta0, tc0, ta1, tc1;
         glasm::p2c0_x2(LO(x[B + 0]), HI(x[B + 0]), LO(x[B + 2]), HI(x[B + 2]), ta0, tc0, LO(x[B + 1]), HI(x[B + 1]), LO(x[B + 3]), HI(x[B + 3]), ta1, tc1);
         x[B + 0] = ta0; x[B + 2] = tc0;
@@ -1660,6 +1988,122 @@
     }
 }
 
+template <int B>
+__device__ __forceinline__ void dft32_inv_from2(uint64_t* x) {
+    {
+        uint64_t ta0, tc0, ta1, tc1, ta2, tc2, ta3, tc3;
+        glasm::p2c0_x4(LO(x[B + 0]), HI(x[B + 0]), LO(x[B + 4]), HI(x[B + 4]), ta0, tc0, LO(x[B + 1]), HI(x[B + 1]), LO(x[B + 5]), HI(x[B + 5]), ta1, tc1, LO(x[B + 2]), HI(x[B + 2]), LO(x[B + 6]), HI(x[B + 6]), ta2, tc2, LO(x[B + 3]), HI(x[B + 3]), LO(x[B + 7]), HI(x[B + 7]), ta3, tc3);
+        x[B + 0] = ta0; x[B + 4] = tc0;
+        x[B + 1] = ta1; x[B + 5] = tc1;
+        x[B + 2] = ta2; x[B + 6] = tc2;
+        x[B + 3] = ta3; x[B + 7] = tc3;
+    }
+    {
+        uint64_t ta0, tc0, ta1, tc1, ta2, tc2, ta3, tc3;
+        glasm::p2c1_x4<24, 24, 24, 24>(LO(x[B + 24]), HI(x[B + 24]), LO(x[B + 28]), HI(x[B + 28]), ta0, tc0, LO(x[B + 25]), HI(x[B + 25]), LO(x[B + 29]), HI(x[B + 29]), ta1, tc1, LO(x[B + 26]), HI(x[B + 26]), LO(x[B + 30]), HI(x[B + 30]), ta2, tc2, LO(x[B + 27]), HI(x[B + 27]), LO(x[B + 31]), HI(x[B + 31]), ta3, tc3);
+        x[B + 24] = ta0; x[B + 28] = tc0;
+        x[B + 25] = ta1; x[B + 29] = tc1;
+        x[B + 26] = ta2; x[B + 30] = tc2;
+        x[B + 27] = ta3; x[B + 31] = tc3;
+    }
+    {
+        uint64_t ta0, tc0, ta1, tc1, ta2, tc2, ta3, tc3;
+        glasm::p2c2_x4<16, 16, 16, 16>(LO(x[B + 8]), HI(x[B + 8]), LO(x[B + 12]), HI(x[B + 12]), ta0, tc0, LO(x[B + 9]), HI(x[B + 9]), LO(x[B + 13]), HI(x[B + 13]), ta1, tc1, LO(x[B + 10]), HI(x[B + 10]), LO(x[B + 14]), HI(x[B + 14]), ta2, tc2, LO(x[B + 11]), HI(x[B + 11]), LO(x[B + 15]), HI(x[B + 15]), ta3, tc3);
+        x[B + 8] = tc0; x[B + 12] = ta0;
+        x[B + 9] = tc1; x[B + 13] = ta1;
+        x[B + 10] = tc2; x[B + 14] = ta2;
+        x[B + 11] = tc3; x[B + 15] = ta3;
+    }
+    {
+        uint64_t ta0, tc0, ta1, tc1, ta2, tc2, ta3, tc3;
+        glasm::p2c3_x4<8, 8, 8, 8>(LO(x[B + 16]), HI(x[B + 16]), LO(x[B + 20]), HI(x[B + 20]), ta0, tc0, LO(x[B + 17]), HI(x[B + 17]), LO(x[B + 21]), HI(x[B + 21]), ta1, tc1, LO(x[B + 18]), HI(x[B + 18]), LO(x[B + 22]), HI(x[B + 22]), ta2, tc2, LO(x[B + 19]), HI(x[B + 19]), LO(x[B + 23]), HI(x[B + 23]), ta3, tc3);
+        x[B + 16] = ta0; x[B + 20] = tc0;
+        x[B + 17] = ta1; x[B + 21] = tc1;
+        x[B + 18] = ta2; x[B + 22] = tc2;
+        x[B + 19] = ta3; x[B + 23] = tc3;
+    }
+    {
+        uint64_t ta0, tc0, ta1, tc1;
+        glasm::p2c0_x2(LO(x[B + 0]), HI(x[B + 0]), LO(x[B + 2]), HI(x[B + 2]), ta0, tc0, LO(x[B + 1]), HI(x[B + 1]), LO(x[B + 3]), HI(x[B + 3]), ta1, tc1);
+        x[B + 0] = ta0; x[B + 2] = tc0;
+        x[B + 1] = ta1; x[B + 3] = tc1;
+    }
+    {
+        uint64_t ta0, tc0, ta1, tc1, ta2, tc2, ta3, tc3;
+        glasm::p2c1_x4<24, 24, 12, 12>(LO(x[B + 12]), HI(x[B + 12]), LO(x[B + 14]), HI(x[B + 14]), ta0, tc0, LO(x[B + 13]), HI(x[B + 13]), LO(x[B + 15]), HI(x[B + 15]), ta1, tc1, LO(x[B + 24]), HI(x[B + 24]), LO(x[B + 26]), HI(x[B + 26]), ta2, tc2, LO(x[B + 25]), HI(x[B + 25]), LO(x[B + 27]), HI(x[B + 27]), ta3, tc3);
+        x[B + 12] = ta0; x[B + 14] = tc0;
+        x[B + 13] = ta1; x[B + 15] = tc1;
+        x[B + 24] = tc2; x[B + 26] = ta2;
+        x[B + 25] = tc3; x[B + 27] = ta3;
+    }
+    {
+        uint64_t ta0, tc0, ta1, tc1, ta2, tc2, ta3, tc3;
+        glasm::p2c2_x4<16, 16, 4, 4>(LO(x[B + 4]), HI(x[B + 4]), LO(x[B + 6]), HI(x[B + 6]), ta0, tc0, LO(x[B + 5]), HI(x[B + 5]), LO(x[B + 7]), HI(x[B + 7]), ta1, tc1, LO(x[B + 16]), HI(x[B + 16]), LO(x[B + 18]), HI(x[B + 18]), ta2, tc2, LO(x[B + 17]), HI(x[B + 17]), LO(x[B + 19]), HI(x[B + 19]), ta3, tc3);
+        x[B + 4] = tc0; x[B + 6] = ta0;
+        x[B + 5] = tc1; x[B + 7] = ta1;
+        x[B + 16] = ta2; x[B + 18] = tc2;
+        x[B + 17] = ta3; x[B + 19] = tc3;
+    }
+    {
+        uint64_t ta0, tc0, ta1, tc1;
+        glasm::p2c2_x2<28, 28>(LO(x[B + 28]), HI(x[B + 28]), LO(x[B + 30]), HI(x[B + 30]), ta0, tc0, LO(x[B + 29]), HI(x[B + 29]), LO(x[B + 31]), HI(x[B + 31]), ta1, tc1);
+        x[B + 28] = ta0; x[B + 30] = tc0;
+        x[B + 29] = ta1; x[B + 31] = tc1;
+    }
+    {
+        uint64_t ta0, tc0, ta1, tc1, ta2, tc2, ta3, tc3;
+        glasm::p2c3_x4<8, 8, 20, 20>(LO(x[B + 8]), HI(x[B + 8]), LO(x[B + 10]), HI(x[B + 10]), ta0, tc0, LO(x[B + 9]), HI(x[B + 9]), LO(x[B + 11]), HI(x[B + 11]), ta1, tc1, LO(x[B + 20]), HI(x[B + 20]), LO(x[B + 22]), HI(x[B + 22]), ta2, tc2, LO(x[B + 21]), HI(x[B + 21]), LO(x[B + 23]), HI(x[B + 23]), ta3, tc3);
+        x[B + 8] = ta0; x[B + 10] = tc0;
+        x[B + 9] = ta1; x[B + 11] = tc1;
+        x[B + 20] = tc2; x[B + 22] = ta2;
+        x[B + 21] = tc3; x[B + 23] = ta3;
+    }
+    {
+        uint64_t ta0, tc0;
+        glasm::p2c0_x1(LO(x[B + 0]), HI(x[B + 0]), LO(x[B + 1]), HI(x[B + 1]), ta0, tc0);
+        x[B + 0] = ta0; x[B + 1] = tc0;
+    }
+    {
+        uint64_t ta0, tc0, ta1, tc1, ta2, tc2, ta3, tc3;
+        glasm::p2c1_x4<24, 12, 18, 6>(LO(x[B + 6]), HI(x[B + 6]), LO(x[B + 7]), HI(x[B + 7]), ta0, tc0, LO(x[B + 12]), HI(x[B + 12]), LO(x[B + 13]), HI(x[B + 13]), ta1, tc1, LO(x[B + 16]), HI(x[B + 16]), LO(x[B + 17]), HI(x[B + 17]), ta2, tc2, LO(x[B + 26]), HI(x[B + 26]), LO(x[B + 27]), HI(x[B + 27]), ta3, tc3);
+        x[B + 6] = ta0; x[B + 7] = tc0;
+        x[B + 12] = tc1; x[B + 13] = ta1;
+        x[B + 16] = tc2; x[B + 17] = ta2;
+        x[B + 26] = tc3; x[B + 27] = ta3;
+    }
+    {
+        uint64_t ta0, tc0;
+        glasm::p2c1_x1<30>(LO(x[B + 28]), HI(x[B + 28]), LO(x[B + 29]), HI(x[B + 29]), ta0, tc0);
+        x[B + 28] = ta0; x[B + 29] = tc0;
+    }
+    {
+        uint64_t ta0, tc0, ta1, tc1, ta2, tc2, ta3, tc3;
+        glasm::p2c2_x4<16, 4, 28, 10>(LO(x[B + 2]), HI(x[B + 2]), LO(x[B + 3]), HI(x[B + 3]), ta0, tc0, LO(x[B + 8]), HI(x[B + 8]), LO(x[B + 9]), HI(x[B + 9]), ta1, tc1, LO(x[B + 14]), HI(x[B + 14]), LO(x[B + 15]), HI(x[B + 15]), ta2, tc2, LO(x[B + 22]), HI(x[B + 22]), LO(x[B + 23]), HI(x[B + 23]), ta3, tc3);
+        x[B + 2] = tc0; x[B + 3] = ta0;
+        x[B + 8] = ta1; x[B + 9] = tc1;
+        x[B + 14] = ta2; x[B + 15] = tc2;
+        x[B + 22] = tc3; x[B + 23] = ta3;
+    }
+    {
+        uint64_t ta0, tc0;
+        glasm::p2c2_x1<22>(LO(x[B + 24]), HI(x[B + 24]), LO(x[B + 25]), HI(x[B + 25]), ta0, tc0);
+        x[B + 24] = tc0; x[B + 25] = ta0;
+    }
+    {
+        uint64_t ta0, tc0, ta1, tc1, ta2, tc2, ta3, tc3;
+        glasm::p2c3_x4<8, 20, 2, 26>(LO(x[B + 4]), HI(x[B + 4]), LO(x[B + 5]), HI(x[B + 5]), ta0, tc0, LO(x[B + 10]), HI(x[B + 10]), LO(x[B + 11]), HI(x[B + 11]), ta1, tc1, LO(x[B + 18]), HI(x[B + 18]), LO(x[B + 19]), HI(x[B + 19]), ta2, tc2, LO(x[B + 20]), HI(x[B + 20]), LO(x[B + 21]), HI(x[B + 21]), ta3, tc3);
+        x[B + 4] = ta0; x[B + 5] = tc0;
+        x[B + 10] = tc1; x[B + 11] = ta1;
+        x[B + 18] = ta2; x[B + 19] = tc2;
+        x[B + 20] = tc3; x[B + 21] = ta3;
+    }
+    {
+        uint64_t ta0, tc0;
+        glasm::p2c3_x1<14>(LO(x[B + 30]), HI(x[B + 30]), LO(x[B + 31]), HI(x[B + 31]), ta0, tc0);
+        x[B + 30] = tc0; x[B + 31] = ta0;
+    }
+}
+
 #undef LO
 #undef HI
 }
```

After: 5.950 billion elems/s (median of 6 runs). Within noise of the previous version (+0.9%).
